# sile/libflate

Measured on AMD Instinct MI355X. Metric: gzip encode+decode throughput on 256 MiB synthetic text per GPU (uncompressed bytes through the round trip), higher is better.
Workload: dtype u8; 1 GPU; cfg2: gzip::Encoder (DefaultLz77Encoder, default options, mtime=0) + gzip::Decoder on TEXT(268435456 B) per GPU, write schedule S8K (8192-byte writes); bytes_per_gpu=268435456, schedule=S8K, compressed_bytes=129579521, parallelism=1 rank

## Files before the change

include/lfx_testhooks.h:

```cpp
#ifndef LFX_TESTHOOKS_H
#define LFX_TESTHOOKS_H

#include "lfx.h"

#ifdef __cplusplus
extern "C" {
#endif

int lfx_debug_huff_block(const uint32_t *hist320, uint32_t type, uint32_t *lit288, uint32_t *dist32, uint32_t *hdr160,
                         uint32_t *hdr_bits, uint64_t *body_bits);

int lfx_debug_plan(int format, const lfx_encode_opts *o, const lfx_schedule *s, uint64_t n, uint64_t *chunk_out,
                   size_t max_chunks, size_t *n_chunks, uint64_t *block_out, size_t max_blocks, size_t *n_blocks);

int lfx_debug_plan_incremental(int format, const lfx_encode_opts *o, const lfx_schedule *s, uint64_t n,
                               uint32_t take_every, uint64_t *chunk_out, size_t max_chunks, size_t *n_chunks,
                               uint64_t *block_out, size_t max_blocks, size_t *n_blocks);

void lfx_debug_symbols(uint32_t length, uint32_t distance, uint32_t *out6);

#ifdef __cplusplus
}
#endif
#endif
```

libflate_amd/_ffi.py:

```python
import ctypes as C
import os

_HERE = os.path.dirname(os.path.abspath(__file__))
SO_PATH = os.environ.get("LFX_SO") or os.path.join(_HERE, "liblfx.so")

DEFLATE, ZLIB, GZIP = 0, 1, 2
OK, E_INVALID_DATA, E_UNEXPECTED_EOF, E_IO, E_OOM, E_DEVICE, E_ARG, E_NOSPACE, E_UNSUPPORTED, E_WOULD_BLOCK = range(10)
LZ77_DEFAULT, LZ77_NOCOMPRESSION = 0, 1
FLUSH_NONE, FLUSH_SYNC = 0, 2
SCHED_SINGLE, SCHED_FIXED, SCHED_LIST = 0, 1, 2
SCHED_FLUSH = (1 << 64) - 1
DEC_MULTI = 1
DEC_NONBLOCKING = 2
MEMBERS_BGZF = 1
BGZF_MEMBER_SIZE = 65280

EXPORTS = [
    "lfx_encode_opts_default", "lfx_ctx_new", "lfx_ctx_free", "lfx_ctx_last_error", "lfx_ctx_set_stream",
    "lfx_device_count", "lfx_encode_bound", "lfx_encode_device", "lfx_encode_batch_device", "lfx_encode_host", "lfx_decode_device",
    "lfx_decode_host", "lfx_decode_batch_device", "lfx_encode_shard_prepare", "lfx_encode_shard_emit", "lfx_encode_shard_prezero", "lfx_decode_shard_device", "lfx_shard_place_device", "lfx_decode_range_scan", "lfx_decode_chain", "lfx_decode_range_emit", "lfx_decode_range_map", "lfx_decode_range_finish",
    "lfx_crc32_combine", "lfx_adler32_combine", "lfx_container_header_len", "lfx_encoder_new",
    "lfx_encoder_write", "lfx_encoder_write_codes", "lfx_encoder_flush", "lfx_encoder_finish", "lfx_encoder_last_error",
    "lfx_encoder_free", "lfx_decoder_new", "lfx_decoder_read", "lfx_decoder_unread",
    "lfx_decoder_consumed", "lfx_decoder_buffered", "lfx_decoder_surplus", "lfx_decoder_header", "lfx_decoder_last_error", "lfx_decoder_free", "lfx_lz77_new",
# ... 93 lines not shown
class LfxError(Exception):
    def __init__(self, status, message=""):
        super().__init__("lfx status %d: %s" % (status, message))
        self.status = status
        self.message = message


class DeviceError(LfxError):
    pass


_lib = None


def lib():
    global _lib
    if _lib is not None:
        return _lib
    if not os.path.exists(SO_PATH):
        raise ImportError(
            "libflate_amd: native library %s is missing — run `python -c 'import __graft_entry__ as g; "
            "g.build()'` (hipcc, gfx950). There is no CPU fallback." % SO_PATH)
    try:
        import torch
    except ImportError:
        pass
    L = C.CDLL(SO_PATH)
    u64, u32, vp, i32 = C.c_uint64, C.c_uint32, C.c_void_p, C.c_int
    L.lfx_encode_opts_default.argtypes = [C.POINTER(EncodeOpts)]
    L.lfx_ctx_new.restype = vp
    L.lfx_ctx_new.argtypes = [i32, C.POINTER(i32)]
    L.lfx_ctx_free.argtypes = [vp]
    L.lfx_ctx_last_error.restype = C.c_char_p
    L.lfx_ctx_last_error.argtypes = [vp]
    L.lfx_ctx_set_stream.argtypes = [vp, vp]
    L.lfx_encode_bound.restype = u64
    L.lfx_encode_bound.argtypes = [u64, C.POINTER(EncodeOpts), C.POINTER(Schedule)]
    L.lfx_encode_device.argtypes = [vp, i32, C.POINTER(EncodeOpts), C.POINTER(Schedule), vp, u64, vp, u64,
                                    C.POINTER(u64)]
    L.lfx_encode_host.argtypes = [vp, i32, C.POINTER(EncodeOpts), C.POINTER(Schedule), vp, u64, vp,
                                  u64, C.POINTER(u64)]
    L.lfx_host_alloc.restype = vp
    L.lfx_host_alloc.argtypes = [C.c_size_t]
    L.lfx_host_free.argtypes = [vp]
    L.lfx_ctx_match_fallbacks.restype = u64
    L.lfx_ctx_match_fallbacks.argtypes = [vp]
    L.lfx_decode_device.argtypes = [vp, i32, u32, vp, u64, vp, u64, C.POINTER(u64), C.POINTER(u64)]
    L.lfx_decode_host.argtypes = [vp, i32, u32, vp, u64, vp, u64, C.POINTER(u64), C.POINTER(u64)]
    L.lfx_decode_batch_device.argtypes = [vp, i32, u32, vp, vp, vp, vp, vp, vp, vp, vp]
    L.lfx_decode_members_device.argtypes = [vp, vp, u64, vp, u64, C.POINTER(u64), C.POINTER(u64), C.POINTER(Member), u32,
                                            C.POINTER(u32)]
    L.lfx_decode_members_host.argtypes = [vp, vp, u64, vp, u64, C.POINTER(u64), C.POINTER(u64), C.POINTER(Member), u32,
                                          C.POINTER(u32)]
    for f in (L.lfx_decode_size_device, L.lfx_decode_size_host):
        f.argtypes = [vp, i32, u32, vp, u64, C.POINTER(u64), C.POINTER(u64)]
    L.lfx_decode_batch_size_device.argtypes = [vp, i32, u32, vp, vp, vp, vp, vp, vp]
    for f in (L.lfx_decode_members_size_device, L.lfx_decode_members_size_host):
        f.argtypes = [vp, vp, u64, C.POINTER(u64), C.POINTER(u64), C.POINTER(Member), u32, C.POINTER(u32)]
    L.lfx_encode_members_bound.restype = u64
    L.lfx_encode_members_bound.argtypes = [u64, u64, u32, C.POINTER(EncodeOpts), C.POINTER(Schedule)]
    for f in (L.lfx_encode_members_device, L.lfx_encode_members_host):
        f.argtypes = [vp, C.POINTER(EncodeOpts), C.POINTER(Schedule), u64, u32, vp, u64, vp, u64, C.POINTER(u64),
                      C.POINTER(Member), u32, C.POINTER(u32)]
    L.lfx_members_gzi.argtypes = [C.POINTER(Member), u32, vp, u64, C.POINTER(u64)]
    L.lfx_decode_index_device.argtypes = [vp, i32, u32, vp, u64, vp, u64, C.POINTER(u64), C.POINTER(u64), u64, C.POINTER(vp)]
    L.lfx_encode_index_device.argtypes = [vp, i32, C.POINTER(EncodeOpts), C.POINTER(Schedule), vp, u64, vp, u64, C.POINTER(u64), u64,
                                          C.POINTER(vp)]
    L.lfx_index_read_device.argtypes = [vp, vp, vp, u64, u64, u32, vp, vp, vp, vp, vp, vp]
    L.lfx_index_span.argtypes = [vp, u64, u64, C.POINTER(u64), C.POINTER(u64)]
    L.lfx_index_get_info.argtypes = [vp, C.POINTER(IndexInfo)]
    L.lfx_index_get_point.argtypes = [vp, u32, C.POINTER(IndexPoint)]
    L.lfx_index_export.argtypes = [vp, vp, vp, u64, C.POINTER(u64)]
    L.lfx_index_import.argtypes = [vp, vp, u64, C.POINTER(i32)]
    L.lfx_index_import.restype = vp
    L.lfx_index_check.argtypes = [vp, u64, C.POINTER(IndexInfo)]
    L.lfx_index_free.argtypes = [vp]
    L.lfx_index_free.restype = None
    L.lfx_encode_batch_device.argtypes = [vp, i32, C.POINTER(EncodeOpts), C.POINTER(Schedule), u32, vp, vp, vp, vp, vp, vp, vp, vp]
    L.lfx_encode_shard_prepare.argtypes = [vp, i32, C.POINTER(EncodeOpts), C.POINTER(Schedule), vp, u64, i32,
                                           i32, C.POINTER(ShardInfo)]
    L.lfx_encode_shard_emit.argtypes = [vp, u64, u32, u64, vp, u64, C.POINTER(u64)]
    L.lfx_encode_shard_prezero.argtypes = [vp, vp, u64]
    L.lfx_decode_shard_device.argtypes = [vp, vp, u64, u64, u64, i32, vp, u64, C.POINTER(u64)]
    L.lfx_shard_place_device.argtypes = [vp, vp, u64, vp, u64, u64, i32]
    L.lfx_decode_range_scan.argtypes = [vp, vp, u64, u64, u64, u64, u64, u32, C.POINTER(BlkTuple), u32, C.POINTER(u32)]
    L.lfx_decode_chain.argtypes = [C.POINTER(BlkTuple), u32, u64, C.POINTER(u32), u32, C.POINTER(u32), C.POINTER(u64)]
    L.lfx_decode_range_emit.argtypes = [vp, vp, u64, u64, C.POINTER(BlkTuple), C.POINTER(u32), u32, u32, vp, u64,
                                        C.POINTER(u64), C.POINTER(u64), C.POINTER(u32)]
    L.lfx_decode_range_map.argtypes = [vp, vp]
    L.lfx_decode_range_finish.argtypes = [vp, vp, u32, C.POINTER(u32), C.POINTER(u32)]
    L.lfx_crc32_combine.restype = u32
    L.lfx_crc32_combine.argtypes = [u32, u32, u64]
    L.lfx_adler32_combine.restype = u32
    L.lfx_adler32_combine.argtypes = [u32, u32, u64]
    L.lfx_container_header_len.restype = u64
    L.lfx_container_header_len.argtypes = [i32, C.POINTER(EncodeOpts)]
    L.lfx_encoder_new.restype = vp
    L.lfx_encoder_new.argtypes = [vp, i32, C.POINTER(EncodeOpts), WRITE_CB, FLUSH_CB, vp, C.POINTER(i32)]
    L.lfx_encoder_write.restype = C.c_int64
    L.lfx_encoder_write.argtypes = [vp, C.c_char_p, C.c_size_t]
    L.lfx_encoder_write_codes.argtypes = [vp, C.POINTER(u32), C.c_size_t, C.c_char_p, C.c_size_t, i32]
    L.lfx_encoder_flush.argtypes = [vp]
    L.lfx_encoder_finish.argtypes = [vp]
    L.lfx_encoder_last_error.restype = C.c_char_p
    L.lfx_encoder_last_error.argtypes = [vp]
    L.lfx_encoder_free.argtypes = [vp]
    L.lfx_decoder_new.restype = vp
    L.lfx_decoder_new.argtypes = [vp, i32, u32, READ_CB, vp, C.POINTER(i32)]
    L.lfx_decoder_read.restype = C.c_int64
    L.lfx_decoder_read.argtypes = [vp, vp, C.c_size_t]
    L.lfx_decoder_unread.argtypes = [vp, C.POINTER(C.POINTER(C.c_uint8)), C.POINTER(C.c_size_t)]
    L.lfx_decoder_consumed.restype = u64
    L.lfx_decoder_consumed.argtypes = [vp]
    L.lfx_decoder_buffered.restype = u64
    L.lfx_decoder_buffered.argtypes = [vp]
    L.lfx_decoder_surplus.argtypes = [vp, C.POINTER(C.POINTER(C.c_uint8)), C.POINTER(C.c_size_t)]
    L.lfx_decoder_header.argtypes = [vp, C.POINTER(Header)]
    L.lfx_decoder_last_error.restype = C.c_char_p
    L.lfx_decoder_last_error.argtypes = [vp]
    L.lfx_decoder_free.argtypes = [vp]
    L.lfx_lz77_new.restype = vp
    L.lfx_lz77_new.argtypes = [vp, u32, u32, C.POINTER(i32)]
    L.lfx_lz77_encode.argtypes = [vp, C.c_char_p, C.c_size_t, SINK_CB, vp]
    L.lfx_lz77_flush.argtypes = [vp, SINK_CB, vp]
    L.lfx_lz77_window_size.restype = u32
    L.lfx_lz77_window_size.argtypes = [vp]
    L.lfx_lz77_compression_level.argtypes = [vp]
    L.lfx_lz77_free.argtypes = [vp]
    L.lfx_ctx_last_timing.argtypes = [vp, C.POINTER(Timing)]
    L.lfx_ctx_enable_timing.argtypes = [vp, i32]
    L.lfx_version.restype = u32
    L.lfx_comm_rccl.argtypes = [vp, vp, u32, u32, C.POINTER(Comm)]
    L.lfx_comm_rccl_free.argtypes = [C.POINTER(Comm)]
    L.lfx_comm_rccl_free.restype = None
    L.lfx_sharded_encode_begin.argtypes = [vp, C.POINTER(Comm), i32, C.POINTER(EncodeOpts), C.POINTER(Schedule), vp, u64, vp, u64,
                                           vp, u64, vp, u64, C.POINTER(vp), C.POINTER(ShardedPart)]
    L.lfx_sharded_encode_finish.argtypes = [vp, C.POINTER(Comm), vp, C.POINTER(u64)]
    L.lfx_sharded_byte_range.argtypes = [u64, u64, u32, u32, C.POINTER(u64), C.POINTER(u64), C.POINTER(u64)]
    L.lfx_sharded_byte_range.restype = None
    L.lfx_sharded_decode.argtypes = [vp, C.POINTER(Comm), vp, u64, u64, u64, u64, u64, vp, u64, C.POINTER(ShardedSlice)]
    L.lfx_sharded_layout.argtypes = [C.POINTER(Comm), C.POINTER(ShardInfo), u64, i32, C.POINTER(u64), C.POINTER(u32), C.POINTER(u64)]
    L.lfx_sharded_gather_tuples.argtypes = [C.POINTER(Comm), C.POINTER(BlkTuple), u32, i32, C.POINTER(C.POINTER(BlkTuple)),
                                            C.POINTER(u32), C.POINTER(u32)]
    L.lfx_sharded_fold.argtypes = [C.POINTER(Comm), i32, u32, u64, u32, u32, C.POINTER(u32), C.POINTER(u32), C.POINTER(u32),
                                   C.POINTER(u64), C.POINTER(u32)]
    L.lfx_sharded_free.argtypes = [vp]
    L.lfx_sharded_free.restype = None
    L.lfx_debug_huff_block.argtypes = [vp, u32, vp, vp, vp, C.POINTER(u32), C.POINTER(u64)]
    L.lfx_debug_plan.argtypes = [i32, C.POINTER(EncodeOpts), C.POINTER(Schedule), u64, vp, C.c_size_t,
                                 C.POINTER(C.c_size_t), vp, C.c_size_t, C.POINTER(C.c_size_t)]
    L.lfx_debug_plan_incremental.argtypes = [i32, C.POINTER(EncodeOpts), C.POINTER(Schedule), u64, u32, vp, C.c_size_t,
                                             C.POINTER(C.c_size_t), vp, C.c_size_t, C.POINTER(C.c_size_t)]
    L.lfx_debug_symbols.argtypes = [u32, u32, vp]
    _lib = L
    return L


def make_opts(**kw):
    o = EncodeOpts()
    lib().lfx_encode_opts_default(C.byref(o))
    keep = []
    for k, v in kw.items():
        if k == "extra":
            v = bytes(v)
            keep.append(v)
            o.extra, o.extra_len = v, len(v)
        elif k in ("filename", "comment"):
            v = bytes(v)
            keep.append(v)
            setattr(o, k, v)
        else:
            setattr(o, k, v)
    o._keep = keep
    return o


def members_to_gzi(members):
    members = list(members)
    table = (Member * max(len(members), 1))()
    for i, m in enumerate(members):
        table[i].in_off, table[i].in_len, table[i].out_off, table[i].out_len = m
    need = C.c_uint64(0)
    lib().lfx_members_gzi(table, len(members), None, 0, C.byref(need))
    buf = C.create_string_buffer(need.value)
    rc = lib().lfx_members_gzi(table, len(members), buf, need.value, C.byref(need))
    if rc:
        raise LfxError(rc, "lfx_members_gzi")
    return buf.raw[:need.value]


def make_schedule(write_size=0, writes=None):
    s = Schedule()
    if writes is not None:
        arr = (C.c_uint64 * len(writes))(*[SCHED_FLUSH if w is None else int(w) for w in writes])
        s.kind, s.writes, s.n_writes = SCHED_LIST, arr, len(writes)
        s._keep = arr
    elif write_size:
        s.kind, s.fixed_write = SCHED_FIXED, write_size
    else:
        s.kind = SCHED_SINGLE
    return s
```

libflate_amd/context.py:

```python
import ctypes as C

from . import _ffi


class Context:
    def __init__(self, device=0):
        st = C.c_int(0)
        self._h = _ffi.lib().lfx_ctx_new(device, C.byref(st))
        if not self._h:
            raise _ffi.DeviceError(st.value, "no usable MI355X device %d (there is no CPU fallback)" % device)
        self.device = device
        self._users = 0
        self._closing = False

    def _retain(self):
        self._users += 1

    def _release(self):
        self._users -= 1
        if self._users <= 0 and self._closing:
            self._free_now()

    def _free_now(self):
        if self._h:
            _ffi.lib().lfx_ctx_free(self._h)
            self._h = None

    def close(self):
        self._closing = True
        if self._users <= 0:
            self._free_now()

    def __del__(self):
        try:
            self.close()
        except Exception:
            pass

    @property
    def handle(self):
        return self._h

    def last_error(self):
        return (_ffi.lib().lfx_ctx_last_error(self._h) or b"").decode("utf-8", "replace")

    def set_stream(self, hip_stream_ptr):
        _ffi.lib().lfx_ctx_set_stream(self._h, hip_stream_ptr)

    def enable_timing(self, on=True):
        _ffi.lib().lfx_ctx_enable_timing(self._h, int(on) if on is not True and on is not False and 2 <= int(on) <= 6 else (1 if on else 0))

    def last_timing(self):
        t = _ffi.Timing()
        if _ffi.lib().lfx_ctx_last_timing(self._h, C.byref(t)) != 0:
            return None
        return {"total_ms": t.total_ms,
                "phases": [(bytes(t.phase_name[i]).split(b"\0")[0].decode(), t.phase_ms[i])
                           for i in range(t.n_phases)]}

    def match_fallbacks(self):
        return int(_ffi.lib().lfx_ctx_match_fallbacks(self._h))

    def encode_host_ptr(self, fmt, in_ptr, n, out_ptr, cap, opts=None, schedule=None):
        out_len = C.c_uint64(0)
        rc = _ffi.lib().lfx_encode_host(self._h, fmt, C.byref(opts) if opts is not None else None,
                                        C.byref(schedule) if schedule is not None else None, in_ptr, n, out_ptr, cap, C.byref(out_len))
        if rc:
            raise (_ffi.DeviceError if rc == _ffi.E_DEVICE else _ffi.LfxError)(rc, self.last_error())
        return out_len.value

    def decode_host_ptr(self, fmt, in_ptr, n, out_ptr, cap, flags=0):
        out_len, consumed = C.c_uint64(0), C.c_uint64(0)
        rc = _ffi.lib().lfx_decode_host(self._h, fmt, flags, in_ptr, n, out_ptr, cap, C.byref(out_len), C.byref(consumed))
        if rc in (_ffi.E_DEVICE, _ffi.E_OOM, _ffi.E_ARG):
            raise (_ffi.DeviceError if rc == _ffi.E_DEVICE else _ffi.LfxError)(rc, self.last_error())
        return rc, out_len.value, consumed.value, self.last_error() if rc else ""

    def encode_device(self, fmt, d_in, n, d_out, cap, opts=None, schedule=None):
        out_len = C.c_uint64(0)
        rc = _ffi.lib().lfx_encode_device(self._h, fmt, C.byref(opts) if opts is not None else None,
                                          C.byref(schedule) if schedule is not None else None,
                                          d_in, n, d_out, cap, C.byref(out_len))
        if rc:
            raise (_ffi.DeviceError if rc == _ffi.E_DEVICE else _ffi.LfxError)(rc, self.last_error())
        return out_len.value

    def encode_index_device(self, fmt, d_in, n, d_out, cap, opts=None, schedule=None, spacing=1 << 20):
        out_len, h = C.c_uint64(0), C.c_void_p(None)
        rc = _ffi.lib().lfx_encode_index_device(self._h, fmt, C.byref(opts) if opts is not None else None,
                                                C.byref(schedule) if schedule is not None else None,
                                                d_in, n, d_out, cap, C.byref(out_len), spacing, C.byref(h))
        if rc:
            raise (_ffi.DeviceError if rc == _ffi.E_DEVICE else _ffi.LfxError)(rc, self.last_error())
        return out_len.value, h.value

    def decode_device(self, fmt, d_in, n, d_out, cap, flags=0):
        out_len, consumed = C.c_uint64(0), C.c_uint64(0)
        rc = _ffi.lib().lfx_decode_device(self._h, fmt, flags, d_in, n, d_out, cap, C.byref(out_len),
                                          C.byref(consumed))
        if rc in (_ffi.E_DEVICE, _ffi.E_OOM, _ffi.E_ARG):
            raise (_ffi.DeviceError if rc == _ffi.E_DEVICE else _ffi.LfxError)(rc, self.last_error())
        return rc, out_len.value, consumed.value, self.last_error() if rc else ""

    def decode_members_device(self, d_in, n, d_out, cap, max_members=None):
        return self._members(_ffi.lib().lfx_decode_members_device, d_in, n, d_out, cap, max_members)

    def decode_index_device(self, fmt, d_in, n, d_out, cap, spacing=1 << 20, flags=0):
        out_len, consumed, h = C.c_uint64(0), C.c_uint64(0), C.c_void_p(None)
        rc = _ffi.lib().lfx_decode_index_device(self._h, fmt, flags, d_in, n, d_out, cap, C.byref(out_len), C.byref(consumed),
                                                spacing, C.byref(h))
        if rc in (_ffi.E_DEVICE, _ffi.E_OOM, _ffi.E_ARG):
            raise (_ffi.DeviceError if rc == _ffi.E_DEVICE else _ffi.LfxError)(rc, self.last_error())
        return rc, out_len.value, consumed.value, h.value, self.last_error() if rc else ""

    def index_read_device(self, index_handle, d_in, in_base, n, offs, lens, d_out, out_offs):
        k = len(offs)
        a = lambda v: (C.c_uint64 * max(k, 1))(*v)
        o, ln, oo = a(offs), a(lens), a(out_offs)
        out_len, st = (C.c_uint64 * max(k, 1))(), (C.c_int32 * max(k, 1))()
        rc = _ffi.lib().lfx_index_read_device(self._h, index_handle, d_in, in_base, n, k, o, ln, d_out, oo, out_len, st)
        if rc in (_ffi.E_DEVICE, _ffi.E_OOM) or (rc == _ffi.E_ARG and not any(st[i] == _ffi.E_ARG for i in range(k))):
            raise (_ffi.DeviceError if rc == _ffi.E_DEVICE else _ffi.LfxError)(rc, self.last_error())
        return rc, list(out_len[:k]), list(st[:k]), self.last_error() if rc else ""

    def _members(self, fn, src, n, dst, cap, max_members):
        if max_members is None:
            max_members = n // 20 + 1
        table = (_ffi.Member * max(int(max_members), 1))()
        out_len, consumed, count = C.c_uint64(0), C.c_uint64(0), C.c_uint32(0)
        rc = fn(self._h, src, n, dst, cap, C.byref(out_len), C.byref(consumed), table, int(max_members), C.byref(count))
        if rc in (_ffi.E_DEVICE, _ffi.E_OOM, _ffi.E_ARG):
            raise (_ffi.DeviceError if rc == _ffi.E_DEVICE else _ffi.LfxError)(rc, self.last_error())
        members = [(m.in_off, m.in_len, m.out_off, m.out_len) for m in table[:min(count.value, int(max_members))]]
        return rc, out_len.value, consumed.value, members, self.last_error() if rc else ""

    def decode_members_host(self, data, cap=None, max_members=None):
        data = bytes(data)
        grow = cap is None
        cap = cap if cap is not None else max(1 << 16, len(data) * 16)
        while True:
            out = C.create_string_buffer(cap)
            rc, ol, used, members, msg = self._members(_ffi.lib().lfx_decode_members_host, data, len(data), out, cap, max_members)
            if grow and rc == _ffi.E_NOSPACE and cap < len(data) * 1040 + (1 << 20):
                cap *= 8
                continue
            return rc, out.raw[:ol], used, members, msg

    def _raise_fatal(self, rc):
        if rc in (_ffi.E_DEVICE, _ffi.E_OOM, _ffi.E_ARG):
            raise (_ffi.DeviceError if rc == _ffi.E_DEVICE else _ffi.LfxError)(rc, self.last_error())

    def decode_size_device(self, fmt, d_in, n, flags=0):
        out_len, consumed = C.c_uint64(0), C.c_uint64(0)
        rc = _ffi.lib().lfx_decode_size_device(self._h, fmt, flags, d_in, n, C.byref(out_len), C.byref(consumed))
        self._raise_fatal(rc)
        return rc, out_len.value, consumed.value, self.last_error() if rc else ""

    def decode_size_host(self, fmt, data, flags=0):
        data = bytes(data)
        out_len, consumed = C.c_uint64(0), C.c_uint64(0)
        rc = _ffi.lib().lfx_decode_size_host(self._h, fmt, flags, data, len(data), C.byref(out_len), C.byref(consumed))
        self._raise_fatal(rc)
        return rc, out_len.value, consumed.value, self.last_error() if rc else ""

    def decode_batch_size_device(self, fmt, d_in, in_offs, in_lens):
        k = len(in_offs)
        a = lambda v: (C.c_uint64 * max(k, 1))(*v)
        io, il = a(in_offs), a(in_lens)
        ol, used, st = (C.c_uint64 * max(k, 1))(), (C.c_uint64 * max(k, 1))(), (C.c_int32 * max(k, 1))()
        rc = _ffi.lib().lfx_decode_batch_size_device(self._h, fmt, k, d_in, io, il, ol, used, st)
        if rc:
            raise (_ffi.DeviceError if rc == _ffi.E_DEVICE else _ffi.LfxError)(rc, self.last_error())
        return list(ol[:k]), list(used[:k]), list(st[:k])

    def _members_size(self, fn, src, n, max_members):
        if max_members is None:
            max_members = n // 20 + 1
        table = (_ffi.Member * max(int(max_members), 1))()
        out_len, consumed, count = C.c_uint64(0), C.c_uint64(0), C.c_uint32(0)
        rc = fn(self._h, src, n, C.byref(out_len), C.byref(consumed), table, int(max_members), C.byref(count))
        self._raise_fatal(rc)
        members = [(m.in_off, m.in_len, m.out_off, m.out_len) for m in table[:min(count.value, int(max_members))]]
        return rc, out_len.value, consumed.value, members, self.last_error() if rc else ""

    def decode_members_size_device(self, d_in, n, max_members=None):
        return self._members_size(_ffi.lib().lfx_decode_members_size_device, d_in, n, max_members)

    def decode_members_size_host(self, data, max_members=None):
        data = bytes(data)
        return self._members_size(_ffi.lib().lfx_decode_members_size_host, data, len(data), max_members)

    def _encode_members(self, fn, src, n, dst, cap, member_size, flags, opts, schedule, max_members):
        count = 0 if (flags & _ffi.MEMBERS_BGZF and n == 0) else max(1, -(-n // member_size)) if member_size else 0
        if max_members is None:
            max_members = count
        table = (_ffi.Member * max(int(max_members), 1))()
        out_len, got = C.c_uint64(0), C.c_uint32(0)
        rc = fn(self._h, C.byref(opts) if opts is not None else None, C.byref(schedule) if schedule is not None else None,
                member_size, flags, src, n, dst, cap, C.byref(out_len), table, int(max_members), C.byref(got))
        if rc in (_ffi.E_DEVICE, _ffi.E_OOM, _ffi.E_ARG, _ffi.E_UNSUPPORTED):
            raise (_ffi.DeviceError if rc == _ffi.E_DEVICE else _ffi.LfxError)(rc, self.last_error())
        members = [(m.in_off, m.in_len, m.out_off, m.out_len) for m in table[:min(got.value, int(max_members))]]
        return rc, out_len.value, got.value, members, self.last_error() if rc else ""

    def encode_members_device(self, d_in, n, d_out, cap, member_size=1 << 20, flags=0, opts=None, schedule=None, max_members=None):
        return self._encode_members(_ffi.lib().lfx_encode_members_device, d_in, n, d_out, cap, member_size, flags, opts, schedule,
                                    max_members)

    def encode_members_host(self, data, member_size=1 << 20, flags=0, opts=None, schedule=None, cap=None, max_members=None):
        data = bytes(data)
        if cap is None:
# ... 46 lines not shown
```

libflate_amd/csrc/lfx_api.cpp:

```cpp
#include "../../include/lfx.h"
#include "../../include/lfx_testhooks.h"

#include <hip/hip_runtime.h>

#include <algorithm>
#include <cstddef>
#include <cstdio>
#include <cstdlib>
#include <cstring>
#include <mutex>
#include <string>
#include <vector>

#include "lfx_ctx.h"
#include "lfx_device.h"
#include "lfx_huff.h"
#include "lfx_index.h"
#include "lfx_plan.h"
#include "lfx_abi_guard.h"

using namespace lfx;

static uint32_t host_crc32(const uint8_t *p, size_t n) {
    static uint32_t tab[256];
// ... 54 lines not shown
    lfx_encode_opts d;
    if (o) d = *o; else lfx_encode_opts_default(&d);
    if (d.window_size > MAX_WINDOW) d.window_size = MAX_WINDOW;
    if (d.max_length > MAX_LENGTH) d.max_length = MAX_LENGTH;
    return d;
}
static int check_opts(const lfx_encode_opts &o) {
    if (o.block_size == 0) return LFX_E_ARG;
    if (o.max_length < 3) return LFX_E_ARG;
    return LFX_OK;
}
static PlanOpts plan_opts(int format, const lfx_encode_opts &o) {
    PlanOpts p;
    p.block_size = o.block_size;
    p.dynamic_huffman = o.dynamic_huffman != 0;
    p.no_compression = o.no_compression != 0;
    p.lz77_kind = o.lz77_kind;
    p.window_size = o.window_size;
    p.max_length = o.max_length;
    p.zlib_sync = format == LFX_ZLIB && o.zlib_flush_mode == LFX_FLUSH_SYNC;
    return p;
}

static void gzip_header(const lfx_encode_opts &o, bool with_hcrc, std::vector<uint8_t> &b) {
    uint8_t flg = (uint8_t)((o.is_text ? 1 : 0) | (with_hcrc ? 2 : 0) | (o.extra ? 4 : 0) |
                            (o.filename ? 8 : 0) | (o.comment ? 16 : 0));
    const uint8_t xfl = o.lz77_level == 1 + LFX_LEVEL_FAST ? 4 : o.lz77_level == 1 + LFX_LEVEL_BEST ? 2 : 0;
    const uint8_t h[10] = {31, 139, 8, flg, (uint8_t)o.mtime, (uint8_t)(o.mtime >> 8),
                           (uint8_t)(o.mtime >> 16), (uint8_t)(o.mtime >> 24), xfl, o.os};
    b.insert(b.end(), h, h + 10);
    if (o.extra) {
        b.push_back((uint8_t)o.extra_len);
        b.push_back((uint8_t)(o.extra_len >> 8));
        b.insert(b.end(), o.extra, o.extra + o.extra_len);
    }
    if (o.filename) b.insert(b.end(), o.filename, o.filename + strlen(o.filename) + 1);
    if (o.comment) b.insert(b.end(), o.comment, o.comment + strlen(o.comment) + 1);
    if (with_hcrc) {
        std::vector<uint8_t> t;
        gzip_header(o, false, t);
        uint32_t c = host_crc32(t.data(), t.size());
        b.push_back((uint8_t)c);
        b.push_back((uint8_t)(c >> 8));
    }
}
static int container_header(int format, const lfx_encode_opts &o, std::vector<uint8_t> &b) {
    if (format == LFX_GZIP) {
        if (o.extra && o.extra_len > 0xFFFF) return LFX_E_INVALID_DATA;
        gzip_header(o, o.hcrc != 0, b);
    } else if (format == LFX_ZLIB) {
        uint32_t ws = o.window_size;
        uint8_t cinfo = ws > 16384 ? 7 : ws > 8192 ? 6 : ws > 4096 ? 5 : ws > 2048 ? 4 : ws > 1024 ? 3
                        : ws > 512 ? 2 : ws > 256 ? 1 : 0;
        uint8_t level = (o.no_compression || o.lz77_kind == LFX_LZ77_NOCOMPRESSION) ? 0 : 2;
        if (o.lz77_level && !o.no_compression) level = (uint8_t)((o.lz77_level - 1) & 3);
        uint8_t cmf = (uint8_t)((cinfo << 4) | 8), flg = (uint8_t)(level << 6);
        uint32_t check = ((uint32_t)cmf << 8) + flg;
        if (check % 31 != 0) flg = (uint8_t)(flg + (31 - check % 31));
        b.push_back(cmf);
        b.push_back(flg);
    } else if (format != LFX_DEFLATE) {
        return LFX_E_ARG;
    }
    return LFX_OK;
}
extern "C" uint64_t lfx_container_header_len(int format, const lfx_encode_opts *o) {
    std::vector<uint8_t> b;
    lfx_encode_opts d = norm_opts(o);
    container_header(format, d, b);
    return b.size();
}

static void apply_schedule(Planner &pl, const lfx_schedule *s, uint64_t n) {
    if (!s || s->kind == LFX_SCHED_SINGLE) {
        pl.write(n);
    } else if (s->kind == LFX_SCHED_FIXED) {
        uint64_t w = s->fixed_write ? s->fixed_write : n;
        if (w) {
            pl.write_repeat(w, n / w);
            if (n % w) pl.write(n % w);
        }
    } else {
        uint64_t used = 0;
        for (size_t i = 0; i < s->n_writes; i++) {
            if (s->writes[i] == LFX_SCHED_FLUSH) { pl.flush(); continue; }
            uint64_t w = std::min(s->writes[i], n - used);
            pl.write(w);
            used += w;
        }
        if (used < n) pl.write(n - used);
    }
}

extern "C" uint64_t lfx_encode_bound(uint64_t n, const lfx_encode_opts *o, const lfx_schedule *s) {
    lfx_encode_opts d = norm_opts(o);
    if (check_opts(d)) return 0;
    Planner pl(plan_opts(LFX_ZLIB, d));
    apply_schedule(pl, s, n);
    Plan &p = pl.finish();
    uint64_t hdr = 64 + (d.extra ? d.extra_len + 2 : 0) + (d.filename ? strlen(d.filename) + 1 : 0) +
                   (d.comment ? strlen(d.comment) + 1 : 0);
    return n + n / 4 + 1024 * (uint64_t)p.blocks.size() + hdr + 64;
}

namespace lfx {

#define HIP_TRY(expr)                                                                 \
    do {                                                                              \
        hipError_t e_ = (expr);                                                       \
        if (e_ != hipSuccess) {                                                       \
            c->set_error(std::string(#expr) + ": " + hipGetErrorString(e_));          \
            return LFX_E_DEVICE;                                                      \
        }                                                                             \
    } while (0)

int DevBuf::reserve(size_t bytes) {
    if (bytes <= cap) return 0;
    if (p) (void)hipFree(p);
    p = nullptr;
    cap = 0;
    gen++;
    size_t want = bytes + bytes / 8 + 4096;
    if (hipMalloc(&p, want) != hipSuccess) {
        if (hipMalloc(&p, bytes) != hipSuccess) { p = nullptr; return LFX_E_OOM; }
        want = bytes;
    }
    cap = want;
    return 0;
}
void DevBuf::release() {
    if (p) (void)hipFree(p);
    p = nullptr;
    cap = 0;
}

void Diag::read() {
    auto on = [](const char *k) { return getenv(k) != nullptr; };
    debug = on("LFX_DEBUG");
    match_v1 = on("LFX_MATCH_V1");
    match_v5 = on("LFX_MATCH_V5");
    if (const char *mp = getenv("LFX_MATCH_PARTS")) match_parts = atoi(mp);
    if (const char *rc7 = getenv("LFX_R7_CAP")) r7_cap = atoi(rc7);
    no_serial = on("LFX_NO_SERIAL");
    batch_serial = on("LFX_BATCH_SERIAL");
    no_pieces = on("LFX_NO_PIECES");
    no_final_cand = on("LFX_NO_FINAL_CAND");
    if (const char *eb = getenv("LFX_ENC_BATCH_MB")) enc_batch_mb = atoi(eb);
    two_pass = on("LFX_TWO_PASS");
    hist_separate = on("LFX_HIST_SEPARATE");
    find2_exp = getenv("LFX_FIND2_EXP") ? atoi(getenv("LFX_FIND2_EXP")) : 0;
    no_pin_slots = on("LFX_NO_PIN_SLOTS");
    no_small_scan = on("LFX_NO_SMALL_SCAN");
    store_tight = on("LFX_STORE_TIGHT");
}

void Ctx::phase(const char *name) {
    if (!timing_on) return;
    if (timing_on >= 2 && timing_on <= 5) {
        static const char *const pair[4][2] = {{"lz77_resolve", "lz77_walk"}, {"find2", "blk_scan"}, {"upload", "lz77_cand"}, {"blk_emit", "lz77_copy"}};
        const char *const *pr = pair[timing_on - 2];
        if (strcmp(name, pr[0]) != 0 && strcmp(name, pr[1]) != 0) return;
    }
    if (n_ev >= 17) return;
    if (!ev[n_ev]) (void)hipEventCreate(&ev[n_ev]);
    (void)hipEventRecord(ev[n_ev], stream);
    snprintf(ev_name[n_ev], sizeof ev_name[n_ev], "%s", name);
    n_ev++;
}

}

extern "C" int lfx_device_count(void) {
    int n = 0;
    if (hipGetDeviceCount(&n) != hipSuccess) return 0;
    return n;
}

extern "C" lfx_ctx *lfx_ctx_new(int device, int *status) try {
    int st = LFX_OK;
    int n = 0;
    if (hipGetDeviceCount(&n) != hipSuccess || n <= 0 || device < 0 || device >= n) {
        if (status) *status = LFX_E_DEVICE;
        return nullptr;
    }
    Ctx *c = new Ctx();
    c->device = device;
    if (hipSetDevice(device) != hipSuccess || hipStreamCreate(&c->own_stream) != hipSuccess) {
        delete c;
        if (status) *status = LFX_E_DEVICE;
        return nullptr;
    }
    c->stream = c->own_stream;
    c->diag.read();
    (void)hipDeviceGetAttribute(&c->n_cu, hipDeviceAttributeMultiprocessorCount, device);
    if (hipStreamCreateWithFlags(&c->side_stream, hipStreamNonBlocking) != hipSuccess ||
        hipEventCreateWithFlags(&c->ev_fork, hipEventDisableTiming) != hipSuccess ||
        hipEventCreateWithFlags(&c->ev_join, hipEventDisableTiming) != hipSuccess ||
        hipEventCreateWithFlags(&c->ev_zero, hipEventDisableTiming) != hipSuccess ||
        hipEventCreateWithFlags(&c->ev_res, hipEventDisableTiming) != hipSuccess ||
        hipEventCreateWithFlags(&c->ev_part[0], hipEventDisableTiming) != hipSuccess ||
        hipEventCreateWithFlags(&c->ev_part[1], hipEventDisableTiming) != hipSuccess ||
        hipEventCreateWithFlags(&c->ev_part[2], hipEventDisableTiming) != hipSuccess ||
        hipEventCreateWithFlags(&c->ev_part[3], hipEventDisableTiming) != hipSuccess) {
        (void)hipStreamDestroy(c->own_stream);
        delete c;
        if (status) *status = LFX_E_DEVICE;
        return nullptr;
    }
    if (hipHostMalloc((void **)&c->h_res, 4096 + Ctx::PIN_ARENA, hipHostMallocDefault) != hipSuccess) {
        (void)hipStreamDestroy(c->own_stream);
        delete c;
        if (status) *status = LFX_E_OOM;
        return nullptr;
    }
    if (status) *status = st;
    return reinterpret_cast<lfx_ctx *>(c);
} LFX_ABI_CATCH_NEW
extern "C" void lfx_ctx_free(lfx_ctx *cc) {
    if (!cc) return;
    Ctx *c = reinterpret_cast<Ctx *>(cc);
    (void)hipSetDevice(c->device);
    (void)hipStreamSynchronize(c->stream);
    for (DevBuf *b : c->all_bufs()) b->release();
    for (DevBuf &b : c->dev_pool) b.release();
    c->dev_pool.clear();
    c->pin_pool.clear();
    for (auto &e : c->ev) if (e) (void)hipEventDestroy(e);
    if (c->h_res) (void)hipHostFree(c->h_res);
    c->hostio.release();
    if (c->ev_fork) (void)hipEventDestroy(c->ev_fork);
    if (c->ev_join) (void)hipEventDestroy(c->ev_join);
    if (c->ev_zero) (void)hipEventDestroy(c->ev_zero);
    if (c->ev_res) (void)hipEventDestroy(c->ev_res);
    for (hipEvent_t e : c->ev_part) if (e) (void)hipEventDestroy(e);
    if (c->side_stream) (void)hipStreamDestroy(c->side_stream);
    if (c->own_stream) (void)hipStreamDestroy(c->own_stream);
    delete c;
}
extern "C" const char *lfx_ctx_last_error(const lfx_ctx *cc) {
    return cc ? reinterpret_cast<const Ctx *>(cc)->err.c_str() : "no context";
}
extern "C" void lfx_ctx_set_stream(lfx_ctx *cc, void *s) {
    Ctx *c = reinterpret_cast<Ctx *>(cc);
    c->stream = s ? (hipStream_t)s : c->own_stream;
}
extern "C" uint64_t lfx_ctx_match_fallbacks(const lfx_ctx *cc) {
    return cc ? reinterpret_cast<const Ctx *>(cc)->match_fallbacks : 0;
}
extern "C" void lfx_ctx_enable_timing(lfx_ctx *cc, int on) { reinterpret_cast<Ctx *>(cc)->timing_on = on >= 2 && on <= 6 ? on : on != 0; }
extern "C" int lfx_ctx_last_timing(lfx_ctx *cc, lfx_timing *t) try {
    Ctx *c = reinterpret_cast<Ctx *>(cc);
    std::lock_guard<std::recursive_mutex> lock(c->mu);
    memset(t, 0, sizeof *t);
    if (c->n_ev < 2) return LFX_E_ARG;
    (void)hipEventSynchronize(c->ev[c->n_ev - 1]);
    (void)hipEventElapsedTime(&t->total_ms, c->ev[0], c->ev[c->n_ev - 1]);
    t->n_phases = c->n_ev - 1;
    for (int i = 0; i + 1 < c->n_ev && i < 16; i++) {
        (void)hipEventElapsedTime(&t->phase_ms[i], c->ev[i], c->ev[i + 1]);
        snprintf(t->phase_name[i], sizeof t->phase_name[i], "%s", c->ev_name[i + 1]);
    }
    return LFX_OK;
} LFX_ABI_CATCH

namespace lfx {

int encode_prepare(Ctx *c, const Plan &plan, const PlanOpts &po, const uint8_t *d_in, uint64_t n,
                   int ck_mode, const HostCodes *hc) {
    const bool want_checksum = ck_mode != 0;
    (void)hipSetDevice(c->device);
    hipStream_t st = c->stream;
    c->n_ev = 0;
    c->phase("start");
    for (const ChunkDesc &ch : plan.chunks)
        if (ch.len >= (1ull << 32) - 4) {
            c->set_error("an LZ77 chunk of 4 GiB or more is outside the reference's domain (u32 positions, default.rs:78)");
            return LFX_E_ARG;
        }
    const uint32_t nchunks = (uint32_t)plan.chunks.size(), nblocks = (uint32_t)plan.blocks.size();
    const bool match_v1 = c->force_match_v1 || c->diag.match_v1;
    if (c->force_match_v1 && !hc) c->match_fallbacks++;
    std::vector<SegDesc> segs;
    if (!hc) {
        uint64_t seg_len = SEG_POSITIONS;
        for (;;) {
            uint64_t cnt = 0;
            for (const ChunkDesc &ch : plan.chunks)
                if (!(ch.flags & CH_LITERALS) && ch.len > 3) cnt += div_up(ch.len - 3, seg_len);
            if (cnt >= 512 || seg_len <= 32768) break;
            seg_len /= 2;
        }
        for (uint32_t ci = 0; ci < nchunks; ci++) {
            const ChunkDesc &ch = plan.chunks[ci];
            if (ch.flags & CH_LITERALS) continue;
            for (uint64_t s = 0; s + 3 < ch.len; s += seg_len)
                segs.push_back(SegDesc{ci, (uint32_t)s, (uint32_t)std::min<uint64_t>(seg_len, ch.len - s), 0});
        }
    }
    uint64_t lnk_units = 0;
    for (SegDesc &sg : segs) {
        if (lnk_units > 0xFFFFFFFFull) { c->set_error("input too large for the link scratch"); return LFX_E_ARG; }
        sg.lnk_base = (uint32_t)lnk_units;
        lnk_units += div_up((uint64_t)sg.len + std::min<uint64_t>(sg.start, MAX_WINDOW) + 4, 64);
        lnk_units = (lnk_units + 1) & ~1ull;
    }
    std::vector<ParseWg> pwgs;
    for (uint32_t ci = 0; ci < nchunks && !hc; ci++) {
        const ChunkDesc &ch = plan.chunks[ci];
        if (ch.flags & CH_LITERALS) continue;
        for (uint32_t s = 0; s < ch.n_seg; s += PARSE_WG_SEGS) pwgs.push_back(ParseWg{ci, s});
    }
    if (pwgs.size() > 8) {
        const size_t nl = pwgs.size(), per = (nl + 7) / 8;
        std::vector<ParseWg> phys(per * 8);
        for (size_t i = 0; i < phys.size(); i++) {
            const size_t l = (i % 8) * per + i / 8;
            phys[i] = (i / 8 < per && l < nl && l / per == i % 8) ? pwgs[l] : ParseWg{0xFFFFFFFFu, 0u};
        }
        pwgs.swap(phys);
    }
    c->cur_nchunks = nchunks;
    c->cur_nblocks = nblocks;
    c->cur_ntiles = plan.n_tiles;
    c->cur_n = n;
    c->cur_in = d_in;
    int rc;
    if ((rc = c->d_chunks.reserve(sizeof(ChunkDesc) * std::max<size_t>(nchunks, 1)))) return rc;
    if ((rc = c->d_blocks.reserve(sizeof(BlockDesc) * std::max<size_t>(nblocks, 1)))) return rc;
    if ((rc = c->d_segs.reserve(sizeof(SegDesc) * std::max<size_t>(segs.size(), 1)))) return rc;
    if ((rc = c->d_pwgs.reserve(sizeof(ParseWg) * std::max<size_t>(pwgs.size(), 1)))) return rc;
    if (!hc && (rc = c->d_cd.reserve(2 * n + 64))) return rc;
    if (!hc && !match_v1 && (rc = c->d_glnk.reserve(264 * std::max<uint64_t>(lnk_units, 1)))) return rc;
    if (!hc && !match_v1 && (rc = c->d_ucount.reserve(4 * std::max<size_t>(segs.size(), 1)))) return rc;
    if (!hc && match_v1 && (rc = c->d_md.reserve(4 * std::max<uint64_t>(n, 1)))) return rc;
    if ((rc = c->d_codes.reserve(4 * std::max<uint64_t>(plan.n_codes_cap, 1)))) return rc;
    if ((rc = c->d_ncodes.reserve(4 * std::max<size_t>(nchunks, 1)))) return rc;
    if ((rc = c->d_vis.reserve(8 * std::max<uint64_t>(plan.n_vis, 1)))) return rc;
    if ((rc = c->d_segtmp.reserve(24ull * std::max<uint32_t>(plan.n_segs, 1)))) return rc;
    if (!hc && (rc = c->d_stage.reserve(4ull * (n + 64)))) return rc;
    if ((rc = c->d_chunkmap.reserve(4ull * (plan.n_tiles + plan.n_segs + 2)))) return rc;
    if ((rc = c->d_hist.reserve(4ull * 320 * std::max<size_t>(nblocks, 1)))) return rc;
    if ((rc = c->d_bc.reserve(sizeof(BlockCodes) * std::max<size_t>(nblocks, 1)))) return rc;
    if ((rc = c->d_block_start.reserve(8 * std::max<size_t>(nblocks, 1)))) return rc;
    if ((rc = c->d_tile_bits.reserve(4 * std::max<uint64_t>(plan.n_tiles, 1)))) return rc;
    if ((rc = c->d_tile_start.reserve(8 * std::max<uint64_t>(plan.n_tiles, 1)))) return rc;
    const uint64_t nspans = ck_nspans(n);
    if ((rc = c->d_ck.reserve(12 * nspans))) return rc;
    if ((rc = c->d_res.reserve(256))) return rc;
    if ((rc = c->d_small.reserve(70000))) return rc;

    auto upload = [&](int slot, DevBuf &b, const void *src, size_t bytes) -> hipError_t {
        std::vector<uint8_t> &sh = c->up_shadow[slot];
        const uint64_t tag = (uint64_t)(uintptr_t)b.p ^ ((uint64_t)b.gen << 48) ^ (1ull << 63);
        if (c->up_dev[slot] == tag && sh.size() == bytes && (bytes == 0 || memcmp(sh.data(), src, bytes) == 0)) return hipSuccess;
        sh.assign((const uint8_t *)src, (const uint8_t *)src + bytes);
        c->up_dev[slot] = tag;
        return bytes ? hipMemcpyAsync(b.p, sh.data(), bytes, hipMemcpyHostToDevice, st) : hipSuccess;
    };
    HIP_TRY(upload(0, c->d_chunks, plan.chunks.data(), sizeof(ChunkDesc) * nchunks));
    HIP_TRY(upload(1, c->d_blocks, plan.blocks.data(), sizeof(BlockDesc) * nblocks));
    HIP_TRY(upload(2, c->d_segs, segs.data(), sizeof(SegDesc) * segs.size()));
    HIP_TRY(upload(3, c->d_pwgs, pwgs.data(), sizeof(ParseWg) * pwgs.size()));
    const bool ucount_here = !hc && !match_v1 && !c->diag.match_v5;
    const ZeroSpan z_hist{(uint32_t *)c->d_hist.p, (uint32_t)(320 * std::max<size_t>(nblocks, 1))}, z_res{(uint32_t *)c->d_res.p, 64u},
        z_ucount{ucount_here ? (uint32_t *)c->d_ucount.p : nullptr, ucount_here ? (uint32_t)std::max<size_t>(segs.size(), 1) : 0u};
    c->phase("upload");
    uint32_t *tile_map = (uint32_t *)c->d_chunkmap.p, *seg_map = tile_map + plan.n_tiles;
    c->cur_tile_map = tile_map;
    if (int e_ = launch_chunk_maps(st, (const ChunkDesc *)c->d_chunks.p, nchunks, plan.n_tiles, plan.n_segs, tile_map, seg_map, z_hist,
                                   z_res, z_ucount)) {
        c->set_error(hipGetErrorString((hipError_t)e_));
        return LFX_E_DEVICE;
    }

#define LAUNCH_TRY(call)                                                              \
    do {                                                                              \
        int e_ = (call);                                                              \
        if (e_) {                                                                     \
            c->set_error(std::string(#call) + ": " + hipGetErrorString((hipError_t)e_)); \
            return LFX_E_DEVICE;                                                      \
        }                                                                             \
    } while (0)

    uint64_t *mdbg = nullptr;
    if (c->diag.debug) mdbg = (uint64_t *)((uint8_t *)c->d_small.p + 32768);
    bool fused_hist = false;
    bool forked = false;
    uint32_t emit_per = 0, emit_parts = 0;
    if (hc) {
        if (hc->n_codes) HIP_TRY(hipMemcpyAsync(c->d_codes.p, hc->codes, 4ull * hc->n_codes, hipMemcpyHostToDevice, st));
        if (nchunks) HIP_TRY(hipMemcpyAsync(c->d_ncodes.p, hc->chunk_codes, 4ull * nchunks, hipMemcpyHostToDevice, st));
        c->phase("codes_upload");
    } else {
    uint32_t *d_match_flags = (uint32_t *)((uint8_t *)c->d_res.p + offsetof(EncodeResult, match_flags));
    uint16_t *d_cd = (uint16_t *)c->d_cd.p;
    if (match_v1) {
        LAUNCH_TRY(launch_match(st, d_in, n, (const ChunkDesc *)c->d_chunks.p, (const SegDesc *)c->d_segs.p,
                                (uint32_t)segs.size(), po.window_size, po.max_length, (uint32_t *)c->d_md.p, mdbg));
        LAUNCH_TRY(launch_md_to_cd(st, (const uint32_t *)c->d_md.p, n, d_cd));
    } else {
// ... 1164 lines not shown
```

libflate_amd/csrc/lfx_blk.h:

```cpp
#pragma once
#include <stdint.h>

namespace lfx {

enum : uint32_t { BLK_OK = 0, BLK_BAD = 1, BLK_NO_EOB = 2 };
constexpr uint32_t BLK_PIECE_KNOWN = 2;
struct BlkJob {
    uint64_t start_bit;
    uint64_t end_bit;
    uint64_t lo_bit, warm_bit;
    uint32_t piece, _pad;
    uint64_t temp_off;
    uint32_t cap, _pad2;
};
struct BlkInfo {
    uint64_t end_bit;
    uint64_t n_out;
    uint64_t data_bit;
    uint32_t n_codes;
    uint32_t status, btype, bfinal, nlanes, rounds;
    uint32_t _pad;
    uint32_t cyc_hdr, cyc_total;
};
struct BlkLanes {
    uint64_t start[1024];
    uint64_t out_off[1024];
    uint32_t code_off[1024];
};
struct BlkLanesX {
    uint32_t n_head[1024];
    uint32_t n_rest[1024];
    uint32_t rest_at[1024];
    int32_t reach[1024];
    uint32_t cut_code[1024];
    uint32_t cut_out[1024];
};
struct BlkEmit {
    uint64_t start_bit, data_bit;
    uint64_t code_off;
    uint64_t out_off;
    uint64_t n_out;
    uint32_t n_codes, nlanes, btype, cand;
    uint64_t hist;
    uint64_t end_limit;
    uint32_t preload;
    uint32_t placed;
    uint64_t temp_off;
    uint32_t cap, _pad;
};
constexpr uint32_t MAX_FREE_UNITS = 64;
struct BlkUnits {
    uint32_t n;
    uint32_t code0[9];
    uint64_t out0[9];
    uint32_t cyc[4];
    uint32_t fn;
    uint32_t fcode0[MAX_FREE_UNITS + 1];
    uint64_t fout0[MAX_FREE_UNITS + 1];
};
struct SymUnit {
    uint64_t start;
    uint64_t len;
};
}
```

libflate_amd/csrc/lfx_ctx.h:

```cpp
#pragma once
#include <hip/hip_runtime.h>

#include <mutex>
#include <string>
#include <vector>

#include "lfx_common.h"
#include "lfx_device.h"
#include <string.h>

#include "lfx_hostio.h"

namespace lfx {

struct DevBuf {
    void *p = nullptr;
    size_t cap = 0;
    uint32_t gen = 0;
    int reserve(size_t bytes);
    void release();
};

struct Diag {
    bool debug = false;
    bool match_v1 = false;
    bool match_v5 = false;
    int r7_cap = 0;
    int match_parts = 1;
    bool no_serial = false;
    bool batch_serial = false;
    bool no_pieces = false;
    bool no_final_cand = false;
    bool no_small_scan = false;
    bool two_pass = false;
    bool no_pin_slots = false;
    int find2_exp = 0;
    bool hist_separate = false;
    bool store_tight = false;
    int enc_batch_mb = 0;
    void read();
};

struct RangeState {
    int state = -1;
    uint64_t total = 0, before = 0, max_len = 0;
    uint8_t *d_out = nullptr;
    uint32_t nsu = 0;
};

struct Ctx {
    int device = 0;
    RangeState range;
    std::vector<uint8_t> range_stored;
    std::vector<uint64_t> range_temp_off;
    std::vector<uint32_t> range_cap;
    Diag diag;
    int n_cu = 0;
    hipStream_t own_stream = nullptr, stream = nullptr;
    hipStream_t side_stream = nullptr;
    hipEvent_t ev_fork = nullptr, ev_join = nullptr, ev_zero = nullptr;
    hipEvent_t ev_part[4] = {}, ev_res = nullptr;
    const void *prezero_ptr = nullptr;
    uint64_t prezero_bytes = 0;
    std::recursive_mutex mu;
    std::string err;
    void set_error(const std::string &e) { err = e; }

    DevBuf d_chunks, d_blocks, d_segs, d_pwgs, d_cd, d_md, d_codes, d_ncodes, d_hist, d_bc, d_block_start, d_tile_bits,
        d_tile_start, d_ck, d_res, d_small, d_hdr, d_io_in, d_io_out, d_vis, d_segtmp, d_stage, d_chunkmap, d_glnk, d_ucount;
    std::vector<uint8_t> up_shadow[4];
    uint64_t up_dev[4] = {0, 0, 0, 0};
    DevBuf d_dec_streams, d_dec_state, d_dec_tmp, d_dec_cand, d_dec_blocks, d_dec_tabs, d_dec_sym, d_dec_win, d_dec_maps,
        d_dec_temp, d_dec_lanesx;
    DevBuf d_idx_tasks, d_idx_probe, d_idx_stage;
    DevBuf d_idx_enc;
    struct IdxCollect *idx = nullptr;
    struct IdxCollect *idx_enc = nullptr;
    std::vector<DevBuf *> all_bufs() {
        return {&d_chunks, &d_blocks, &d_segs, &d_pwgs, &d_cd, &d_md, &d_codes, &d_ncodes, &d_hist, &d_bc, &d_block_start,
                &d_tile_bits, &d_tile_start, &d_ck, &d_res, &d_small, &d_hdr, &d_io_in, &d_io_out, &d_vis, &d_segtmp, &d_stage, &d_chunkmap, &d_glnk, &d_ucount,
                &d_dec_streams, &d_dec_state, &d_dec_tmp, &d_dec_cand, &d_dec_blocks, &d_dec_tabs, &d_dec_sym, &d_dec_win, &d_dec_maps,
                &d_dec_temp, &d_dec_lanesx, &d_idx_tasks, &d_idx_probe, &d_idx_stage, &d_idx_enc};
    }
    void *h_res = nullptr;
    static constexpr size_t PIN_ARENA = 1u << 20;
    size_t pin_used = 0;
    struct PinDown { void *slot, *dst; size_t n; };
    std::vector<PinDown> pin_pending;
    void pin_reset() { pin_used = 0; pin_pending.clear(); }
    void *pin_take(size_t n) {
        const size_t at = (pin_used + 63) & ~(size_t)63;
        if (!h_res || diag.no_pin_slots || at + n > PIN_ARENA) return nullptr;
        pin_used = at + n;
        return (uint8_t *)h_res + 4096 + at;
    }
    hipError_t small_up(void *dev, const void *host, size_t n, hipStream_t st) {
        if (!n) return hipSuccess;
        void *slot = pin_take(n);
        if (!slot) return hipMemcpyAsync(dev, host, n, hipMemcpyHostToDevice, st);
        memcpy(slot, host, n);
        return hipMemcpyAsync(dev, slot, n, hipMemcpyHostToDevice, st);
    }
    hipError_t small_down(void *host, const void *dev, size_t n, hipStream_t st) {
        if (!n) return hipSuccess;
        void *slot = pin_take(n);
        if (!slot) return hipMemcpyAsync(host, dev, n, hipMemcpyDeviceToHost, st);
        pin_pending.push_back({slot, host, n});
        return hipMemcpyAsync(slot, dev, n, hipMemcpyDeviceToHost, st);
    }
    hipError_t small_sync(hipStream_t st) {
        const hipError_t e = hipStreamSynchronize(st);
        for (const PinDown &d : pin_pending) memcpy(d.dst, d.slot, d.n);
        pin_pending.clear();
        return e;
    }

    uint32_t cur_nchunks = 0, cur_nblocks = 0;
    uint64_t cur_ntiles = 0, cur_n = 0;
    const uint32_t *cur_tile_map = nullptr;
    const uint8_t *cur_in = nullptr;
    bool force_match_v1 = false;
    uint64_t match_fallbacks = 0;
    HostIo hostio;
    static constexpr size_t POOL_MAX = 8;
    std::vector<PinVec> pin_pool;
    std::vector<DevBuf> dev_pool;
    PinVec take_pin() {
        std::lock_guard<std::recursive_mutex> lock(mu);
        if (pin_pool.empty()) return PinVec();
        size_t best = 0;
        for (size_t i = 1; i < pin_pool.size(); i++)
            if (pin_pool[i].capacity() > pin_pool[best].capacity()) best = i;
        PinVec v = std::move(pin_pool[best]);
        pin_pool.erase(pin_pool.begin() + (std::ptrdiff_t)best);
        v.clear();
        return v;
    }
    void give_pin(PinVec &&v) {
        std::lock_guard<std::recursive_mutex> lock(mu);
        if (v.capacity() && pin_pool.size() < POOL_MAX) { v.clear(); pin_pool.push_back(std::move(v)); }
    }
    DevBuf take_dev() {
        std::lock_guard<std::recursive_mutex> lock(mu);
        if (dev_pool.empty()) return DevBuf();
        DevBuf b = dev_pool.back();
        dev_pool.pop_back();
        return b;
    }
    void give_dev(DevBuf &b) {
        std::lock_guard<std::recursive_mutex> lock(mu);
        if (b.p && dev_pool.size() < POOL_MAX) dev_pool.push_back(b);
        else b.release();
        b = DevBuf();
    }
    std::vector<uint8_t> shard_hdr;
    int shard_format = 0;
    bool shard_last = false;

    int timing_on = 0;
    bool timing_fine() const { return timing_on >= 2; }
    hipEvent_t ev[17] = {};
    char ev_name[17][24] = {};
    int n_ev = 0;
    void phase(const char *name);
};

struct HostCodes {
    const uint32_t *codes;
    uint64_t n_codes;
    const uint32_t *chunk_codes;
};
int encode_prepare(Ctx *c, const struct Plan &plan, const struct PlanOpts &po, const uint8_t *d_in,
                   uint64_t n, int ck_mode, const HostCodes *hc = nullptr);

}
```

libflate_amd/csrc/lfx_decode.h:

```cpp
#pragma once
#include <hip/hip_runtime.h>
#include <stdint.h>

#include "lfx_common.h"
#include "lfx_blk.h"

namespace lfx {

enum : uint32_t {
    ERR_NONE = 0,
    ERR_EOF,
    ERR_HUFF,
    ERR_CONFLICT,
    ERR_HDIST,
    ERR_NO_PREV,
    ERR_DIST_LIST,
    ERR_286,
    ERR_BACKREF,
    ERR_BTYPE3,
    ERR_LEN_NLEN,
    ERR_STORED_SHORT,
    ERR_NOSPACE,
    ERR_ZLIB_CHECK, ERR_METHOD, ERR_CINFO, ERR_FDICT,
    ERR_GZIP_ID, ERR_HCRC,
    ERR_CRC32, ERR_ADLER32,
};

struct DecStream {
    uint64_t in_off, in_len;
    uint64_t out_off, out_cap;
};
struct DecHeader {
    uint64_t deflate_off;
    uint32_t status;
    uint32_t err, a0, a1;
    uint32_t flags;
    uint32_t _pad;
};

enum : uint32_t { JOB_SINGLE_BLOCK = 1, JOB_COUNT_ONLY = 2 };
struct InflateJob {
    uint64_t in_off;
    uint64_t in_len;
    uint64_t start_bit;
    uint64_t out_off, out_cap;
    uint64_t hist_avail;
    uint64_t stop_bit;
    uint32_t flags;
    uint32_t _pad;
};
struct InflateResult {
    uint64_t end_bit;
    uint64_t out_len;
    uint32_t status;
    uint32_t final_seen;
    uint32_t err, a0, a1;
    uint32_t needs_hist;
    uint32_t nblocks;
    uint32_t _pad;
    uint64_t blk_out_start;
    uint64_t blk_start_bit;
};

enum : uint32_t { WALK_FINAL = 0,
                  WALK_STOP = 1,
                  WALK_STUCK = 2 };
struct WalkJob {
    uint64_t start_bit;
    uint64_t end_bit;
    uint64_t stop_bit;
};
struct WalkResult {
    uint64_t end_bit;
    uint64_t n_out;
    uint64_t stuck_bit, stuck_out;
    int64_t reach;
    uint32_t status, nblocks;
};
int launch_blk_walk_size(hipStream_t st, const uint8_t *in, uint64_t nbytes, const WalkJob *jobs, uint32_t njobs,
                         WalkResult *results, bool small_blocks);
size_t blk_tabs_bytes();
int launch_blk_scan(hipStream_t st, const uint8_t *in, uint64_t nbytes, const BlkJob *jobs, uint32_t njobs,
                    BlkInfo *infos, BlkLanes *lanes, void *tabs = nullptr,
                    bool small_blocks = false);
int launch_blk_scan_store(hipStream_t st, const uint8_t *in, uint64_t nbytes, const BlkJob *jobs, uint32_t njobs,
                          BlkInfo *infos, BlkLanes *lanes, void *tabs, uint32_t *temp, BlkLanesX *lanesx);
int launch_blk_place(hipStream_t st, const BlkEmit *jobs, uint32_t njobs, const BlkLanes *lanes, const BlkLanesX *lanesx,
                     const uint32_t *temp, uint32_t *codes, uint32_t *flags, BlkUnits *units, uint32_t unit_target,
                     uint32_t *job_flags, uint32_t free_shift);
int launch_blk_emit(hipStream_t st, const uint8_t *in, uint64_t nbytes, const BlkEmit *jobs, uint32_t njobs,
                    const BlkLanes *lanes, uint32_t *codes, uint32_t *flags, BlkUnits *units, uint32_t unit_target,
                    uint32_t *job_flags = nullptr,
                    const void *tabs = nullptr,
                    uint32_t free_shift = 17,
                    bool large_blocks = false,
                    bool small_blocks = false);
int launch_blk_materialize(hipStream_t st, const uint8_t *in, const BlkEmit *jobs, uint32_t njobs,
                           const BlkLanes *lanes, const BlkUnits *units, const uint32_t *codes, uint8_t *out,
                           uint64_t *dbg);

int launch_blk_materialize_sym(hipStream_t st, const uint8_t *in, const BlkEmit *jobs, uint32_t njobs,
                               const BlkUnits *units, const uint32_t *codes, uint16_t *sym,
                               bool few_units = false );
int launch_window_chain(hipStream_t st, const uint16_t *sym, const SymUnit *units, uint32_t nunits, uint8_t *windows,
                        const uint8_t *init_win = nullptr);
size_t window_prefix_scratch_bytes(uint32_t nunits);
int launch_window_prefix(hipStream_t st, const uint16_t *sym, const SymUnit *units, uint32_t nunits, void *scratch,
                         uint8_t *windows, const uint8_t *init_win = nullptr);
int launch_window_rank_map(hipStream_t st, const uint16_t *sym, const SymUnit *units, uint32_t nunits, void *scratch, uint16_t *out_map);
int launch_bytes_to_map(hipStream_t st, const uint8_t *out, uint64_t len, uint16_t *map);
int launch_window_ranks(hipStream_t st, const uint16_t *maps, uint32_t nranks, uint8_t *win);
int launch_sym_substitute(hipStream_t st, const uint16_t *sym, const SymUnit *units, uint32_t nunits,
                          const uint8_t *windows, uint8_t *out, uint64_t max_len, const uint8_t *init_win = nullptr);

int launch_container(hipStream_t st, int format, uint32_t count, const uint8_t *in,
                     const DecStream *streams, DecHeader *hdrs);
int launch_inflate(hipStream_t st, const uint8_t *in, uint8_t *out, const InflateJob *jobs,
                   InflateResult *results, uint32_t njobs);
constexpr uint32_t FIND_SHARDS = 256;
constexpr uint32_t FIND_HDR_WORDS = 1024, FIND_HDR_FINAL = 320, FIND_HDR_DBG = 360, FIND_HDR_READ = 512 ;
constexpr uint32_t FIND2_GROUPS = 16, FIND_HDR_WORK = 512, FIND_HDR_WORK_STRIDE = 32;
inline uint32_t find_shard_cap(uint64_t comp_bytes) {
    const uint64_t want = comp_bytes / 4000;
    return (uint32_t)(want < 4096 ? 4096 : want > (1u << 23) ? (1u << 23) : want);
}
int launch_find_stage1(hipStream_t st, const uint8_t *in, uint64_t nbytes, uint64_t first_byte,
                       uint32_t *count, uint64_t *cand, uint32_t shard_cap, uint64_t final_from_bit, uint32_t n_cu);
int launch_find_stage2(hipStream_t st, const uint8_t *in, uint64_t nbytes, const uint64_t *cand,
                       uint32_t shard_cap, const uint32_t *count ,
                       uint32_t *work ,
                       uint32_t *final_count, uint64_t *final_list, uint32_t final_cap, uint32_t n_cu,
                       uint64_t *dbg = nullptr ,
                       int exp = 0 );
constexpr uint64_t MEMBER_TILE = 16384;
constexpr uint64_t MEMBER_SKIP = ~0ull;
inline uint64_t member_tiles(uint64_t n) { return (n + MEMBER_TILE - 1) / MEMBER_TILE; }
int launch_member_count(hipStream_t st, const uint8_t *in, uint64_t n, uint32_t *tile_count );
int launch_member_emit(hipStream_t st, const uint8_t *in, uint64_t n, const uint64_t *tile_pos ,
                       uint64_t *out, uint64_t cap);
int launch_verify_trailers(hipStream_t st, int format, uint32_t count, const uint8_t *in,
                           const DecStream *streams, const DecHeader *hdrs, InflateResult *results,
                           const uint32_t *crc, const uint32_t *adler, uint64_t *consumed);
}
```

libflate_amd/csrc/lfx_device.h:

```cpp
#pragma once
#include <hip/hip_runtime.h>
#include <stdint.h>

#include "../../include/lfx.h"
#include "lfx_common.h"

namespace lfx {

struct SegDesc {
    uint32_t chunk;
    uint32_t start;
    uint32_t len;
    uint32_t lnk_base;
};
constexpr uint32_t SEG_POSITIONS = 256 * 1024;

struct EncodeResult {
    uint64_t end_bit;
    uint64_t out_bytes;
    uint32_t status;
    uint32_t crc32;
    uint32_t adler32;
    uint32_t match_flags;
};

struct BatchStream {
    uint64_t in_off, in_len;
    uint64_t out_off, out_cap;
    uint32_t first_block, n_blocks;
};

struct ParseWg {
    uint32_t chunk;
    uint32_t seg0;
};

int launch_match(hipStream_t st, const uint8_t *in, uint64_t in_bytes, const ChunkDesc *chunks,
                 const SegDesc *segs, uint32_t nsegs, uint32_t window, uint32_t max_len, uint32_t *md,
                 uint64_t *dbg = nullptr);
int launch_match7(hipStream_t st, const uint8_t *in, uint64_t in_bytes, const ChunkDesc *chunks, const SegDesc *segs,
                  uint32_t nsegs, uint32_t window, uint16_t *cd, uint32_t *glnk ,
                  uint64_t *umask , uint32_t *flags, uint64_t *dbg = nullptr);
int launch_resolve7(hipStream_t st, const ChunkDesc *chunks, const SegDesc *segs, uint32_t nsegs, uint32_t window, uint16_t *cd,
                    const uint32_t *glnk, const uint64_t *umask, uint32_t *ulist ,
                    uint32_t *ucount ,
                    uint32_t hop_cap = 0 );
int launch_match5(hipStream_t st, const uint8_t *in, uint64_t in_bytes, const ChunkDesc *chunks, const SegDesc *segs,
                  uint32_t nsegs, uint32_t window, uint16_t *cd, uint16_t *glnk, uint32_t *flags, uint64_t *dbg = nullptr);
int launch_md_to_cd(hipStream_t st, const uint32_t *md, uint64_t n, uint16_t *cd);
int launch_parse(hipStream_t st, const uint8_t *in, uint64_t in_bytes, const ChunkDesc *chunks, uint32_t nchunks,
                 uint32_t nsegs, const ParseWg *wgs, uint32_t nwgs, const uint16_t *cd, uint32_t max_len, uint64_t *vis,
                 uint32_t *seg_tmp, uint32_t *codes, uint32_t *ncodes, uint32_t *stage ,
                 const uint32_t *seg_map, int stop_after = 0 ,
                 uint64_t *dbg = nullptr ,
                 uint32_t *hist = nullptr ,
                 uint32_t emit_per = 0 ,
                 uint32_t emit_parts = 0 ,
                 hipEvent_t ev_walked = nullptr ,
                 const uint32_t *mflags = nullptr ,
                 int start_at = 0 );
struct ZeroSpan { uint32_t *p; uint32_t n; };
int launch_chunk_maps(hipStream_t st, const ChunkDesc *chunks, uint32_t nchunks, uint64_t ntiles, uint32_t nsegs,
                      uint32_t *tile_map, uint32_t *seg_map, ZeroSpan z0 = ZeroSpan{nullptr, 0}, ZeroSpan z1 = ZeroSpan{nullptr, 0},
                      ZeroSpan z2 = ZeroSpan{nullptr, 0});
int launch_histogram(hipStream_t st, const ChunkDesc *chunks, uint32_t nchunks, uint32_t split,
                     const uint32_t *codes, const uint32_t *ncodes, uint32_t *hist);
int launch_huffman(hipStream_t st, const BlockDesc *blocks, uint32_t nblocks, const uint32_t *hist,
                   BlockCodes *bc, uint64_t *dbg = nullptr);
int launch_offsets(hipStream_t st, const BlockDesc *blocks, uint32_t nblocks, const BlockCodes *bc,
                   uint64_t start_bit, uint64_t cap_bits, uint64_t *block_start, EncodeResult *res);
int launch_offsets_batch(hipStream_t st, const BatchStream *streams, uint32_t count, const BlockDesc *blocks, const BlockCodes *bc,
                         uint32_t hdr_len, uint32_t trailer_len, uint64_t *block_start, uint64_t *stream_end, int32_t *status,
                         EncodeResult *res);
int launch_frame_batch(hipStream_t st, int format, const BatchStream *streams, uint32_t count, const uint8_t *hdr, uint32_t hdr_len,
                       const uint64_t *stream_end, const uint32_t *crc, const uint32_t *adler, const EncodeResult *res, uint32_t *out,
                       uint64_t *out_len);
struct MembersGeom {
    uint64_t n, member_size;
    uint32_t count;
    uint32_t bpm, bpm_last;
    uint32_t hdr_len;
    uint32_t bgzf;
};
int launch_members_layout(hipStream_t st, const MembersGeom &g, BlockDesc *blocks, const BlockCodes *bc, uint64_t *local_off,
                          uint64_t *mlen, uint64_t *wg_sum, uint64_t cap, uint64_t *block_start, lfx_member *members,
                          EncodeResult *res);
int launch_members_frame(hipStream_t st, const MembersGeom &g, const uint8_t *hdr, const lfx_member *members, const uint32_t *crc,
                         const EncodeResult *res, uint32_t *out);
int launch_pack(hipStream_t st, const uint8_t *in, uint64_t in_bytes, const ChunkDesc *chunks,
                uint32_t nchunks, const BlockDesc *blocks, uint32_t nblocks, uint64_t ntiles,
                const uint32_t *codes, const uint32_t *ncodes, const BlockCodes *bc,
                const uint64_t *block_start, uint32_t *tile_bits, uint64_t *tile_start,
                const EncodeResult *res, uint64_t out_base_bit, uint32_t *out, const uint32_t *tile_map);
inline uint32_t ck_span(uint64_t n) { return n <= (64ull << 20) ? 8192u : 65536u; }
inline uint64_t ck_nspans(uint64_t n) { return div_up(n ? n : 1, ck_span(n)); }
int launch_checksum(hipStream_t st, const uint8_t *in, uint64_t n, uint32_t *crc_part,
                    uint32_t *a_part, uint32_t *b_part, EncodeResult *res,
                    int mode = 3)   ;
int launch_checksum_part(hipStream_t st, const uint8_t *in, uint64_t n, uint32_t *crc_part, uint32_t *a_part, uint32_t *b_part,
                         EncodeResult *res, int mode, uint32_t part, uint32_t nparts);
int launch_checksum_ranges(hipStream_t st, const uint8_t *data, uint32_t count, const uint64_t *off,
                           uint32_t off_stride, const uint64_t *len, uint32_t len_stride, uint32_t *crc, uint32_t *adler);
int launch_or_byte(hipStream_t st, uint8_t *dst, const uint8_t *src);
int launch_put_bytes(hipStream_t st, const uint8_t *d_bytes, uint32_t n, uint64_t at_byte, uint32_t *out);
int launch_trailer(hipStream_t st, int format, uint32_t isize, uint64_t out_base_bit,
                   EncodeResult *res, uint32_t *out);

}
```

libflate_amd/csrc/lfx_encode_kernels.hip:

```cpp
#include <hip/hip_runtime.h>
#include <stdint.h>

#include "lfx_common.h"
#include "lfx_device.h"
#include "lfx_huff.h"

namespace lfx {

struct ByteSrc {
    gptr_u32 w;
    uint64_t shift;
    uint64_t nbytes;
    __device__ __forceinline__ uint32_t load4(uint64_t off) const {
        uint64_t a = off + shift;
        uint64_t idx = a >> 2;
        uint32_t sh = (uint32_t)a & 3;
        uint64_t last = (nbytes + shift + 3) >> 2;
        uint32_t w0 = idx < last ? w[idx] : 0;
        uint32_t w1 = (sh != 0 && idx + 1 < last) ? w[idx + 1] : 0;
        return __builtin_amdgcn_alignbyte(w1, w0, sh);
    }
    __device__ __forceinline__ uint32_t load1(uint64_t off) const {
        uint64_t a = off + shift;
        return (w[a >> 2] >> (((uint32_t)a & 3) * 8)) & 0xFF;
// ... 746 lines not shown
}
__constant__ Xp8Table XP8 = cx_xp8_table();

struct AdvTable { uint32_t t[4][256]; };
constexpr uint32_t cx_xpow8n(uint64_t n) {
    uint32_t r = 0x80000000u, sq = 0x00800000u;
    while (n) { if (n & 1) r = cx_mulmod(r, sq); sq = cx_mulmod(sq, sq); n >>= 1; }
    return r;
}
constexpr AdvTable cx_adv_table() {
    AdvTable a{};
    const uint32_t adv = cx_xpow8n(4096 - 64);
    for (int k = 0; k < 4; ++k)
        for (uint32_t b = 0; b < 256; ++b) a.t[k][b] = cx_mulmod(b << (8 * k), adv);
    return a;
}
__constant__ AdvTable ADV = cx_adv_table();

__device__ __forceinline__ uint32_t gf2_xpow8n(uint64_t nbytes) {
    uint32_t r = 0x80000000u;
    bool first = true;
    for (uint32_t k = 0; nbytes; ++k, nbytes >>= 1)
        if (nbytes & 1) {
            const uint32_t f = XP8.v[k < 47 ? k : 47];
            r = first ? f : gf2_mulmod(r, f);
            first = false;
        }
    return r;
}

__device__ __forceinline__ void ck_tables(uint32_t (*tab)[256], uint32_t (*advt)[256]) {
    {
        uint32_t c = threadIdx.x;
        for (int k = 0; k < 8; ++k) c = (c >> 1) ^ (CRC_POLY & (0u - (c & 1)));
        tab[0][threadIdx.x] = c;
    }
    for (int k = 0; k < 4; ++k) advt[k][threadIdx.x] = ADV.t[k][threadIdx.x];
    __syncthreads();
    for (int t = 1; t < 4; ++t) {
        const uint32_t pv = tab[t - 1][threadIdx.x];
        tab[t][threadIdx.x] = (pv >> 8) ^ tab[0][pv & 0xFF];
        __syncthreads();
    }
}

struct CkPartial { uint32_t crc, a, b; };
template <int MODE = 3>
__device__ __forceinline__ CkPartial ck_span_partial(const uint8_t *p, uint32_t rlen, uint32_t lane,
                                                     const uint32_t (*tab)[256], const uint32_t (*advt)[256]) {
    constexpr bool CRC = (MODE & 1) != 0, ADL = (MODE & 2) != 0;
    const ByteSrc src = make_src(p, rlen);
    uint32_t crc = 0, stand = 0;
    uint32_t s1 = 0, s1_before = 0;
    uint64_t s2 = 0;
    const uint32_t first = 64 * lane;
    const uint32_t shb = (uint32_t)src.shift;
    const bool wide = shb == 0 && ((uint64_t)src.w & 15) == 0;
    auto load_piece = [&](uint32_t (&w)[16], uint32_t o) {
        if (wide) {
            const uint32_t last16 = (rlen - 1) >> 4;
            const uint4 *w16 = (const uint4 *)src.w;
#pragma unroll
            for (uint32_t q = 0; q < 4; ++q) {
                const uint32_t i = min((o >> 4) + q, last16);
                const uint4 v = w16[i];
                w[4 * q] = v.x; w[4 * q + 1] = v.y; w[4 * q + 2] = v.z; w[4 * q + 3] = v.w;
            }
        } else {
            const uint32_t lastd = (rlen + shb - 1) >> 2;
            const uint32_t i0 = (o + shb) >> 2;
            uint32_t raw[17];
#pragma unroll
            for (uint32_t q = 0; q < 17; ++q) raw[q] = src.w[min(i0 + q, lastd)];
#pragma unroll
            for (uint32_t q = 0; q < 16; ++q) w[q] = __builtin_amdgcn_alignbyte(raw[q + 1], raw[q], shb);
        }
#pragma unroll
        for (uint32_t q = 0; q < 16; ++q) {
            const int rem = (int)rlen - (int)(o + 4 * q);
            w[q] = rem >= 4 ? w[q] : rem <= 0 ? 0u : w[q] & ((1u << (8 * rem)) - 1u);
        }
    };
    auto walk_piece = [&](const uint32_t (&w)[16], uint32_t o) {
        if (CRC && o != first)
            crc = advt[0][crc & 0xFF] ^ advt[1][(crc >> 8) & 0xFF] ^ advt[2][(crc >> 16) & 0xFF] ^ advt[3][crc >> 24];
        const uint32_t len = min(64u, rlen - o);
        uint32_t wsum = 0;
#pragma unroll
        for (uint32_t q = 0; q < 16; ++q) {
            const uint32_t m = len > 4 * q ? min(4u, len - 4 * q) : 0u;
            if (m == 4) {
                if (CRC) {
                    const uint32_t x = crc ^ w[q];
                    crc = tab[3][x & 0xFF] ^ tab[2][(x >> 8) & 0xFF] ^ tab[1][(x >> 16) & 0xFF] ^ tab[0][x >> 24];
                }
                if (ADL) {
                    const uint32_t b0 = w[q] & 0xFF, b1 = (w[q] >> 8) & 0xFF, b2 = (w[q] >> 16) & 0xFF, b3 = w[q] >> 24;
                    s1 += b0 + b1 + b2 + b3;
                    wsum += 4 * q * (b0 + b1 + b2 + b3) + b1 + 2 * b2 + 3 * b3;
                }
            } else {
                for (uint32_t k = 0; k < m; ++k) {
                    const uint32_t byte = (w[q] >> (8 * k)) & 0xFF;
                    if (CRC) crc = (crc >> 8) ^ tab[0][(crc ^ byte) & 0xFF];
                    if (ADL) { s1 += byte; wsum += (4 * q + k) * byte; }
                }
            }
        }
        s2 += (uint64_t)o * (s1 - s1_before) + wsum;
        s1_before = s1;
        stand = o + len;
    };
    uint32_t wa[16], wb[16];
    load_piece(wa, first);
    for (uint32_t o = first; o < rlen; o += 2 * 4096) {
        load_piece(wb, o + 4096);
        walk_piece(wa, o);
        load_piece(wa, o + 2 * 4096);
        if (o + 4096 < rlen) walk_piece(wb, o + 4096);
    }
    CkPartial r;
    r.crc = 0; r.a = 0; r.b = 0;
    if (CRC) {
        uint32_t reg = first < rlen ? gf2_mulmod(crc, gf2_xpow8n(rlen - stand)) : 0u;
        for (int o = 32; o > 0; o >>= 1) reg ^= __shfl_xor(reg, o);
        r.crc = reg;
    }
    if (ADL) {
        uint64_t t1 = s1, t2 = s2 % 65521u;
        for (int o = 32; o > 0; o >>= 1) { t1 += __shfl_xor(t1, o); t2 += __shfl_xor(t2, o); }
        r.a = (uint32_t)(t1 % 65521u);
        r.b = (uint32_t)(((uint64_t)(rlen % 65521u) * r.a + 65521ull * 65521ull - (t2 % 65521u)) % 65521u);
    }
    return r;
}

template <int MODE>
__global__ __launch_bounds__(256) void checksum_span_kernel(const uint8_t *__restrict__ in,
                                                            uint64_t n, uint32_t span, uint32_t *__restrict__ crc_part,
                                                            uint32_t *__restrict__ a_part,
                                                            uint32_t *__restrict__ b_part, uint64_t region0) {
    __shared__ uint32_t tab[4][256];
    __shared__ uint32_t advt[4][256];
    ck_tables(tab, advt);
    const uint32_t lane = threadIdx.x & 63;
    const uint64_t region = region0 + (uint64_t)blockIdx.x * 4 + (threadIdx.x >> 6);
    const uint64_t r0 = region * span;
    if (r0 >= n) return;
    const uint32_t rlen = (uint32_t)min((uint64_t)span, n - r0);
    const CkPartial r = ck_span_partial<MODE>(in + r0, rlen, lane, tab, advt);
    if (lane == 0) { crc_part[region] = r.crc; a_part[region] = r.a; b_part[region] = r.b; }
}

__global__ __launch_bounds__(256) void checksum_ranges_kernel(const uint8_t *__restrict__ data, uint32_t count,
                                                              const uint64_t *__restrict__ off, uint32_t off_stride,
                                                              const uint64_t *__restrict__ len, uint32_t len_stride,
                                                              uint32_t *__restrict__ crc_out,
                                                              uint32_t *__restrict__ adler_out) {
    __shared__ uint32_t tab[4][256];
    __shared__ uint32_t advt[4][256];
    ck_tables(tab, advt);
    const uint32_t lane = threadIdx.x & 63;
    const uint32_t i = blockIdx.x * 4 + (threadIdx.x >> 6);
    if (i >= count) return;
    const uint8_t *p = data + off[(uint64_t)i * off_stride];
    const uint64_t n = len[(uint64_t)i * len_stride];
    uint32_t crc = 0, a = 0, b = 0;
    const uint32_t xs = gf2_xpow8n(CK_SPAN);
    for (uint64_t o = 0; o < n; o += CK_SPAN) {
        const uint32_t sl = (uint32_t)min((uint64_t)CK_SPAN, n - o);
        const CkPartial r = ck_span_partial(p + o, sl, lane, tab, advt);
        crc = gf2_mulmod(crc, sl == CK_SPAN ? xs : gf2_xpow8n(sl)) ^ r.crc;
        b = (uint32_t)((b + r.b + (sl % 65521u) * (uint64_t)a) % 65521u);
        a = (a + r.a) % 65521u;
    }
    if (lane == 0) {
        crc_out[i] = crc ^ gf2_mulmod(0xFFFFFFFFu, gf2_xpow8n(n)) ^ 0xFFFFFFFFu;
        const uint32_t A = (1u + a) % 65521u;
        const uint32_t B = (uint32_t)((n % 65521u + b) % 65521u);
        adler_out[i] = (B << 16) | A;
    }
}

__global__ __launch_bounds__(1024) void checksum_combine_kernel(const uint32_t *__restrict__ crc_part,
                                                                const uint32_t *__restrict__ a_part,
                                                                const uint32_t *__restrict__ b_part,
                                                                uint64_t n, uint32_t span,
                                                                EncodeResult *__restrict__ res) {
    __shared__ uint32_t s_crc[16], s_a[16], s_b[16];
    const uint64_t nspans = div_up(n, span);
    const uint64_t per = div_up(nspans ? nspans : 1, 1023);
    const uint32_t t = threadIdx.x;
    uint32_t crc = 0, a = 0, b = 0;
    if (t < 1023) {
        const uint64_t lo = (uint64_t)t * per, hi = min(nspans, lo + per);
        if (lo < hi) {
            uint64_t len = 0;
            const uint32_t xs = gf2_xpow8n(span);
            for (uint64_t s = lo; s < hi; ++s) {
                const uint64_t sl = min((uint64_t)span, n - s * span);
                const uint32_t sh = sl == span ? xs : gf2_xpow8n(sl);
                crc = gf2_mulmod(crc, sh) ^ crc_part[s];
                b = (uint32_t)((b + b_part[s] + (sl % 65521u) * (uint64_t)a) % 65521u);
                a = (a + a_part[s]) % 65521u;
                len += sl;
            }
            const uint64_t after = n - (lo * span + len);
            if (after) crc = gf2_mulmod(crc, gf2_xpow8n(after));
            b = (uint32_t)((b + (after % 65521u) * (uint64_t)a) % 65521u);
        }
    } else {
        crc = gf2_mulmod(0xFFFFFFFFu, gf2_xpow8n(n));
    }
    for (int o = 32; o > 0; o >>= 1) {
        crc ^= __shfl_xor(crc, o);
        a += __shfl_xor(a, o);
        b += __shfl_xor(b, o);
    }
    if ((t & 63) == 0) { s_crc[t >> 6] = crc; s_a[t >> 6] = a; s_b[t >> 6] = b; }
    __syncthreads();
    if (t == 0) {
        uint32_t c = 0;
        uint64_t A = 0, B = 0;
        for (int w = 0; w < 16; ++w) { c ^= s_crc[w]; A += s_a[w]; B += s_b[w]; }
        res->crc32 = c ^ 0xFFFFFFFFu;
        const uint32_t Af = (uint32_t)((1u + A) % 65521u);
        const uint32_t Bv = (uint32_t)((n % 65521u + B) % 65521u);
        res->adler32 = (Bv << 16) | Af;
    }
}

__global__ void put_bytes_kernel(const uint8_t *__restrict__ bytes, uint32_t n, uint64_t at_byte,
                                 uint32_t *__restrict__ out) {
    for (uint32_t i = threadIdx.x; i < n; i += blockDim.x) {
        const uint64_t ob = at_byte + i;
        atomicOr(&out[ob >> 2], (uint32_t)bytes[i] << (8 * (ob & 3)));
    }
}
__global__ void or_byte_kernel(uint8_t *__restrict__ dst, const uint8_t *__restrict__ src) {
    if (threadIdx.x == 0 && blockIdx.x == 0) dst[0] = (uint8_t)(dst[0] | src[0]);
}
int launch_or_byte(hipStream_t st, uint8_t *dst, const uint8_t *src) {
    hipLaunchKernelGGL(or_byte_kernel, dim3(1), dim3(64), 0, st, dst, src);
    const hipError_t e_ = hipGetLastError();
    return e_ != hipSuccess ? (int)e_ : 0;
}
__global__ void trailer_kernel(int format, uint32_t isize, uint64_t out_base_bit,
                               EncodeResult *__restrict__ res, uint32_t *__restrict__ out) {
    if (threadIdx.x != 0 || res->status != 0) return;
    const uint64_t at = (res->end_bit - out_base_bit + 7) >> 3;
    uint8_t t[8];
    uint32_t nt = 0;
    if (format == 2) {
        const uint32_t c = res->crc32;
        t[0] = c; t[1] = c >> 8; t[2] = c >> 16; t[3] = c >> 24;
        t[4] = isize; t[5] = isize >> 8; t[6] = isize >> 16; t[7] = isize >> 24;
        nt = 8;
    } else if (format == 1) {
        const uint32_t a = res->adler32;
        t[0] = a >> 24; t[1] = a >> 16; t[2] = a >> 8; t[3] = a;
        nt = 4;
    }
    for (uint32_t i = 0; i < nt; ++i) {
        const uint64_t ob = at + i;
        atomicOr(&out[ob >> 2], (uint32_t)t[i] << (8 * (ob & 3)));
    }
    res->out_bytes = at + nt;
}

#define LFX_LAUNCH_CHECK()                          \
    do {                                            \
        hipError_t e_ = hipGetLastError();          \
        if (e_ != hipSuccess) return (int)e_;       \
    } while (0)

int launch_match(hipStream_t st, const uint8_t *in, uint64_t in_bytes, const ChunkDesc *chunks,
                 const SegDesc *segs, uint32_t nsegs, uint32_t window, uint32_t max_len, uint32_t *md, uint64_t *dbg) {
    if (nsegs == 0) return 0;
    const size_t lds = MATCH_LDS;
    static bool attr_set[64] = {};
    int dev_ = 0;
    (void)hipGetDevice(&dev_);
    if (!attr_set[dev_ & 63]) {
        (void)hipFuncSetAttribute((const void *)lz77_match_kernel, hipFuncAttributeMaxDynamicSharedMemorySize, (int)lds);
        attr_set[dev_ & 63] = true;
    }
    hipLaunchKernelGGL(lz77_match_kernel, dim3(nsegs), dim3(MATCH_THREADS), lds, st, in, in_bytes,
                       chunks, segs, window, max_len, md, dbg);
    LFX_LAUNCH_CHECK();
    return 0;
}
int launch_chunk_maps(hipStream_t st, const ChunkDesc *chunks, uint32_t nchunks, uint64_t ntiles, uint32_t nsegs,
                      uint32_t *tile_map, uint32_t *seg_map, ZeroSpan z0, ZeroSpan z1, ZeroSpan z2) {
    if (nchunks == 0) {
        for (const ZeroSpan &z : {z0, z1, z2})
            if (z.n && hipMemsetAsync(z.p, 0, 4ull * z.n, st) != hipSuccess) return (int)hipGetLastError();
        return 0;
    }
    uint32_t split = nchunks >= 256 ? 1 : 256 / nchunks + 1;
    if (split > 64) split = 64;
    hipLaunchKernelGGL(chunk_maps_kernel, dim3(nchunks, split), dim3(256), 0, st, chunks, nchunks, ntiles, nsegs, tile_map, seg_map, z0, z1, z2);
    LFX_LAUNCH_CHECK();
    return 0;
}
int launch_histogram(hipStream_t st, const ChunkDesc *chunks, uint32_t nchunks, uint32_t split,
                     const uint32_t *codes, const uint32_t *ncodes, uint32_t *hist) {
    if (nchunks == 0) return 0;
    hipLaunchKernelGGL(histogram_kernel, dim3(nchunks, split), dim3(256), 0, st, chunks, codes, ncodes, hist);
    LFX_LAUNCH_CHECK();
    return 0;
}
int launch_huffman(hipStream_t st, const BlockDesc *blocks, uint32_t nblocks, const uint32_t *hist,
                   BlockCodes *bc, uint64_t *dbg) {
    if (nblocks == 0) return 0;
    hipLaunchKernelGGL(huffman_kernel, dim3(nblocks), dim3(HUFF_THREADS), 0, st, blocks, hist, bc, dbg);
    LFX_LAUNCH_CHECK();
    return 0;
}
int launch_offsets(hipStream_t st, const BlockDesc *blocks, uint32_t nblocks, const BlockCodes *bc,
                   uint64_t start_bit, uint64_t cap_bits, uint64_t *block_start, EncodeResult *res) {
    hipLaunchKernelGGL(offsets_kernel, dim3(1), dim3(256), 0, st, blocks, nblocks, bc, start_bit,
                       cap_bits, block_start, res);
    LFX_LAUNCH_CHECK();
    return 0;
}
int launch_offsets_batch(hipStream_t st, const BatchStream *streams, uint32_t count, const BlockDesc *blocks, const BlockCodes *bc,
                         uint32_t hdr_len, uint32_t trailer_len, uint64_t *block_start, uint64_t *stream_end, int32_t *status,
                         EncodeResult *res) {
    if (!count) return 0;
    hipLaunchKernelGGL(offsets_batch_kernel, dim3((count + 255) / 256), dim3(256), 0, st, streams, count, blocks, bc, hdr_len,
                       trailer_len, block_start, stream_end, status, res);
    LFX_LAUNCH_CHECK();
    return 0;
}
int launch_frame_batch(hipStream_t st, int format, const BatchStream *streams, uint32_t count, const uint8_t *hdr, uint32_t hdr_len,
                       const uint64_t *stream_end, const uint32_t *crc, const uint32_t *adler, const EncodeResult *res, uint32_t *out,
                       uint64_t *out_len) {
    if (!count) return 0;
    hipLaunchKernelGGL(frame_batch_kernel, dim3((count + 255) / 256), dim3(256), 0, st, format, streams, count, hdr, hdr_len,
                       stream_end, crc, adler, res, out, out_len);
    LFX_LAUNCH_CHECK();
    return 0;
}
int launch_pack(hipStream_t st, const uint8_t *in, uint64_t in_bytes, const ChunkDesc *chunks,
                uint32_t nchunks, const BlockDesc *blocks, uint32_t nblocks, uint64_t ntiles,
                const uint32_t *codes, const uint32_t *ncodes, const BlockCodes *bc,
                const uint64_t *block_start, uint32_t *tile_bits, uint64_t *tile_start,
                const EncodeResult *res, uint64_t out_base_bit, uint32_t *out, const uint32_t *tile_map) {
    if (ntiles) {
        const uint32_t ngroups = (uint32_t)div_up(ntiles, PACK_TPW);
        hipLaunchKernelGGL(tile_bits_kernel, dim3(ngroups), dim3(PACK_THREADS), 0, st, chunks,
                           nchunks, blocks, codes, ncodes, bc, tile_bits, tile_map, ntiles);
        LFX_LAUNCH_CHECK();
        hipLaunchKernelGGL(tile_scan_kernel, dim3(nblocks), dim3(ntiles / (nblocks ? nblocks : 1) > 2048 ? 1024 : 256), 0, st, chunks, blocks, bc,
                           block_start, tile_bits, ntiles, nchunks, tile_start);
        LFX_LAUNCH_CHECK();
        hipLaunchKernelGGL(pack_kernel, dim3(ngroups), dim3(PACK_THREADS), 0, st, chunks,
                           nchunks, blocks, codes, ncodes, bc, tile_start, res, out_base_bit, out, tile_map, ntiles);
        LFX_LAUNCH_CHECK();
    }
    if (nblocks) {
        hipLaunchKernelGGL(block_header_kernel, dim3(nblocks), dim3(256), 0, st, in, in_bytes, blocks,
                           bc, block_start, res, out_base_bit, out);
        LFX_LAUNCH_CHECK();
    }
    return 0;
}
int launch_checksum_part(hipStream_t st, const uint8_t *in, uint64_t n, uint32_t *crc_part, uint32_t *a_part, uint32_t *b_part,
                         EncodeResult *res, int mode, uint32_t part, uint32_t nparts) {
    const uint32_t span = ck_span(n);
    const uint64_t nspans = div_up(n, span);
    const uint64_t ngroups = div_up(nspans, 4);
    const uint64_t g0 = ngroups * part / nparts, g1 = ngroups * (part + 1) / nparts;
    if (g1 > g0) {
        const dim3 grid((uint32_t)(g1 - g0));
        if (mode == 1) hipLaunchKernelGGL(checksum_span_kernel<1>, grid, dim3(256), 0, st, in, n, span, crc_part, a_part, b_part, 4 * g0);
        else if (mode == 2) hipLaunchKernelGGL(checksum_span_kernel<2>, grid, dim3(256), 0, st, in, n, span, crc_part, a_part, b_part, 4 * g0);
        else hipLaunchKernelGGL(checksum_span_kernel<3>, grid, dim3(256), 0, st, in, n, span, crc_part, a_part, b_part, 4 * g0);
        LFX_LAUNCH_CHECK();
    }
    if (part + 1 == nparts) {
        hipLaunchKernelGGL(checksum_combine_kernel, dim3(1), dim3(1024), 0, st, crc_part, a_part, b_part, n, span, res);
        LFX_LAUNCH_CHECK();
    }
    return 0;
}
int launch_checksum(hipStream_t st, const uint8_t *in, uint64_t n, uint32_t *crc_part,
                    uint32_t *a_part, uint32_t *b_part, EncodeResult *res, int mode) {
    return launch_checksum_part(st, in, n, crc_part, a_part, b_part, res, mode, 0, 1);
}
int launch_checksum_ranges(hipStream_t st, const uint8_t *data, uint32_t count, const uint64_t *off,
                           uint32_t off_stride, const uint64_t *len, uint32_t len_stride, uint32_t *crc, uint32_t *adler) {
    if (!count) return 0;
    hipLaunchKernelGGL(checksum_ranges_kernel, dim3((count + 3) / 4), dim3(256), 0, st, data, count, off, off_stride, len,
                       len_stride, crc, adler);
    LFX_LAUNCH_CHECK();
    return 0;
}
int launch_put_bytes(hipStream_t st, const uint8_t *d_bytes, uint32_t n, uint64_t at_byte, uint32_t *out) {
    if (n == 0) return 0;
    hipLaunchKernelGGL(put_bytes_kernel, dim3(1), dim3(256), 0, st, d_bytes, n, at_byte, out);
    LFX_LAUNCH_CHECK();
    return 0;
}
int launch_trailer(hipStream_t st, int format, uint32_t isize, uint64_t out_base_bit,
                   EncodeResult *res, uint32_t *out) {
    hipLaunchKernelGGL(trailer_kernel, dim3(1), dim3(64), 0, st, format, isize, out_base_bit, res, out);
    LFX_LAUNCH_CHECK();
    return 0;
}

}
```

libflate_amd/csrc/lfx_inflate_fast.hip:

```cpp
#include <hip/hip_runtime.h>
#include <stdint.h>
#include <stdlib.h>

#include <type_traits>

#include "lfx_common.h"
#include "lfx_decode.h"

namespace lfx {

__constant__ uint16_t f_len_base[29] = {3,  4,  5,  6,  7,  8,  9,  10, 11,  13,  15,  17,  19,  23, 27,
                                        31, 35, 43, 51, 59, 67, 83, 99, 115, 131, 163, 195, 227, 258};
__constant__ uint8_t f_len_extra[29] = {0, 0, 0, 0, 0, 0, 0, 0, 1, 1, 1, 1, 2, 2, 2,
                                        2, 3, 3, 3, 3, 4, 4, 4, 4, 5, 5, 5, 5, 0};
__constant__ uint16_t f_dist_base[30] = {1,    2,    3,    4,    5,    7,    9,    13,    17,    25,
                                         33,   49,   65,   97,   129,  193,  257,  385,   513,   769,
                                         1025, 1537, 2049, 3073, 4097, 6145, 8193, 12289, 16385, 24577};
__constant__ uint8_t f_dist_extra[30] = {0, 0, 0, 0, 1, 1, 2, 2,  3,  3,  4,  4,  5,  5,  6,
                                         6, 7, 7, 8, 8, 9, 9, 10, 10, 11, 11, 12, 12, 13, 13};
__constant__ uint8_t f_clen_order[19] = {16, 17, 18, 0, 8, 7, 9, 6, 10, 5, 11, 4, 12, 3, 13, 2, 14, 1, 15};
constexpr uint32_t f_clen_order_c(uint32_t k) {
    constexpr uint8_t o[19] = {16, 17, 18, 0, 8, 7, 9, 6, 10, 5, 11, 4, 12, 3, 13, 2, 14, 1, 15};
    return o[k];
}
__device__ __forceinline__ uint32_t clen_order(uint32_t k) {
    const uint64_t lo = 16ull | 17ull << 5 | 18ull << 10 | 0ull << 15 | 8ull << 20 | 7ull << 25 | 9ull << 30 | 6ull << 35 |
                        10ull << 40 | 5ull << 45 | 11ull << 50 | 4ull << 55;
    const uint64_t hi = 12ull | 3ull << 5 | 13ull << 10 | 2ull << 15 | 14ull << 20 | 1ull << 25 | 15ull << 30;
    return k < 12 ? (uint32_t)(lo >> (5 * k)) & 31 : (uint32_t)(hi >> (5 * (k - 12))) & 31;
}

constexpr uint32_t K_LIT = 0, K_LEN = 1, K_EOB = 2, K_LONG = 3;
constexpr uint32_t E_LONG = (K_LONG << 4);

struct LaneBits {
    gptr_u32 w;
    uint64_t wlast;
    uint64_t widx;
    uint64_t pos;
    uint64_t buf;
    uint32_t nb;
    uint32_t c0, c1, c2, c3, cn;
    uint32_t n0, n1, n2, n3;
    __device__ __forceinline__ uint32_t ld(uint64_t i) const { return w[i < wlast ? i : wlast]; }
    __device__ __forceinline__ void init(const uint8_t *base, uint64_t nbytes, uint64_t bitpos) {
        const uint64_t a = (uint64_t)base;
        w = (gptr_u32)(a & ~3ull);
        const uint64_t sh = (a & 3) * 8;
        wlast = ((a & 3) + nbytes + 3) / 4;
        wlast = wlast ? wlast - 1 : 0;
        const uint64_t abs = bitpos + sh;
        widx = abs >> 5;
        const uint32_t off = (uint32_t)abs & 31;
        c0 = ld(widx); c1 = ld(widx + 1); c2 = ld(widx + 2); c3 = ld(widx + 3);
        n0 = ld(widx + 4); n1 = ld(widx + 5); n2 = ld(widx + 6); n3 = ld(widx + 7);
        widx += 8;
        buf = (uint64_t)(c0 >> off);
        nb = 32 - off;
        c0 = c1; c1 = c2; c2 = c3; cn = 3;
        pos = bitpos;
    }
    __device__ __forceinline__ void refill() {
        if (nb <= 32) {
            buf |= (uint64_t)c0 << nb;
            nb += 32;
            c0 = c1; c1 = c2; c2 = c3;
            if (--cn == 0) {
                c0 = n0; c1 = n1; c2 = n2; c3 = n3; cn = 4;
                n0 = ld(widx); n1 = ld(widx + 1); n2 = ld(widx + 2); n3 = ld(widx + 3);
                widx += 4;
            }
        }
    }
    __device__ __forceinline__ void skip(uint32_t k) { buf >>= k; nb -= k; pos += k; }
};

constexpr uint32_t LIT_BITS = 12, DIST_BITS = 10;
struct FastTabs {
    uint32_t lit[1u << LIT_BITS];
    uint32_t dist[1u << DIST_BITS];
    uint32_t lit_info[288];
    uint32_t dist_info[32];
    uint16_t lit_sorted[288];
    uint16_t dist_sorted[32];
    uint16_t lit_count[16];
    uint16_t dist_count[16];
};

__device__ __forceinline__ uint32_t long_decode(const uint16_t *count, const uint16_t *sorted, uint64_t bits,
                                                uint32_t &width) {
    uint32_t code = 0, first = 0, index = 0;
    for (uint32_t w = 1; w <= 15; ++w) {
        code |= (uint32_t)(bits >> (w - 1)) & 1;
        const uint32_t cnt = count[w];
        if (code < first + cnt) { width = w; return sorted[index + (code - first)]; }
        index += cnt;
        first = (first + cnt) << 1;
        code <<= 1;
    }
    width = 0;
    return 0xFFFF;
}

__device__ __forceinline__ uint32_t lit_entry_of(uint32_t s, uint32_t w) {
    if (s < 256) return w | (K_LIT << 4) | (s << 16);
    if (s == 256) return w | (K_EOB << 4);
    if (s < 286) return w | (K_LEN << 4) | ((uint32_t)f_len_extra[s - 257] << 6) | ((uint32_t)f_len_base[s - 257] << 16);
    return 0;
}
__device__ __forceinline__ uint32_t dist_entry_of(uint32_t s, uint32_t w) {
    if (s >= 30) return 0;
    return w | ((uint32_t)f_dist_extra[s] << 6) | ((uint32_t)f_dist_base[s] << 16);
}

__device__ __forceinline__ uint32_t short_decode(const uint16_t *count, const uint16_t *sorted, uint32_t bits,
                                                 uint32_t maxw, uint32_t &width) {
    uint32_t code = 0, first = 0, index = 0;
    for (uint32_t w = 1; w <= maxw; ++w) {
        code |= (bits >> (w - 1)) & 1;
        const uint32_t cnt = count[w];
        if (code < first + cnt) { width = w; return sorted[index + (code - first)]; }
        index += cnt;
        first = (first + cnt) << 1;
        code <<= 1;
    }
    width = 0;
    return 0xFFFF;
}

__device__ bool build_fast(FastTabs &T, const uint8_t *lw, uint32_t nl, const uint8_t *dw, uint32_t nd,
                           uint32_t tid, uint32_t nthreads) {
    __shared__ uint32_t s_cnt[2][16], s_off[2][16], s_bad, s_long[2];
    if (tid < 32) s_cnt[tid >> 4][tid & 15] = 0;
    for (uint32_t i = tid; i < 288; i += nthreads) T.lit_info[i] = lit_entry_of(i, 0);
    for (uint32_t i = tid; i < 32; i += nthreads) T.dist_info[i] = dist_entry_of(i, 0);
    __syncthreads();
    for (uint32_t s = tid; s < nl + nd; s += nthreads) {
        const uint32_t t = s >= nl;
        const uint32_t w = t ? dw[s - nl] : lw[s];
        if (w) atomicAdd(&s_cnt[t][w], 1u);
    }
    __syncthreads();
    if (tid < 2) {
        const uint32_t t = tid;
        uint16_t *cnt = t ? T.dist_count : T.lit_count;
        const uint32_t pri = t ? DIST_BITS : LIT_BITS;
        uint32_t off = 0, nlong = 0;
        int left = 1;
        bool bad = false;
        cnt[0] = 0;
        for (uint32_t w = 1; w <= 15; ++w) {
            const uint32_t c = s_cnt[t][w];
            cnt[w] = (uint16_t)c;
            s_off[t][w] = off;
            left = (left << 1) - (int)c;
            if (left < 0) bad = true;
            off += c;
            if (w > pri) nlong += c;
        }
        s_long[t] = nlong;
// ... 1002 lines not shown
    if (lane == 0) s_wmin[wave] = sfx;
    __syncthreads();
    int64_t later = __shfl_down(sfx, 1);
    if (lane == 63) later = INT64_MAX;
    for (uint32_t w = wave + 1; w < NT / 64; ++w) { const int64_t y = s_wmin[w]; if (y < later) later = y; }
    if (cut_code != 0xFFFFFFFFu && later < (int64_t)cut_pos) cut_code = 0xFFFFFFFFu;
    __shared__ uint32_t s_cut_code[NT];
    __shared__ uint64_t s_cut_pos[NT];
    s_cut_code[tid] = cut_code;
    s_cut_pos[tid] = cut_pos;
    __shared__ uint64_t s_legal[NT / 64];
    const uint64_t legal = __ballot(cut_code != 0xFFFFFFFFu);
    if (lane == 0) s_legal[wave] = legal;
    __syncthreads();
    const uint64_t t_cut = clock64();
    if (tid == 0) {
        uint32_t nu = 0, last = 0;
        uint32_t want_units = (job.n_codes + unit_target / 2) / unit_target;
        if (want_units < 1) want_units = 1;
        if (want_units > MAX_UNITS) want_units = MAX_UNITS;
        const uint32_t tol = job.n_codes / (2 * want_units);
        U->code0[0] = 0; U->out0[0] = 0;
        for (uint32_t b = 1; b < want_units; ++b) {
            const uint32_t ideal = (uint32_t)((uint64_t)job.n_codes * b / want_units);
            uint32_t l0 = (uint32_t)((uint64_t)job.nlanes * b / want_units);
            if (l0 >= NT) l0 = NT - 1;
            int up = -1, dn = -1;
            for (uint32_t w = l0 >> 6; w < NT / 64 && up < 0; ++w) {
                uint64_t m = s_legal[w];
                if (w == (l0 >> 6)) m &= ~0ull << (l0 & 63);
                if (m) up = (int)(w * 64 + (uint32_t)__builtin_ctzll(m));
            }
            for (int w = (int)(l0 >> 6); w >= 0 && dn < 0; --w) {
                uint64_t m = s_legal[w];
                if (w == (int)(l0 >> 6)) m &= (l0 & 63) ? ~0ull >> (64 - (l0 & 63)) : 0ull;
                if (m) dn = w * 64 + 63 - __builtin_clzll(m);
            }
            int pick = -1;
            uint32_t best = 0xFFFFFFFFu;
            if (up >= 0) { const uint32_t cc = s_cut_code[up]; const uint32_t d = cc > ideal ? cc - ideal : ideal - cc; if (d < best) { best = d; pick = up; } }
            if (dn >= 0) { const uint32_t cc = s_cut_code[dn]; const uint32_t d = cc > ideal ? cc - ideal : ideal - cc; if (d < best) { best = d; pick = dn; } }
            if (pick < 0 || best > tol) continue;
            const uint32_t cc = s_cut_code[pick];
            if (cc == 0 || cc <= last || cc >= job.n_codes) continue;
            nu++;
            U->code0[nu] = cc; U->out0[nu] = s_cut_pos[pick];
            last = cc;
        }
        nu++;
        U->code0[nu] = job.n_codes; U->out0[nu] = job.n_out;
        U->n = nu;
        uint32_t fn = 0;
        uint32_t fwant = (uint32_t)(job.n_out >> free_shift);
        fwant = fwant < 1 ? 1 : fwant > MAX_FREE_UNITS ? MAX_FREE_UNITS : fwant;
        U->fcode0[0] = 0; U->fout0[0] = 0;
        for (uint32_t b = 1; b < fwant; ++b) {
            const uint32_t l = (uint32_t)((uint64_t)job.nlanes * b / fwant);
            if (l == 0 || l >= job.nlanes) continue;
            const uint32_t cc = L->code_off[l];
            if (cc <= U->fcode0[fn] || cc >= job.n_codes) continue;
            fn++;
            U->fcode0[fn] = cc; U->fout0[fn] = L->out_off[l];
        }
        fn++;
        U->fcode0[fn] = job.n_codes; U->fout0[fn] = job.n_out;
        U->fn = fn;
        U->cyc[0] = (uint32_t)(t_hdr - t_begin); U->cyc[1] = (uint32_t)(t_dec - t_hdr);
        U->cyc[2] = (uint32_t)(t_cut - t_dec); U->cyc[3] = (uint32_t)(clock64() - t_cut);
    }
}

__device__ __forceinline__ void blk_flag_reach(uint32_t tid, int64_t reach, uint64_t hist, uint32_t *__restrict__ flags,
                                               uint32_t *__restrict__ job_flags) {
    __shared__ uint32_t s_fl;
    if (tid == 0) s_fl = 0;
    __syncthreads();
    if (reach < -(int64_t)hist) atomicOr(&s_fl, 1u);
    else if (reach < 0) atomicOr(&s_fl, 2u);
    __syncthreads();
    if (tid == 0 && s_fl) {
        const uint32_t f = s_fl;
        if ((f & 1u) && job_flags) job_flags[blockIdx.x] = 1u;
        if ((__atomic_load_n(&flags[0], __ATOMIC_RELAXED) & f) != f) atomicOr(&flags[0], f);
    }
}

template <bool RING, int NT = SCAN_THREADS>
__global__ __launch_bounds__(NT, RING ? 4 : 8) void blk_emit_kernel(const uint8_t *__restrict__ in, uint64_t nbytes,
                                                                const BlkEmit *__restrict__ jobs,
                                                                const BlkLanes *__restrict__ lanes,
                                                                uint32_t *__restrict__ codes,
                                                                uint32_t *__restrict__ flags,
                                                                BlkUnits *__restrict__ units, uint32_t unit_target, uint32_t free_shift,
                                                                uint32_t *__restrict__ job_flags,
                                                                const FastTabs *__restrict__ tabs) {
    __shared__ FastTabs T;
    __shared__ __attribute__((aligned(4))) uint8_t lens[640];
    __shared__ uint32_t hdr[8];
    __shared__ uint64_t hdr64[2];
    extern __shared__ uint32_t emit_stage[];
    __shared__ uint32_t s_ring[RING ? NT * RING_STRIDE : 1];
    const uint32_t tid = threadIdx.x;
    const BlkEmit job = jobs[blockIdx.x];
    BlkUnits *U = &units[blockIdx.x];
    if (job.placed) return;
    if (job.btype == 0) {
        if (tid == 0) {
            U->n = 1; U->code0[0] = 0; U->code0[1] = 0; U->out0[0] = 0; U->out0[1] = job.n_out;
            U->fn = 1; U->fcode0[0] = 0; U->fcode0[1] = 0; U->fout0[0] = 0; U->fout0[1] = job.n_out;
        }
        return;
    }
    const uint64_t t_begin = clock64();
    if (tabs) {
        const uint32_t *srcw = (const uint32_t *)&tabs[job.cand];
        uint32_t *dst = (uint32_t *)&T;
        constexpr uint32_t TW = sizeof(FastTabs) / 4, TPER = (TW + NT - 1) / NT;
        uint32_t tv[TPER];
#pragma unroll
        for (uint32_t k = 0; k < TPER; ++k) tv[k] = srcw[min(tid + k * NT, TW - 1)];
#pragma unroll
        for (uint32_t k = 0; k < TPER; ++k) if (tid + k * NT < TW) dst[tid + k * NT] = tv[k];
        __syncthreads();
    } else parse_header<NT>(in, nbytes, job.start_bit, T, lens, hdr, hdr64, tid);
    const uint64_t t_hdr = clock64();
    const BlkLanes *L = &lanes[job.cand];
    int64_t reach = INT64_MAX;
    uint32_t cut_code = 0xFFFFFFFFu;
    uint64_t cut_pos = 0;
    if (tid < job.nlanes) {
        const uint64_t st = L->start[tid];
        const uint64_t lim = tid + 1 < job.nlanes ? L->start[tid + 1] : (job.end_limit ? job.end_limit : ~0ull >> 1);
        uint32_t nc = 0, cc = 0, co = 0;
        const uint64_t out0 = L->out_off[tid];
        uint64_t no = out0, endpos;
        if (RING)
            lane_decode<true>(T, in, nbytes, st, lim, nc, no, codes + job.code_off + L->code_off[tid], reach, endpos, cc, co,
                              s_ring + tid * RING_STRIDE, emit_stage + tid * EMIT_STRIDE);
        else
            lane_decode_fifo<true>(T, in, nbytes, st, lim, nc, no, codes + job.code_off + L->code_off[tid], reach, endpos, cc, co,
                                   emit_stage + tid * EMIT_STRIDE);
        if (cc < nc) { cut_code = L->code_off[tid] + cc; cut_pos = out0 + co; }
    }
    blk_flag_reach(tid, reach, job.hist, flags, job_flags);
    blk_units_tail<NT>(tid, job, L, reach, cut_code, cut_pos, U, unit_target, free_shift, t_begin, t_hdr);
}



__global__ __launch_bounds__(SCAN_THREADS) void blk_place_kernel(const BlkEmit *__restrict__ jobs, const BlkLanes *__restrict__ lanes,
                                                                  const BlkLanesX *__restrict__ lanesx, const uint32_t *__restrict__ temp,
                                                                  uint32_t *__restrict__ codes, uint32_t *__restrict__ flags,
                                                                  BlkUnits *__restrict__ units, uint32_t unit_target, uint32_t free_shift,
                                                                  uint32_t *__restrict__ job_flags) {
    const uint32_t tid = threadIdx.x, lane = tid & 63;
    const BlkEmit job = jobs[blockIdx.x];
    if (!job.placed) return;
    const uint64_t t_begin = clock64();
    BlkUnits *U = &units[blockIdx.x];
    const BlkLanes *L = &lanes[job.cand];
    const BlkLanesX *X = &lanesx[job.cand];
    const bool live = tid < job.nlanes;
    const uint32_t my_head = live ? X->n_head[tid] : 0u, my_rest = live ? X->n_rest[tid] : 0u, my_at = X->rest_at[tid];
    const uint32_t my_off = L->code_off[tid];
    const uint32_t *src0 = temp + job.temp_off + (uint64_t)(tid & ~63u) * job.cap;
    uint32_t *dst0 = codes + job.code_off;
    constexpr uint32_t DEEP = 8;
    const uint32_t j0 = blockIdx.y * 32u;
    for (uint32_t j = j0; j < j0 + 32u; j += 2) {
        uint32_t nh[2], n[2], at[2];
        const uint32_t *src[2];
        uint32_t *dst[2];
#pragma unroll
        for (uint32_t q = 0; q < 2; ++q) {
            nh[q] = (uint32_t)__shfl((int)my_head, (int)(j + q));
            n[q] = nh[q] + (uint32_t)__shfl((int)my_rest, (int)(j + q));
            at[q] = (uint32_t)__shfl((int)my_at, (int)(j + q));
            src[q] = src0 + (uint64_t)(j + q) * job.cap;
            dst[q] = dst0 + (uint32_t)__shfl((int)my_off, (int)(j + q));
        }
        const uint32_t nmax = n[0] > n[1] ? n[0] : n[1];
        for (uint32_t base = 0; base < nmax; base += 64 * DEEP) {
            uint32_t v[2][DEEP];
#pragma unroll
            for (uint32_t q = 0; q < 2; ++q)
#pragma unroll
                for (uint32_t k = 0; k < DEEP; ++k) {
                    const uint32_t i = base + k * 64 + lane;
                    const uint32_t si = i < nh[q] ? i : at[q] + (i - nh[q]);
                    v[q][k] = i < n[q] ? src[q][si] : 0u;
                }
#pragma unroll
            for (uint32_t q = 0; q < 2; ++q)
#pragma unroll
                for (uint32_t k = 0; k < DEEP; ++k) {
                    const uint32_t i = base + k * 64 + lane;
                    if (i < n[q]) dst[q][i] = v[q][k];
                }
        }
    }
    if (blockIdx.y != 0) return;
    const uint64_t t_hdr = clock64();
    int64_t reach = INT64_MAX;
    uint32_t cut_code = 0xFFFFFFFFu;
    uint64_t cut_pos = 0;
    if (live) {
        const uint64_t out0 = L->out_off[tid];
        const int32_t rr = X->reach[tid];
        if (rr != INT32_MAX) reach = (int64_t)out0 + (int64_t)rr;
        const uint32_t cc = X->cut_code[tid];
        if (cc != 0xFFFFFFFFu) { cut_code = my_off + cc; cut_pos = out0 + X->cut_out[tid]; }
    }
    blk_flag_reach(tid, reach, job.hist, flags, job_flags);
    blk_units_tail(tid, job, L, reach, cut_code, cut_pos, U, unit_target, free_shift, t_begin, t_hdr);
}

template <uint32_t THREADS>
struct M2 {
    static constexpr uint32_t WAVES = THREADS / 64;
    static constexpr uint32_t NC = 2 * THREADS;
    static constexpr uint32_t TILE = 4 * THREADS;
    static constexpr uint32_t RING = 32768 + TILE;
    static constexpr uint32_t PASSES = (TILE + 4 * THREADS - 1) / (4 * THREADS);
    static_assert(RING % 4 == 0 && TILE >= 258 && TILE < 0xFFFFu && RING + 64 < 65536, "tile");
};
constexpr uint32_t M2_THREADS = 256;
constexpr uint32_t M2_WIDE_THREADS = 1024;
constexpr uint32_t M2_FEW_JOBS = 4;
constexpr uint32_t M2_SYM_THREADS = 256;
constexpr uint32_t M2_DONE = 0xFFFFu;
#ifndef LFX_M2_PRIO_TILES
#define LFX_M2_PRIO_TILES 8
#endif
constexpr uint32_t M2_PRIO_TILES = LFX_M2_PRIO_TILES;

template <uint32_t RING> __device__ __forceinline__ uint32_t m2_wrap(uint32_t x) { return min(x, x - RING); }
template <uint32_t RING> __device__ __forceinline__ uint32_t m2_back(uint32_t idx, uint32_t d) {
    const uint32_t a = idx - d;
    return min(a, a + RING);
}

template <bool SYM, uint32_t THREADS>
struct M2Lds {
    using elem_t = typename std::conditional<SYM, uint16_t, uint8_t>::type;
    using G = M2<THREADS>;
    static constexpr uint32_t RING_BYTES = ((G::RING + 64) * (uint32_t)sizeof(elem_t) + 15u) & ~15u;
    static constexpr uint32_t P_BYTES = G::PASSES * 4 * THREADS * 2;
    static constexpr uint32_t XC_BYTES = (G::NC + 4) * 8;
    static constexpr uint32_t SW_BYTES = 2 * G::WAVES * 4;
    static constexpr uint32_t BYTES = RING_BYTES + P_BYTES + XC_BYTES + SW_BYTES;
};
template <bool SYM, uint32_t THREADS, bool DYN = false>
__device__ __forceinline__ void materialize2_body(const uint8_t *__restrict__ in, const BlkEmit *__restrict__ jobs,
                                                  const BlkUnits *__restrict__ units,
                                                  const uint32_t *__restrict__ codes,
                                                  typename std::conditional<SYM, uint16_t, uint8_t>::type *__restrict__ out,
                                                  uint32_t njobs, uint64_t *__restrict__ dbg) {
    using elem_t = typename std::conditional<SYM, uint16_t, uint8_t>::type;
    using G = M2<THREADS>;
    using LD = M2Lds<SYM, THREADS>;
    constexpr uint32_t WAVES = G::WAVES, TILE = G::TILE, RING = G::RING, PASSES = G::PASSES, NC = G::NC;
    constexpr uint32_t EPD = 4 / sizeof(elem_t);
    elem_t *ring;
    uint16_t *P;
    uint2 *XC;
    uint32_t *s_w;
    if constexpr (DYN) {
        extern __shared__ __attribute__((aligned(16))) uint8_t m2_dyn[];
        ring = (elem_t *)m2_dyn;
        P = (uint16_t *)(m2_dyn + LD::RING_BYTES);
        XC = (uint2 *)(m2_dyn + LD::RING_BYTES + LD::P_BYTES);
        s_w = (uint32_t *)(m2_dyn + LD::RING_BYTES + LD::P_BYTES + LD::XC_BYTES);
    } else {
        __shared__ __attribute__((aligned(16))) elem_t ring_s[RING + 64];
        __shared__ __attribute__((aligned(8))) uint16_t P_s[PASSES * 4 * THREADS];
        __shared__ __attribute__((aligned(16))) uint2 XC_s[G::NC + 4];
        __shared__ uint32_t s_w_s[2 * WAVES];
        ring = ring_s; P = P_s; XC = XC_s; s_w = s_w_s;
    }
    const uint32_t bidx = blockIdx.x % njobs, u = blockIdx.x / njobs;
    const BlkEmit job = jobs[bidx];
    const uint32_t tid = threadIdx.x, lane = tid & 63, wave = tid >> 6;
    if (job.btype == 0) {
        if (u != 0) return;
        elem_t *o = out + job.out_off;
        const uint8_t *src = in + (job.data_bit >> 3);
        for (uint64_t k = tid; k < job.n_out; k += THREADS) o[k] = src[k];
        return;
    }
    const BlkUnits *U = &units[bidx];
    if (u >= (SYM ? U->fn : U->n)) return;
    const uint32_t c0 = SYM ? U->fcode0[u] : U->code0[u], c1 = SYM ? U->fcode0[u + 1] : U->code0[u + 1];
    const uint64_t ob = SYM ? U->fout0[u] : U->out0[u];
    const uint64_t gbase = job.out_off + ob;
    elem_t *o = out + gbase;
    const uint32_t *cp = codes + job.code_off + c0;
    const uint32_t n = c1 - c0;
    const uint32_t hist = SYM ? 32768u : (u == 0 && job.preload) ? (uint32_t)(job.hist < 32768 ? job.hist : 32768) : 0;
    const uint32_t shift = (uint32_t)((gbase - hist) & (EPD - 1)) + hist;
    for (uint32_t k = tid; k < hist; k += THREADS)
        ring[shift - hist + k] = SYM ? (elem_t)(256 + k) : (elem_t)o[(int64_t)k - (int64_t)hist];
    if (tid < 4) XC[NC + tid] = make_uint2(0xFFFFFFFFu, 0u);
    uint64_t produced = 0, flushed = 0;
    uint32_t tr = shift;
    uint32_t fr = shift;
    uint32_t base = 0, ntiles = 0, nrounds = 0;
    uint32_t cw0 = 2 * tid < n ? cp[2 * tid] : 0u, cw1 = 2 * tid + 1 < n ? cp[2 * tid + 1] : 0u;
    const uint64_t t0 = dbg ? clock64() : 0;
    while (base < n) {
        if ((ntiles & (M2_PRIO_TILES - 1)) == 0) {
            switch (((ntiles / M2_PRIO_TILES) + u) & 3u) {
            case 0: __builtin_amdgcn_s_setprio(0); break;
            case 1: __builtin_amdgcn_s_setprio(1); break;
            case 2: __builtin_amdgcn_s_setprio(2); break;
            default: __builtin_amdgcn_s_setprio(3); break;
            }
        }
        ntiles++;
        const uint32_t i = base + 2 * tid;
        const uint32_t len0 = i < n ? ((cw0 & 0xFFFFu) ? cw0 >> 16 : 1u) : 0u;
        const uint32_t len1 = i + 1 < n ? ((cw1 & 0xFFFFu) ? cw1 >> 16 : 1u) : 0u;
        uint32_t x = wave_inclusive_sum(len0 + len1);
        if (lane == 63) s_w[wave] = x;
        __syncthreads();
        uint32_t tot = 0, cum[WAVES];
#pragma unroll
        for (uint32_t j = 0; j < WAVES; ++j) {
            const uint32_t wj = s_w[j];
            x += j < wave ? wj : 0u;
            tot += wj;
            cum[j] = tot;
        }
        *(uint4 *)&XC[2 * tid] = make_uint4(x - len1, cw0, x, cw1);
        if (tot > TILE) {
            const uint32_t cnt = (uint32_t)__popcll(__ballot(x - len1 <= TILE)) + (uint32_t)__popcll(__ballot(x <= TILE));
            if (lane == 0) s_w[WAVES + wave] = cnt;
        }
        __syncthreads();
        uint32_t take = NC, total = tot;
        if (tot > TILE) {
            take = 0;
#pragma unroll
            for (uint32_t j = 0; j < WAVES; ++j) take += s_w[WAVES + j];
            total = XC[take - 1].x;
        }
        const uint32_t j0 = 2 * tid + take, j1 = j0 + 1;
        const uint32_t rf0 = (j0 >= NC && base + j0 < n) ? cp[base + j0] : 0u;
        const uint32_t rf1 = (j1 >= NC && base + j1 < n) ? cp[base + j1] : 0u;
        uint32_t pp[PASSES][4];
        bool pend = false;
        auto round0 = [&](auto periodic_tag) {
        constexpr bool PERIODIC = decltype(periodic_tag)::value;
#pragma unroll
        for (uint32_t ps = 0; ps < PASSES; ++ps) {
            const uint32_t b = ps * 4 * THREADS + 4 * tid;
#pragma unroll
            for (uint32_t q = 0; q < 4; ++q) pp[ps][q] = M2_DONE;
            if (ps == 0 || __ballot(b < total)) {
                uint32_t k = 0;
#pragma unroll
                for (uint32_t j = 0; j + 1 < WAVES; ++j) k += cum[j] <= b ? 128u : 0u;
#pragma unroll
                for (uint32_t step = 64; step; step >>= 1) k += XC[k + step - 1].x <= b ? step : 0u;
                uint32_t src[4], dst[4], cwq[4];
                bool lit[4], fin[4];
#pragma unroll
                for (uint32_t q = 0; q < 4; ++q) {
                    const uint32_t bi = b + q;
                    if (q) k += bi >= cwq[q - 1] ? 1u : 0u;
                    const uint2 xc = XC[k];
                    const uint32_t d = xc.y & 0xFFFFu;
                    const uint32_t t = m2_wrap<RING>(tr + bi);
                    const bool in = bi < total;
                    lit[q] = d == 0;
                    uint32_t tgt = bi, tt = t;
                    if constexpr (PERIODIC) {
                        const uint32_t s0 = xc.x - (xc.y >> 16);
                        const uint32_t off = bi - s0;
                        if (d != 0 && off >= d) {
                            uint32_t r = off - d * (uint32_t)((float)off * __builtin_amdgcn_rcpf((float)d));
                            r = r >= d ? r - d : r;
// ... 558 lines not shown
        val = run ? val : 0u;
        adv = run ? adv : 0u;
        o += adv;
        const bool pass = o >= 32;
        cur = pass ? nxt : cur;
        nxt = pass ? ahead : nxt;
        di += pass ? 1u : 0u;
        o &= 31u;
        const uint32_t nlit_part = have < nl ? min(rep, nl - have) : 0u;
        const uint32_t ndist_part = rep - nlit_part;
        const uint32_t wgt = val ? 32768u >> val : 0u;
        kl += __umul24(nlit_part, wgt);
        kd += __umul24(ndist_part, wgt);
        nlit += val ? nlit_part : 0u;
        ndist += val ? ndist_part : 0u;
        eob_len = (val && have <= 256 && 256 < have + rep) ? val : eob_len;
        bad |= kl > 32768u || kd > 32768u;
        bad |= have + rep >= nl && have < nl && !(kl == 32768u || (nlit == 1 && kl == 16384u));
        have += rep;
        last = val;
        good = good && !bad;
        run = good && have < total;
    }
    if (good) {
        if (eob_len == 0) good = false;
        if (!(kl == 32768u || (nlit == 1 && kl == 16384u))) good = false;
        if (!(kd == 32768u || (ndist == 1 && kd == 16384u) || ndist == 0)) good = false;
        if (((gd + di - 2) << 5) + o > nbytes * 8 + (a & 3) * 8) good = false;
    }
    if (dbg && lane == 0) {
        const uint64_t t3 = clock64();
        atomicAdd((unsigned long long *)&dbg[0], (unsigned long long)(t1 - t0));
        atomicAdd((unsigned long long *)&dbg[1], (unsigned long long)(t2 - t1));
        atomicAdd((unsigned long long *)&dbg[2], (unsigned long long)(t3 - t2));
        atomicAdd((unsigned long long *)&dbg[3], (unsigned long long)steps);
        atomicAdd((unsigned long long *)&dbg[4], (unsigned long long)restaged);
        atomicAdd((unsigned long long *)&dbg[5], 1ull);
    }
    return good;
}

template <int EXP>
__global__ __launch_bounds__(64) void find_blocks_stage2(const uint8_t *__restrict__ in, uint64_t nbytes,
                                                         const uint64_t *__restrict__ cand, uint32_t shard_cap,
                                                         const uint32_t *__restrict__ count, uint32_t *__restrict__ work,
                                                         uint32_t *__restrict__ final_count,
                                                         uint64_t *__restrict__ final_list, uint32_t final_cap,
                                                         uint64_t *__restrict__ dbg) {
    __shared__ uint8_t cl_tab[128 * 64];
    __shared__ uint32_t hbuf[FIND2_HB * 64];
    const uint64_t tk0 = dbg ? clock64() : 0;
    __shared__ uint32_t s_pre[FIND_SHARDS + 1];
    {
        constexpr uint32_t PER = FIND_SHARDS / 64;
        static_assert(PER * 64 == FIND_SHARDS, "lists per lane");
        uint32_t cnt[PER], sum = 0;
#pragma unroll
        for (uint32_t q = 0; q < PER; ++q) { cnt[q] = min(count[threadIdx.x * PER + q], shard_cap); sum += cnt[q]; }
        const uint32_t incl = wave_inclusive_sum(sum);
        uint32_t at = incl - sum;
#pragma unroll
        for (uint32_t q = 0; q < PER; ++q) { s_pre[threadIdx.x * PER + q] = at; at += cnt[q]; }
        if (threadIdx.x == 63) s_pre[FIND_SHARDS] = incl;
    }
    __syncthreads();
    const uint32_t n1 = s_pre[FIND_SHARDS];
    const uint32_t grp = blockIdx.x % FIND2_GROUPS, members = (gridDim.x - grp + FIND2_GROUPS - 1) / FIND2_GROUPS;
    uint32_t *my_work = work + grp * FIND_HDR_WORK_STRIDE;
    uint32_t base = (grp + FIND2_GROUPS * (blockIdx.x / FIND2_GROUPS)) * 64u;
    while (base < n1) {
        uint32_t next_raw = 0;
        const uint32_t gi = base + threadIdx.x;
        const bool valid = gi < n1;
        uint32_t shard = 0;
#pragma unroll
        for (uint32_t step = FIND_SHARDS / 2; step; step >>= 1) shard += s_pre[shard + step] <= gi ? step : 0u;
        const uint64_t i = (uint64_t)shard * shard_cap + (gi - s_pre[shard]);
        const uint64_t cand_bit = valid ? cand[i] : 0;
        const bool good = stage2_check_staged<EXP>(in, nbytes, cand_bit, valid, cl_tab, hbuf, dbg, my_work, next_raw);
        if (good) {
            const uint32_t slot = atomicAdd(final_count, 1u);
            if (slot < final_cap) final_list[slot] = cand_bit;
        }
        __syncthreads();
        if (EXP == 4) base += gridDim.x * 64u;
        else base = (grp + FIND2_GROUPS * (members + (uint32_t)__builtin_amdgcn_readfirstlane((int)next_raw))) * 64u;
    }
    if (dbg && threadIdx.x == 0) atomicAdd((unsigned long long *)&dbg[6], (unsigned long long)(clock64() - tk0));
}

__global__ __launch_bounds__(M2_SYM_THREADS) void blk_materialize2_sym_kernel(const uint8_t *__restrict__ in,
                                                                          const BlkEmit *__restrict__ jobs,
                                                                          const BlkUnits *__restrict__ units,
                                                                          const uint32_t *__restrict__ codes,
                                                                          uint16_t *__restrict__ sym, uint32_t njobs) {
    materialize2_body<true, M2_SYM_THREADS>(in, jobs, units, codes, sym, njobs, nullptr);
}
__global__ __launch_bounds__(M2_WIDE_THREADS) void blk_materialize2_sym_wide_kernel(const uint8_t *__restrict__ in,
                                                                                const BlkEmit *__restrict__ jobs,
                                                                                const BlkUnits *__restrict__ units,
                                                                                const uint32_t *__restrict__ codes,
                                                                                uint16_t *__restrict__ sym, uint32_t njobs) {
    materialize2_body<true, M2_WIDE_THREADS, true>(in, jobs, units, codes, sym, njobs, nullptr);
}

#define LFX_LAUNCH_CHECK()                          \
    do {                                            \
        hipError_t e_ = hipGetLastError();          \
        if (e_ != hipSuccess) return (int)e_;       \
    } while (0)

size_t blk_tabs_bytes() { return sizeof(FastTabs); }
constexpr int SCAN_SMALL = 256;
int launch_blk_scan(hipStream_t st, const uint8_t *in, uint64_t nbytes, const BlkJob *jobs, uint32_t njobs,
                    BlkInfo *infos, BlkLanes *lanes, void *tabs, bool small_blocks) {
    if (!njobs) return 0;
    if (small_blocks)
        hipLaunchKernelGGL((blk_scan_kernel<false, SCAN_SMALL>), dim3(njobs), dim3(SCAN_SMALL), 0, st, in, nbytes, jobs, infos, lanes,
                           (FastTabs *)tabs, (uint32_t *)nullptr, (BlkLanesX *)nullptr);
    else
        hipLaunchKernelGGL((blk_scan_kernel<false, SCAN_THREADS>), dim3(njobs), dim3(SCAN_THREADS), 0, st, in, nbytes, jobs, infos, lanes,
                           (FastTabs *)tabs, (uint32_t *)nullptr, (BlkLanesX *)nullptr);
    LFX_LAUNCH_CHECK();
    return 0;
}
int launch_blk_walk_size(hipStream_t st, const uint8_t *in, uint64_t nbytes, const WalkJob *jobs, uint32_t njobs,
                         WalkResult *results, bool small_blocks) {
    if (!njobs) return 0;
    if (small_blocks)
        hipLaunchKernelGGL((blk_walk_size_kernel<SCAN_SMALL>), dim3(njobs), dim3(SCAN_SMALL), 0, st, in, nbytes, jobs, results);
    else
        hipLaunchKernelGGL((blk_walk_size_kernel<SCAN_THREADS>), dim3(njobs), dim3(SCAN_THREADS), 0, st, in, nbytes, jobs, results);
    LFX_LAUNCH_CHECK();
    return 0;
}
int launch_blk_scan_store(hipStream_t st, const uint8_t *in, uint64_t nbytes, const BlkJob *jobs, uint32_t njobs,
                          BlkInfo *infos, BlkLanes *lanes, void *tabs, uint32_t *temp, BlkLanesX *lanesx) {
    if (!njobs) return 0;
    constexpr size_t stage_bytes = (size_t)SCAN_THREADS * EMIT_STRIDE * 4;
    static bool attr_set[64] = {};
    int dev_ = 0;
    (void)hipGetDevice(&dev_);
    if (!attr_set[dev_ & 63]) {
        (void)hipFuncSetAttribute((const void *)blk_scan_kernel<true, SCAN_THREADS>, hipFuncAttributeMaxDynamicSharedMemorySize, (int)stage_bytes);
        attr_set[dev_ & 63] = true;
    }
    hipLaunchKernelGGL((blk_scan_kernel<true, SCAN_THREADS>), dim3(njobs), dim3(SCAN_THREADS), stage_bytes, st, in, nbytes, jobs, infos, lanes,
                       (FastTabs *)tabs, temp, lanesx);
    LFX_LAUNCH_CHECK();
    return 0;
}
int launch_blk_place(hipStream_t st, const BlkEmit *jobs, uint32_t njobs, const BlkLanes *lanes, const BlkLanesX *lanesx,
                     const uint32_t *temp, uint32_t *codes, uint32_t *flags, BlkUnits *units, uint32_t unit_target, uint32_t *job_flags,
                     uint32_t free_shift) {
    if (!njobs) return 0;
    hipLaunchKernelGGL(blk_place_kernel, dim3(njobs, 2), dim3(SCAN_THREADS), 0, st, jobs, lanes, lanesx, temp, codes, flags, units,
                       unit_target ? unit_target : 1u, free_shift < 15 ? 15u : free_shift, job_flags);
    LFX_LAUNCH_CHECK();
    return 0;
}
int launch_blk_emit(hipStream_t st, const uint8_t *in, uint64_t nbytes, const BlkEmit *jobs, uint32_t njobs,
                    const BlkLanes *lanes, uint32_t *codes, uint32_t *flags, BlkUnits *units, uint32_t unit_target,
                    uint32_t *job_flags, const void *tabs, uint32_t free_shift, bool large_blocks, bool small_blocks) {
    if (!njobs) return 0;
    constexpr size_t stage_bytes = (size_t)SCAN_THREADS * EMIT_STRIDE * 4, stage_small = (size_t)SCAN_SMALL * EMIT_STRIDE * 4;
    static bool attr_set[64] = {};
    int dev_ = 0;
    (void)hipGetDevice(&dev_);
    if (!attr_set[dev_ & 63]) {
        (void)hipFuncSetAttribute((const void *)blk_emit_kernel<false, SCAN_THREADS>, hipFuncAttributeMaxDynamicSharedMemorySize, (int)stage_bytes);
        (void)hipFuncSetAttribute((const void *)blk_emit_kernel<true, SCAN_THREADS>, hipFuncAttributeMaxDynamicSharedMemorySize, (int)stage_bytes);
        attr_set[dev_ & 63] = true;
    }
    const uint32_t ut = unit_target ? unit_target : 1u, fs = free_shift < 15 ? 15u : free_shift;
    if (small_blocks)
        hipLaunchKernelGGL((blk_emit_kernel<false, SCAN_SMALL>), dim3(njobs), dim3(SCAN_SMALL), stage_small, st, in, nbytes, jobs, lanes, codes,
                           flags, units, ut, fs, job_flags, (const FastTabs *)tabs);
    else if (large_blocks)
        hipLaunchKernelGGL((blk_emit_kernel<true, SCAN_THREADS>), dim3(njobs), dim3(SCAN_THREADS), stage_bytes, st, in, nbytes, jobs, lanes,
                           codes, flags, units, ut, fs, job_flags, (const FastTabs *)tabs);
    else
        hipLaunchKernelGGL((blk_emit_kernel<false, SCAN_THREADS>), dim3(njobs), dim3(SCAN_THREADS), stage_bytes, st, in, nbytes, jobs, lanes, codes,
                           flags, units, ut, fs, job_flags, (const FastTabs *)tabs);
    LFX_LAUNCH_CHECK();
    return 0;
}
int launch_blk_materialize(hipStream_t st, const uint8_t *in, const BlkEmit *jobs, uint32_t njobs,
                           const BlkLanes *lanes, const BlkUnits *units, const uint32_t *codes, uint8_t *out,
                           uint64_t *dbg) {
    if (!njobs) return 0;
    if (njobs <= M2_FEW_JOBS)
        hipLaunchKernelGGL(blk_materialize2_kernel<M2_WIDE_THREADS>, dim3(njobs * MAX_UNITS), dim3(M2_WIDE_THREADS), 0, st, in, jobs, units, codes, out, njobs, dbg);
    else
        hipLaunchKernelGGL(blk_materialize2_kernel<M2_THREADS>, dim3(njobs * MAX_UNITS), dim3(M2_THREADS), 0, st, in, jobs, units, codes, out, njobs, dbg);
    LFX_LAUNCH_CHECK();
    return 0;
}
int launch_blk_materialize_sym(hipStream_t st, const uint8_t *in, const BlkEmit *jobs, uint32_t njobs,
                               const BlkUnits *units, const uint32_t *codes, uint16_t *sym, bool few_units) {
    if (!njobs) return 0;
    if (few_units) {
        constexpr int lds = (int)M2Lds<true, M2_WIDE_THREADS>::BYTES;
        static bool attr_set[64] = {};
        int dev_ = 0;
        (void)hipGetDevice(&dev_);
        if (!attr_set[dev_ & 63]) {
            (void)hipFuncSetAttribute((const void *)blk_materialize2_sym_wide_kernel, hipFuncAttributeMaxDynamicSharedMemorySize, lds);
            attr_set[dev_ & 63] = true;
        }
        hipLaunchKernelGGL(blk_materialize2_sym_wide_kernel, dim3(njobs * MAX_FREE_UNITS), dim3(M2_WIDE_THREADS), lds, st, in, jobs, units, codes, sym, njobs);
    } else
        hipLaunchKernelGGL(blk_materialize2_sym_kernel, dim3(njobs * MAX_FREE_UNITS), dim3(M2_SYM_THREADS), 0, st, in, jobs, units, codes, sym, njobs);
    LFX_LAUNCH_CHECK();
    return 0;
}
int launch_window_chain(hipStream_t st, const uint16_t *sym, const SymUnit *units, uint32_t nunits, uint8_t *windows,
                        const uint8_t *init_win) {
    if (!nunits) return 0;
    static bool attr_set[64] = {};
    int dev_ = 0;
    (void)hipGetDevice(&dev_);
    if (!attr_set[dev_ & 63]) {
        (void)hipFuncSetAttribute((const void *)window_chain_kernel, hipFuncAttributeMaxDynamicSharedMemorySize, 65536);
        attr_set[dev_ & 63] = true;
    }
    hipLaunchKernelGGL(window_chain_kernel, dim3(1), dim3(1024), 65536, st, sym, units, nunits, windows, init_win);
    LFX_LAUNCH_CHECK();
    return 0;
}
size_t window_prefix_scratch_bytes(uint32_t nunits) {
    const uint32_t g = wc_group(nunits);
    return (size_t)nunits * 65536 + (size_t)((nunits + g - 1) / g) * 32768;
}
int launch_window_prefix(hipStream_t st, const uint16_t *sym, const SymUnit *units, uint32_t nunits, void *scratch,
                         uint8_t *windows, const uint8_t *init_win) {
    if (!nunits) return 0;
    static bool attr_set[64] = {};
    int dev_ = 0;
    (void)hipGetDevice(&dev_);
    if (!attr_set[dev_ & 63]) {
        (void)hipFuncSetAttribute((const void *)window_compose_kernel, hipFuncAttributeMaxDynamicSharedMemorySize, 131072);
        (void)hipFuncSetAttribute((const void *)window_groups_kernel, hipFuncAttributeMaxDynamicSharedMemorySize, 65536);
        attr_set[dev_ & 63] = true;
    }
    uint16_t *maps = (uint16_t *)scratch;
    uint8_t *gwin = (uint8_t *)scratch + (size_t)nunits * 65536;
    const uint32_t G = wc_group(nunits);
    const uint32_t ngroups = (nunits + G - 1) / G;
    hipLaunchKernelGGL(window_compose_kernel, dim3(ngroups), dim3(1024), 131072, st, sym, units, nunits, maps, G);
    LFX_LAUNCH_CHECK();
    hipLaunchKernelGGL(window_groups_kernel, dim3(1), dim3(1024), 65536, st, maps, nunits, gwin, init_win, G);
    LFX_LAUNCH_CHECK();
    hipLaunchKernelGGL(window_apply_kernel, dim3(nunits), dim3(1024), 0, st, maps, gwin, windows, init_win, G);
    LFX_LAUNCH_CHECK();
    return 0;
}
int launch_window_rank_map(hipStream_t st, const uint16_t *sym, const SymUnit *units, uint32_t nunits, void *scratch, uint16_t *out_map) {
    static bool attr_set[64] = {};
    int dev_ = 0;
    (void)hipGetDevice(&dev_);
    if (!attr_set[dev_ & 63]) {
        (void)hipFuncSetAttribute((const void *)window_compose_kernel, hipFuncAttributeMaxDynamicSharedMemorySize, 131072);
        (void)hipFuncSetAttribute((const void *)window_rank_map_kernel, hipFuncAttributeMaxDynamicSharedMemorySize, 131072);
        attr_set[dev_ & 63] = true;
    }
    uint16_t *maps = (uint16_t *)scratch;
    const uint32_t G = wc_group(nunits);
    const uint32_t ngroups = (nunits + G - 1) / G;
    if (nunits) {
        hipLaunchKernelGGL(window_compose_kernel, dim3(ngroups), dim3(1024), 131072, st, sym, units, nunits, maps, G);
        LFX_LAUNCH_CHECK();
    }
    hipLaunchKernelGGL(window_rank_map_kernel, dim3(1), dim3(1024), 131072, st, maps, nunits, out_map, G);
    LFX_LAUNCH_CHECK();
    return 0;
}
int launch_bytes_to_map(hipStream_t st, const uint8_t *out, uint64_t len, uint16_t *map) {
    hipLaunchKernelGGL(bytes_to_map_kernel, dim3(128), dim3(256), 0, st, out, len, map);
    LFX_LAUNCH_CHECK();
    return 0;
}
int launch_window_ranks(hipStream_t st, const uint16_t *maps, uint32_t nranks, uint8_t *win) {
    static bool attr_set[64] = {};
    int dev_ = 0;
    (void)hipGetDevice(&dev_);
    if (!attr_set[dev_ & 63]) {
        (void)hipFuncSetAttribute((const void *)window_ranks_kernel, hipFuncAttributeMaxDynamicSharedMemorySize, 65536);
        attr_set[dev_ & 63] = true;
    }
    hipLaunchKernelGGL(window_ranks_kernel, dim3(1), dim3(1024), 65536, st, maps, nranks, win);
    LFX_LAUNCH_CHECK();
    return 0;
}
int launch_sym_substitute(hipStream_t st, const uint16_t *sym, const SymUnit *units, uint32_t nunits,
                          const uint8_t *windows, uint8_t *out, uint64_t max_len, const uint8_t *init_win) {
    if (!nunits) return 0;
    const uint32_t gy = (uint32_t)((max_len + 16383) / 16384);
    hipLaunchKernelGGL(sym_substitute_kernel, dim3(nunits, gy ? gy : 1), dim3(256), 0, st, sym, units, windows, out, init_win);
    LFX_LAUNCH_CHECK();
    return 0;
}
int launch_find_stage2(hipStream_t st, const uint8_t *in, uint64_t nbytes, const uint64_t *cand,
                       uint32_t shard_cap, const uint32_t *count, uint32_t *work, uint32_t *final_count, uint64_t *final_list,
                       uint32_t final_cap, uint32_t n_cu, uint64_t *dbg, int exp) {
    static int per_cu_dev[64] = {};
    int dev_ = 0;
    (void)hipGetDevice(&dev_);
    int &per_cu = per_cu_dev[dev_ & 63];
    if (per_cu == 0) {
        int nb = 0;
// ... 18 lines not shown
```

libflate_amd/csrc/lfx_member.cpp:

```cpp
#include "lfx_decode_int.h"

#include <algorithm>
#include <cstdio>
#include <cstring>

#include "lfx_index.h"

namespace lfx {

std::string format_error(uint32_t err, uint32_t a0, uint32_t a1) {
    char m[200];
    switch (err) {
        case ERR_EOF: return "failed to fill whole buffer";
        case ERR_HUFF: return "Invalid huffman coded stream";
        case ERR_CONFLICT: snprintf(m, sizeof m, "Bit region conflict: symbol=%u", a0); return m;
        case ERR_HDIST: snprintf(m, sizeof m, "The value of HDIST is too big: max=30, actual=%u", a0); return m;
        case ERR_NO_PREV: return "No preceding value";
        case ERR_DIST_LIST:
            snprintf(m, sizeof m, "The length of `distance_code_bitwidthes` is too large: actual=%u, expected=%u", a0, a1);
            return m;
        case ERR_286: snprintf(m, sizeof m, "The value %u must not occur in compressed data", a0); return m;
        case ERR_BACKREF: snprintf(m, sizeof m, "Too long backword reference: buffer.len=%u, distance=%u", a0, a1); return m;
        case ERR_BTYPE3: return "btype 0x11 of DEFLATE is reserved(error) value";
        case ERR_LEN_NLEN: snprintf(m, sizeof m, "LEN=%u is not the one's complement of NLEN=%u", a0, a1); return m;
// ... 197 lines not shown
    Ctx *c = m.c;
    FindBufs fb;
    int rc;
    const uint64_t final_from = c->diag.no_final_cand ? ~0ull >> 1 : find_final_from(m.n, m.comp);
    if ((rc = find_launch(c, m.d_in, m.n, m.off0, final_from, fb))) return rc;
    c->phase("find1");
    if ((rc = find_collect(c, m.d_in, m.n, fb, fd))) return rc;
    starts.clear();
    starts.push_back(m.first_bit);
    if (fd.overflow) return LFX_OK;
    c->phase("find2");
    for (uint64_t b : fd.cand) if (b != m.first_bit) starts.push_back(b);
    std::sort(starts.begin(), starts.end());
    return LFX_OK;
}

int scan_pieces(const Member &m, const std::vector<BlkJob> &jobs, uint32_t slot0, std::vector<BlkInfo> &infos) {
    Ctx *c = m.c;
    hipStream_t st = c->stream;
    const uint32_t nj = (uint32_t)jobs.size();
    infos.resize(nj);
    HIP_TRY(hipMemcpyAsync((BlkJob *)c->d_dec_streams.p + slot0, jobs.data(), sizeof(BlkJob) * nj, hipMemcpyHostToDevice, st));
    LAUNCH_TRY(launch_blk_scan(st, m.d_in, m.n, (const BlkJob *)c->d_dec_streams.p + slot0, nj, (BlkInfo *)c->d_dec_state.p + slot0,
                               (BlkLanes *)c->d_dec_blocks.p + slot0, (uint8_t *)c->d_dec_tabs.p + blk_tabs_bytes() * slot0));
    HIP_TRY(hipMemcpyAsync(infos.data(), (BlkInfo *)c->d_dec_state.p + slot0, sizeof(BlkInfo) * nj, hipMemcpyDeviceToHost, st));
    HIP_TRY(hipStreamSynchronize(st));
    return LFX_OK;
}
int reserve_scan_slots(Ctx *c, size_t nslots) {
    int rc;
    if ((rc = c->d_dec_streams.reserve(sizeof(BlkJob) * nslots))) return rc;
    if ((rc = c->d_dec_state.reserve(sizeof(BlkInfo) * nslots))) return rc;
    if ((rc = c->d_dec_blocks.reserve(sizeof(BlkLanes) * nslots))) return rc;
    return c->d_dec_tabs.reserve(blk_tabs_bytes() * nslots);
}

int pieces_over_ranges(const Member &m, const std::vector<uint64_t> &starts, Chain &ch) {
    Ctx *c = m.c;
    const uint32_t nc = (uint32_t)starts.size();
    const uint64_t end_bits = m.end_bits();
    auto start_at = [&](uint32_t i) { return i < nc ? starts[i] : end_bits; };
    const uint64_t ptarget = (uint64_t)std::max<int64_t>(2ll * std::max(c->n_cu, 1) - (int64_t)nc, (int64_t)nc);
    const uint64_t PIECE_BITS = piece_bits(end_bits - m.first_bit, ptarget), OVERLAP = piece_overlap(PIECE_BITS);
    std::vector<BlkJob> pj;
    std::vector<uint32_t> first_piece(nc + 1, 0);
    for (uint32_t i = 0; i < nc; i++) {
        first_piece[i] = (uint32_t)pj.size();
        add_pieces(pj, starts[i], start_at(i + 1), PIECE_BITS, OVERLAP);
    }
    first_piece[nc] = (uint32_t)pj.size();
    const uint32_t npj = (uint32_t)pj.size();
    ch.units_per_piece = npj >= (uint32_t)std::max(c->n_cu, 1);
    constexpr uint32_t REPAIRS = 2;
    const uint32_t repair_slots = REPAIRS * (2 * (uint32_t)((end_bits - m.first_bit) / nc / PIECE_BITS + 2) + 4);
    const uint32_t nslots = npj + repair_slots;
    int rc;
    if ((rc = reserve_scan_slots(c, nslots))) return rc;
    std::vector<BlkInfo> pi;
    if ((rc = scan_pieces(m, pj, 0, pi))) return rc;
    bool fail = false;
    auto walk_range = [&](const BlkInfo *infos, uint32_t cnt, uint32_t slot0) -> int {
        uint64_t prev_end = 0;
        for (uint32_t q = 0; q < cnt; q++) {
            const BlkInfo &r = infos[q];
            if (r.status == BLK_BAD || r.btype == 0 || (q && r.data_bit != prev_end) || r.end_bit <= ch.pos || r.end_bit > end_bits) return 2;
            ch.push(r, slot0 + q, m.hist);
            prev_end = r.end_bit;
            if (r.status == BLK_OK) {
                ch.pieces_multi |= q > 0;
                ch.close_block(r);
                return 0;
            }
        }
        return 1;
    };
    uint32_t repairs = 0, rslot = npj;
    for (uint32_t i = 0; i < nc && !fail && !ch.ok; i++) {
        if (starts[i] != ch.pos) { fail = true; break; }
        const size_t emit_mark = ch.emit.size();
        const uint64_t total_mark = ch.total, codes_mark = ch.total_codes;
        int res = walk_range(&pi[first_piece[i]], first_piece[i + 1] - first_piece[i], first_piece[i]);
        if (res == 1 && i + 1 < nc && repairs < REPAIRS) {
            ch.emit.resize(emit_mark); ch.total = total_mark; ch.total_codes = codes_mark;
            std::vector<BlkJob> rj;
            add_pieces(rj, starts[i], start_at(i + 2), PIECE_BITS, OVERLAP);
            const uint32_t nr = (uint32_t)rj.size();
            if (rslot + nr > nslots) { fail = true; break; }
            std::vector<BlkInfo> ri;
            if ((rc = scan_pieces(m, rj, rslot, ri))) return rc;
            res = walk_range(ri.data(), nr, rslot);
            if (c->diag.debug) fprintf(stderr, "[lfx]  pieces: candidate %u (bit %llu) is a false one, its block scanned again in %u pieces: %d\n", i + 1,
                                       (unsigned long long)starts[i + 1], nr, res);
            rslot += nr;
            repairs++;
            i++;
        }
        if (res != 0) fail = true;
    }
    if (c->diag.debug) fprintf(stderr, "[lfx]  pieces over %u candidate ranges: ok=%d fail=%d pieces=%zu of %u total=%llu\n", nc, (int)ch.ok, (int)fail,
                               ch.emit.size(), npj, (unsigned long long)ch.total);
    if (fail || !ch.ok) ch = Chain(m.first_bit);
    else ch.pieces = true;
    c->phase("pieces");
    return LFX_OK;
}

int pieces_block_walk(const Member &m, bool small_first, std::vector<uint64_t> &starts, Found &fd, Chain &ch) {
    Ctx *c = m.c;
    const uint64_t end_bits = m.end_bits();
    const uint64_t PIECE_BITS = piece_bits(end_bits - m.first_bit, 2ull * (uint64_t)std::max(c->n_cu, 1)), OVERLAP = piece_overlap(PIECE_BITS);
    const uint32_t cap_slots = (uint32_t)std::min<uint64_t>((end_bits - m.first_bit) / PIECE_BITS * 2 + 64, 1u << 20);
    int rc;
    if ((rc = reserve_scan_slots(c, cap_slots))) return rc;
    uint32_t base = 0;
    bool fail = false;
    for (uint32_t iter = 0; iter < (small_first ? 4u : 64u) && !fail && !ch.ok; iter++) {
        std::vector<BlkJob> pj;
        add_fixed_pieces(pj, ch.pos, end_bits, PIECE_BITS, OVERLAP);
        const uint32_t np = (uint32_t)pj.size();
        if (np == 0 || base + np > cap_slots) { fail = true; break; }
        std::vector<BlkInfo> pi;
        if ((rc = scan_pieces(m, pj, base, pi))) return rc;
        uint32_t used = 0;
        bool closed = false;
        uint64_t prev_end = 0;
        for (uint32_t q = 0; q < np && !closed; q++) {
            const BlkInfo &r = pi[q];
            if (c->diag.debug && (q < 3 || r.status != BLK_NO_EOB))
                fprintf(stderr, "[lfx]   piece %u/%u: status=%u btype=%u data=%llu end=%llu prev_end=%llu lanes=%u codes=%u out=%llu rounds=%u cyc_hdr=%u cyc_total=%u\n", q, np,
                        r.status, r.btype, (unsigned long long)r.data_bit, (unsigned long long)r.end_bit,
                        (unsigned long long)prev_end, r.nlanes, r.n_codes, (unsigned long long)r.n_out, r.rounds, r.cyc_hdr, r.cyc_total);
            if (r.status == BLK_BAD || (q && r.data_bit != prev_end) || r.end_bit <= ch.pos || r.end_bit > end_bits) { fail = true; break; }
            if (q == 0 && r.btype == 0 && r.status != BLK_OK) { fail = true; break; }
            ch.push(r, base + q, m.hist);
            used = q + 1;
            prev_end = r.end_bit;
            if (r.status == BLK_OK) {
                closed = true;
                ch.pieces_multi |= q > 0;
                ch.close_block(r);
            }
        }
        if (!closed) fail = true;
        base += used;
    }
    if (c->diag.debug) fprintf(stderr, "[lfx]  pieces: ok=%d fail=%d pieces=%zu total=%llu\n", (int)ch.ok, (int)fail, ch.emit.size(), (unsigned long long)ch.total);
    if (fail || !ch.ok) ch = Chain(m.first_bit);
    else ch.pieces = true;
    c->phase("pieces");
    if (small_first && !ch.pieces) return find_starts(m, starts, fd);
    return LFX_OK;
}

int block_scan(const Member &m, const std::vector<uint64_t> &starts, uint32_t n1, Chain &ch, MemberResult &mr) {
    Ctx *c = m.c;
    hipStream_t st = c->stream;
    const uint8_t *d_in = m.d_in;
    const uint64_t n = m.n;
    const uint32_t nc = (uint32_t)starts.size();
    const size_t tab_bytes = blk_tabs_bytes();
    int rc;
    std::vector<BlkJob> bj(nc);
    for (uint32_t i = 0; i < nc; i++) bj[i] = BlkJob{starts[i], i + 1 < nc ? starts[i + 1] : n * 8};
    const std::vector<int32_t> alt = add_alt_jobs(bj, starts, n * 8, m.comp);
    const uint32_t nj = (uint32_t)bj.size();
    constexpr uint32_t EXTRA = 64, MAX_ON_DEMAND = 1u << 16;
    if ((rc = c->d_dec_streams.reserve(sizeof(BlkJob) * (nj + 1)))) return rc;
    if ((rc = c->d_dec_state.reserve(sizeof(BlkInfo) * (nj + EXTRA + 1)))) return rc;
    if ((rc = c->d_dec_blocks.reserve(sizeof(BlkLanes) * (size_t)(nj + EXTRA + 1)))) return rc;
    if ((rc = c->d_dec_tabs.reserve(tab_bytes * (nj + EXTRA + 1)))) return rc;
    std::vector<uint8_t> stored(nj + EXTRA + 1, 0);
    ch.scan_small = !c->diag.no_small_scan && nj && (n * 8) / nj < (512ull << 10);
    const bool store_mode = !c->diag.two_pass && nj && (n * 8) / nj >= (1ull << 20) && plan_store(c, bj.data(), nj);
    HIP_TRY(c->small_up(c->d_dec_streams.p, bj.data(), sizeof(BlkJob) * nj, st));
    if (store_mode)
        LAUNCH_TRY(launch_blk_scan_store(st, d_in, n, (const BlkJob *)c->d_dec_streams.p, nj, (BlkInfo *)c->d_dec_state.p,
                                         (BlkLanes *)c->d_dec_blocks.p, c->d_dec_tabs.p, (uint32_t *)c->d_dec_temp.p,
                                         (BlkLanesX *)c->d_dec_lanesx.p));
    else
        LAUNCH_TRY(launch_blk_scan(st, d_in, n, (const BlkJob *)c->d_dec_streams.p, nj, (BlkInfo *)c->d_dec_state.p,
                                   (BlkLanes *)c->d_dec_blocks.p, c->d_dec_tabs.p, ch.scan_small));
    std::vector<BlkInfo> bi(nj);
    HIP_TRY(c->small_down(bi.data(), c->d_dec_state.p, sizeof(BlkInfo) * nj, st));
    HIP_TRY(c->small_sync(st));
    for (BlkInfo &b : bi) if (b.status == BLK_OK && b.end_bit > n * 8) b.status = BLK_NO_EOB;
    if (store_mode) for (uint32_t j = 0; j < nj; j++) stored[j] = bi[j].status == BLK_OK && bi[j].btype != 0 && bi[j]._pad == 0;
    c->phase("blk_scan");
    std::vector<uint32_t> slot(nc);
    for (uint32_t i = 0; i < nc; i++)
        slot[i] = (bi[i].status == BLK_NO_EOB && alt[i] >= 0 && bi[alt[i]].status == BLK_OK) ? (uint32_t)alt[i] : i;
    if (c->diag.debug) {
        fprintf(stderr, "[lfx] finder: stage1=%u candidates=%u scan jobs=%u (alternatives: %u)\n", n1, nc, nj, nj - nc);
        for (uint32_t i = 0; i < nc && i < 12; i++)
            fprintf(stderr, "[lfx]  cand %u start=%llu status=%u btype=%u final=%u end=%llu n_out=%llu n_codes=%u lanes=%u rounds=%u cyc_hdr=%u cyc_total=%u\n",
                    i, (unsigned long long)starts[i], bi[i].status, bi[i].btype, bi[i].bfinal,
                    (unsigned long long)bi[i].end_bit, (unsigned long long)bi[i].n_out, bi[i].n_codes,
                    bi[i].nlanes, bi[i].rounds, bi[i].cyc_hdr, bi[i].cyc_total);
        uint32_t nbad = 0, maxr = 0;
        for (uint32_t i = 0; i < nc; i++) { nbad += bi[i].status != BLK_OK; maxr = std::max(maxr, bi[i].rounds); }
        fprintf(stderr, "[lfx]  not-ok=%u max_rounds=%u\n", nbad, maxr);
    }
    if ((rc = rescan_widen(c, d_in, n, starts, nc, bi, slot, stored, ch.scan_small))) return rc;
    c->phase("repair");
    uint32_t n_extra = 0;
    for (;;) {
        if (ch.pos == m.stop_bit && !ch.emit.empty()) { ch.ok = true; break; }
        auto it = std::lower_bound(starts.begin(), starts.end(), ch.pos);
        uint32_t k;
        BlkInfo r;
        if (it != starts.end() && *it == ch.pos) { k = slot[(uint32_t)(it - starts.begin())]; r = bi[k]; }
        else {
            if (ch.pos >= n * 8 || ch.n_on_demand++ >= MAX_ON_DEMAND || n_extra >= EXTRA) break;
            k = nj + n_extra;
            const BlkJob one{ch.pos, it != starts.end() ? *it : n * 8};
            BlkJob *d_one = (BlkJob *)c->d_dec_streams.p + nj;
            HIP_TRY(hipMemcpyAsync(d_one, &one, sizeof one, hipMemcpyHostToDevice, st));
            LAUNCH_TRY(launch_blk_scan(st, d_in, n, d_one, 1, (BlkInfo *)c->d_dec_state.p + k,
                                       (BlkLanes *)c->d_dec_blocks.p + k, (uint8_t *)c->d_dec_tabs.p + tab_bytes * k, ch.scan_small));
            HIP_TRY(hipMemcpyAsync(&r, (BlkInfo *)c->d_dec_state.p + k, sizeof r, hipMemcpyDeviceToHost, st));
            HIP_TRY(hipStreamSynchronize(st));
            if (r.status == BLK_OK && r.btype != 0) n_extra++;
        }
        if (r.status == BLK_OK && r.end_bit > n * 8) r.status = BLK_NO_EOB;
        if (r.status != BLK_OK || r.end_bit <= ch.pos) { ch.front_bad = ch.emit.empty() && r.status == BLK_BAD; break; }
        if (m.partial && ch.total + r.n_out > m.cap) { mr.need_cap = ch.emit.empty(); break; }
        BlkEmit &e = ch.push(r, k, m.hist);
        if (k < nj && stored[k]) { e.placed = 1; e.temp_off = bj[k].temp_off; e.cap = bj[k].cap; ch.n_placed++; }
        ch.close_block(r);
        if (ch.ok) break;
    }
    if (m.partial && !ch.ok && !ch.emit.empty()) ch.ok = true;
    return LFX_OK;
}

void debug_emit_stats(Ctx *c, uint32_t ne, uint32_t fl, const uint64_t *dbgbuf) {
    fprintf(stderr, "[lfx]  emit flags=%u\n", fl);
    std::vector<BlkUnits> uv(ne);
    (void)hipMemcpy(uv.data(), c->d_hist.p, sizeof(BlkUnits) * ne, hipMemcpyDeviceToHost);
    for (uint32_t u = 0; u < 3 && u < ne; u++)
        fprintf(stderr, "[lfx]  K2 block %u: units=%u hdr=%u decode=%u cut=%u select=%u\n", u, uv[u].n, uv[u].cyc[0],
                uv[u].cyc[1], uv[u].cyc[2], uv[u].cyc[3]);
    std::vector<uint64_t> dv(64ull * ne);
    (void)hipMemcpy(dv.data(), dbgbuf, 64ull * 8 * ne, hipMemcpyDeviceToHost);
    uint32_t nunits = 0;
    uint64_t maxcyc = 0, tmin = ~0ull, tmax = 0;
    for (uint32_t u = 0; u < 8 * ne; u++) {
        if (!dv[u * 8 + 1]) continue;
        nunits++;
        maxcyc = std::max(maxcyc, dv[u * 8]);
        tmin = std::min(tmin, dv[u * 8 + 6]); tmax = std::max(tmax, dv[u * 8 + 6]);
    }
    fprintf(stderr, "[lfx]  K3: units=%u max_cycles=%llu end-time spread=%.1f us (100 MHz clock)\n", nunits,
            (unsigned long long)maxcyc, (double)(tmax - tmin) / 100.0);
    for (uint32_t u = 0; u < 8 && u < 8 * ne; u++)
        fprintf(stderr, "[lfx]  K3 unit %u: cycles=%llu batches=%llu nseq=%llu seq_cycles=%llu codes=%llu bytes=%llu\n", u,
                (unsigned long long)dv[u * 8], (unsigned long long)dv[u * 8 + 1], (unsigned long long)dv[u * 8 + 2],
                (unsigned long long)dv[u * 8 + 3], (unsigned long long)dv[u * 8 + 4], (unsigned long long)dv[u * 8 + 5]);
}

int materialise_markers(const Member &m, const Chain &ch, const BlkEmit *d_emit) {
    Ctx *c = m.c;
    hipStream_t st = c->stream;
    const uint32_t ne = (uint32_t)ch.emit.size();
    int rc;
    const uint8_t *init_win = m.hist ? m.d_out - MAX_WINDOW : nullptr;
    std::vector<BlkUnits> uv(ne);
    HIP_TRY(hipMemcpyAsync(uv.data(), c->d_hist.p, sizeof(BlkUnits) * ne, hipMemcpyDeviceToHost, st));
    HIP_TRY(hipStreamSynchronize(st));
    std::vector<SymUnit> su;
    const uint64_t max_len = sym_units(ch.emit, uv, su);
    const uint32_t nsu = (uint32_t)su.size();
    if ((rc = c->d_dec_sym.reserve(2 * std::max<uint64_t>(ch.total, 1)))) return rc;
    if ((rc = c->d_dec_win.reserve(32768ull * std::max<uint32_t>(nsu, 1) + sizeof(SymUnit) * (size_t)nsu + 64))) return rc;
    uint8_t *d_win = (uint8_t *)c->d_dec_win.p;
    SymUnit *d_su = (SymUnit *)(d_win + 32768ull * std::max<uint32_t>(nsu, 1));
    HIP_TRY(hipMemcpyAsync(d_su, su.data(), sizeof(SymUnit) * nsu, hipMemcpyHostToDevice, st));
    LAUNCH_TRY(launch_blk_materialize_sym(st, m.d_in, d_emit, ne, (const BlkUnits *)c->d_hist.p,
                                          (const uint32_t *)c->d_codes.p, (uint16_t *)c->d_dec_sym.p,
                                          nsu <= (uint32_t)std::max(c->n_cu, 1)));
    c->phase("lz77_sym");
    if (nsu >= 16) {
        if ((rc = c->d_dec_maps.reserve(window_prefix_scratch_bytes(nsu)))) return rc;
        LAUNCH_TRY(launch_window_prefix(st, (const uint16_t *)c->d_dec_sym.p, d_su, nsu, c->d_dec_maps.p, d_win, init_win));
    } else LAUNCH_TRY(launch_window_chain(st, (const uint16_t *)c->d_dec_sym.p, d_su, nsu, d_win, init_win));
    c->phase("win_chain");
    LAUNCH_TRY(launch_sym_substitute(st, (const uint16_t *)c->d_dec_sym.p, d_su, nsu, d_win, m.d_out, max_len, init_win));
    HIP_TRY(hipStreamSynchronize(st));
    c->phase("substitute");
    if (c->diag.debug) fprintf(stderr, "[lfx]  cross-block references: %u blocks, %u units through markers\n", ne, nsu);
    return LFX_OK;
}

int emit_and_materialise(const Member &m, const Chain &ch, MemberResult &mr, bool &done) {
    Ctx *c = m.c;
    hipStream_t st = c->stream;
    const uint8_t *d_in = m.d_in;
    const uint32_t ne = (uint32_t)ch.emit.size();
    const uint64_t total = ch.total;
    int rc;
    uint64_t *dbgbuf = nullptr;
    if (c->diag.debug) {
        if ((rc = c->d_ck.reserve(64ull * 8 * ne + 64))) return rc;
        dbgbuf = (uint64_t *)c->d_ck.p;
        HIP_TRY(hipMemsetAsync(dbgbuf, 0, 64ull * 8 * ne, st));
    }
    EmitBufs eb;
    const uint32_t free_shift = ch.pieces && ch.units_per_piece ? 20 : marker_unit_shift(total, c->n_cu);
    if ((rc = emit_codes(c, d_in, m.n, ch.emit, ch.total_codes, ch.n_placed, free_shift, ch.scan_small && !ch.pieces, eb))) return rc;
    bool giant = ch.pieces_multi;
    for (const BlkEmit &e : ch.emit) giant |= e.n_out >= (8ull << 20);
    const bool probe = !giant && total / ne < (256u << 10);
    uint32_t fl = 0;
    if (probe) {
        HIP_TRY(c->small_down(&fl, eb.d_flags, 4, st));
        HIP_TRY(c->small_sync(st));
    }
    const uint64_t end_bit = ch.pos == m.stop_bit ? ch.pos : ch.last_end, end_byte = end_bit / 8 + ((end_bit & 7) ? 1 : 0);
    bool ck_spec = false;
    if (!giant && !(probe && fl == 2)) {
        LAUNCH_TRY(launch_blk_materialize(st, d_in, eb.d_emit, ne, (const BlkLanes *)c->d_dec_blocks.p,
                                          (const BlkUnits *)c->d_hist.p, (const uint32_t *)c->d_codes.p, m.d_out, dbgbuf));
        if (mr.ck_mode && total && !m.partial && !c->diag.debug && end_byte + mr.trailer_len <= m.n) {
            c->phase("lz77_copy");
            const uint64_t nspans = ck_nspans(total);
            if ((rc = c->d_ck.reserve(12 * nspans))) return rc;
            if ((rc = c->d_res.reserve(256))) return rc;
            uint32_t *ck = (uint32_t *)c->d_ck.p;
            LAUNCH_TRY(launch_checksum(st, m.d_out, total, ck, ck + nspans, ck + 2 * nspans, (EncodeResult *)c->d_res.p, mr.ck_mode));
            HIP_TRY(hipMemcpyAsync(c->h_res, c->d_res.p, sizeof(EncodeResult), hipMemcpyDeviceToHost, st));
            if (mr.trailer_len) HIP_TRY(hipMemcpyAsync((uint8_t *)c->h_res + 256, d_in + end_byte, mr.trailer_len, hipMemcpyDeviceToHost, st));
            ck_spec = true;
        }
    }
    HIP_TRY(c->small_down(&fl, eb.d_flags, 4, st));
    HIP_TRY(c->small_sync(st));
    if (ck_spec && fl == 0) {
        const EncodeResult er = *(EncodeResult *)c->h_res;
        mr.ck_done = true; mr.crc32 = er.crc32; mr.adler32 = er.adler32;
        memcpy(mr.trailer, (uint8_t *)c->h_res + 256, mr.trailer_len);
        c->phase("checksum");
    }
    if (giant && !(fl & 1)) fl = 2;
    else if (giant) {
        LAUNCH_TRY(launch_blk_materialize(st, d_in, eb.d_emit, ne, (const BlkLanes *)c->d_dec_blocks.p,
                                          (const BlkUnits *)c->d_hist.p, (const uint32_t *)c->d_codes.p, m.d_out, dbgbuf));
        HIP_TRY(hipStreamSynchronize(st));
    }
    if (!ck_spec) c->phase("lz77_copy");
    if (c->diag.debug) debug_emit_stats(c, ne, fl, dbgbuf);
    if (fl == 2) {
        if ((rc = materialise_markers(m, ch, eb.d_emit))) return rc;
        fl = 0;
    }
    if (fl != 0) return LFX_OK;
    if (c->idx && (rc = idx_record_chain(c, ch.emit.data(), ne, (const BlkLanes *)c->d_dec_blocks.p, c->idx->bit_base,
                                         c->idx->out_base, true)))
        return rc;
    mr.status = LFX_OK;
    mr.out_len = total;
    mr.blk_out_start = total;
    mr.end_byte = end_byte;
    mr.end_bit = end_bit;
    mr.final_seen = ch.final;
    done = true;
    return LFX_OK;
}

int serial_walk(const Member &m, MemberResult &mr) {
    Ctx *c = m.c;
    const uint64_t n = m.n;
    InflateJob j{};
    j.in_off = 0; j.in_len = n; j.start_bit = m.first_bit;
    j.out_off = 0; j.out_cap = m.cap; j.hist_avail = m.hist; j.flags = 0;
    j.stop_bit = m.stop_bit == ~0ull ? 0 : m.stop_bit;
    std::vector<InflateResult> res;
    int rc;
    if ((rc = run_jobs(c, m.d_in, m.d_out, {j}, res))) return rc;
    c->phase("serial");
    InflateResult &r = res[0];
    if (m.stop_bit != ~0ull && r.status == 0 && (r.final_seen || r.end_bit != m.stop_bit)) {
        r.status = 1; r.err = ERR_HUFF; r.a0 = r.a1 = 0;
    }
    mr.status = map_status(r.status);
    mr.out_len = r.out_len;
    mr.blk_out_start = r.status ? r.blk_out_start : r.out_len;
    mr.end_byte = std::min<uint64_t>((r.end_bit + 7) / 8, n);
    mr.end_bit = r.end_bit;
    mr.final_seen = r.status == 0 && r.final_seen;
    mr.msg = format_error(r.err, r.a0, r.a1);
    if (m.partial && r.status != 0 && (r.status == 2 || r.status == 3 || r.end_bit + 64 >= n * 8)) {
        mr.status = LFX_OK;
        mr.out_len = mr.blk_out_start = r.blk_out_start;
        mr.end_bit = r.blk_start_bit;
        mr.end_byte = r.blk_start_bit / 8;
        mr.final_seen = false;
        mr.need_cap = r.status == 3 && r.blk_out_start == 0;
        mr.msg.clear();
    }
    return LFX_OK;
}

}

int inflate_member(Ctx *c, const uint8_t *d_in, uint64_t n, uint64_t off0, uint8_t *d_out, uint64_t cap, MemberResult &mr,
                   uint64_t start_bit0, uint64_t stop_bit, bool partial, uint64_t hist) {
    const Member m{c, d_in, n, off0, d_out, cap, start_bit0 == ~0ull ? off0 * 8 : start_bit0, stop_bit, partial, hist, n > off0 ? n - off0 : 0};
    mr.end_bit = m.first_bit;
    c->pin_reset();
    bool done = false;
    if (m.comp >= (4u << 10)) {
        int rc;
        std::vector<uint64_t> starts;
        Found fd;
        const bool may_piece = stop_bit == ~0ull && !partial && !c->diag.no_pieces;
        const bool small_first = m.comp < (1536u << 10) && may_piece;
        if (small_first) starts.push_back(m.first_bit);
        else if ((rc = find_starts(m, starts, fd))) return rc;
        if (!fd.overflow) {
            Chain ch(m.first_bit);
            const uint32_t nc = (uint32_t)starts.size();
            const bool giant_blocks = nc <= 8 && m.comp / nc >= (2u << 20);
            if (may_piece && !small_first && !giant_blocks && nc >= 2 && nc <= PIECE_RANGES_MAX && m.comp / nc >= (128u << 10) &&
                (rc = pieces_over_ranges(m, starts, ch)))
                return rc;
            if (!ch.pieces && may_piece && (small_first || giant_blocks) && (rc = pieces_block_walk(m, small_first, starts, fd, ch))) return rc;
            if (!ch.pieces && !fd.overflow && (rc = block_scan(m, starts, fd.n1, ch, mr))) return rc;
            if (c->diag.debug) fprintf(stderr, "[lfx]  chain ok=%d blocks=%zu pos=%llu total=%llu on_demand=%u\n", (int)ch.ok, ch.emit.size(), (unsigned long long)ch.pos, (unsigned long long)ch.total, ch.n_on_demand);
            if (partial && ch.emit.empty() && !ch.front_bad) {
                mr.status = LFX_OK; mr.out_len = 0; mr.blk_out_start = 0; mr.final_seen = false;
                mr.end_bit = m.first_bit; mr.end_byte = m.first_bit / 8;
                return LFX_OK;
            }
            if (ch.ok && ch.total <= cap && (rc = emit_and_materialise(m, ch, mr, done))) return rc;
        }
    }
    if (done) return LFX_OK;
    if (c->diag.no_serial) { c->set_error("serial fallback disabled (LFX_NO_SERIAL)"); return LFX_E_UNSUPPORTED; }
    return serial_walk(m, mr);
}

}
```

libflate_amd/csrc/lfx_stages.h:

```cpp
#pragma once
#include <algorithm>
#include <cstdint>
#include <vector>

#include "lfx_blk.h"

namespace lfx {

constexpr uint32_t PIECE_RANGES_MAX = 100;

inline uint64_t piece_bits(uint64_t span_bits, uint64_t want) {
    return std::min<uint64_t>(4ull << 20, std::max<uint64_t>(256ull << 10, (span_bits / want + 63) & ~63ull));
}
inline uint64_t piece_overlap(uint64_t piece) { return piece <= (1ull << 20) ? 2048 : 8192; }

inline void add_pieces(std::vector<BlkJob> &jobs, uint64_t s0, uint64_t s1, uint64_t piece, uint64_t overlap) {
    const uint64_t len = s1 - s0;
    const uint64_t np0 = std::max<uint64_t>((len + piece - 1) / piece, 1);
    const uint64_t pb = std::max<uint64_t>(((len + np0 - 1) / np0 + 63) & ~63ull, 64);
    const uint32_t np = (uint32_t)std::max<uint64_t>((len + pb - 1) / pb, 1);
    for (uint32_t q = 0; q < np; q++) {
        const uint64_t lo = s0 + q * pb;
        jobs.push_back(BlkJob{s0, std::min(lo + pb, s1), q ? lo : 0, q ? lo - overlap : 0, 1u, 0u});
    }
}
inline void add_fixed_pieces(std::vector<BlkJob> &jobs, uint64_t pos, uint64_t end_bits, uint64_t piece, uint64_t overlap) {
    const uint32_t np = (uint32_t)((end_bits - pos + piece - 1) / piece);
    for (uint32_t q = 0; q < np; q++) {
        const uint64_t lo = pos + q * piece;
        jobs.push_back(BlkJob{pos, std::min(lo + piece, end_bits), q ? lo : 0, q ? lo - overlap : 0, 1u, 0u});
    }
}

inline std::vector<int32_t> add_alt_jobs(std::vector<BlkJob> &bj, const std::vector<uint64_t> &starts, uint64_t end_bits, uint64_t comp) {
    const uint32_t nc = (uint32_t)starts.size();
    auto start_at = [&](uint32_t i) { return i < nc ? starts[i] : end_bits; };
    std::vector<int32_t> alt(nc, -1);
    std::vector<uint64_t> len(nc);
    for (uint32_t i = 0; i < nc; i++) len[i] = bj[i].end_bit - bj[i].start_bit;
    std::vector<uint64_t> sorted = len;
    std::nth_element(sorted.begin(), sorted.begin() + nc / 2, sorted.end());
    const uint64_t median = sorted[nc / 2], thresh = median / 5 * 3;
    const uint32_t max_extra = nc / 4 + 4;
    for (uint32_t i = 0; i + 1 < nc && bj.size() - nc < max_extra; i++) {
        if (len[i] >= thresh && len[i + 1] >= thresh) continue;
        if (i + 2 == nc && len[i] >= thresh) continue;
        if (len[i] + len[i + 1] > median + median / 4) continue;
        alt[i] = (int32_t)bj.size();
        bj.push_back(BlkJob{starts[i], start_at(i + 2)});
    }
    if (nc > 1 && nc <= 8 && alt[0] < 0 && comp / nc >= (2u << 20)) {
        alt[0] = (int32_t)bj.size();
        bj.push_back(BlkJob{starts[0], end_bits});
    }
    return alt;
}

inline uint64_t plan_store_regions(BlkJob *bj, uint32_t nj, bool tight) {
    uint64_t off = 0;
    for (uint32_t j = 0; j < nj; j++) {
        const uint64_t bits = bj[j].end_bit > bj[j].start_bit ? bj[j].end_bit - bj[j].start_bit : 0;
        const uint64_t slice = std::max<uint64_t>((bits + 1023) / 1024, 128);
        const uint64_t cap = (slice / (tight ? 16 : 2) + 448 + 64 + 3) & ~3ull;
        bj[j].temp_off = off;
        bj[j].cap = (uint32_t)cap;
        off += 1024 * cap;
    }
    return off;
}
inline void clear_store_regions(BlkJob *bj, uint32_t nj) {
    for (uint32_t j = 0; j < nj; j++) { bj[j].temp_off = 0; bj[j].cap = 0; }
}

inline BlkEmit blk_emit_of(const BlkInfo &r, uint64_t start_bit, uint32_t slot, uint64_t out_off, uint64_t code_off, uint64_t hist) {
    BlkEmit e{};
    e.start_bit = start_bit; e.data_bit = r.data_bit; e.code_off = code_off; e.out_off = out_off;
    e.n_out = r.n_out; e.n_codes = r.n_codes; e.nlanes = r.nlanes; e.btype = r.btype; e.cand = slot;
    e.hist = hist;
    e.end_limit = r.status == BLK_NO_EOB ? r.end_bit : 0;
    return e;
}
inline uint32_t emit_unit_target(uint64_t total_codes, int n_cu) {
    const uint64_t slots = 4ull * (uint64_t)std::max(n_cu, 1);
    return (uint32_t)std::min<uint64_t>((total_codes + slots - 1) / slots + 1, 0x7FFFFFFFu);
}
inline uint32_t marker_unit_shift(uint64_t total, int n_cu) {
    uint32_t free_shift = 15;
    while (free_shift < 20 && (total >> (free_shift + 1)) >= 2ull * (uint64_t)std::max(n_cu, 1)) free_shift++;
    return free_shift;
}
inline uint64_t sym_units(const std::vector<BlkEmit> &emit, const std::vector<BlkUnits> &uv, std::vector<SymUnit> &su) {
    uint64_t max_len = 0;
    su.clear();
    for (size_t q = 0; q < emit.size(); q++)
        for (uint32_t b = 0; b < uv[q].fn && b < MAX_FREE_UNITS; b++) {
            const uint64_t len = uv[q].fout0[b + 1] - uv[q].fout0[b];
            if (!len) continue;
            su.push_back(SymUnit{emit[q].out_off + uv[q].fout0[b], len});
            max_len = std::max(max_len, len);
        }
    return max_len;
}

}
```

Before: 59.80 GB/s.

## Resolve decode block chain on device to avoid host round trip

Adds a single-workgroup kernel that links scanned block candidates into the chain from the first block to the final block, using pointer jumping and a prefix scan, then writes the emit records and totals on the GPU. Placement and checksum kernels read their sizes and parameters from device memory, so the host no longer has to copy block infos back, walk the chain, and upload emit jobs between scan and emit. This removes a synchronisation and host walk per member, at the cost of a serial-ish one-block kernel and checksum grids sized for the worst case. A host path is kept behind LFX_HOST_CHAIN, and a fallback is counted when the device chain is rejected.

```diff
diff --git a/include/lfx_testhooks.h b/include/lfx_testhooks.h
--- a/include/lfx_testhooks.h
+++ b/include/lfx_testhooks.h
@@ -19,6 +19,8 @@
 
 void lfx_debug_symbols(uint32_t length, uint32_t distance, uint32_t *out6);
 
+void lfx_debug_decode_device_chains(const lfx_ctx *ctx, uint64_t *taken, uint64_t *fell_back);
+
 #ifdef __cplusplus
 }
 #endif
diff --git a/libflate_amd/_ffi.py b/libflate_amd/_ffi.py
--- a/libflate_amd/_ffi.py
+++ b/libflate_amd/_ffi.py
@@ -269,6 +269,8 @@
     L.lfx_debug_plan_incremental.argtypes = [i32, C.POINTER(EncodeOpts), C.POINTER(Schedule), u64, u32, vp, C.c_size_t,
                                              C.POINTER(C.c_size_t), vp, C.c_size_t, C.POINTER(C.c_size_t)]
     L.lfx_debug_symbols.argtypes = [u32, u32, vp]
+    L.lfx_debug_decode_device_chains.restype = None
+    L.lfx_debug_decode_device_chains.argtypes = [vp, C.POINTER(u64), C.POINTER(u64)]
     _lib = L
     return L
 
diff --git a/libflate_amd/context.py b/libflate_amd/context.py
--- a/libflate_amd/context.py
+++ b/libflate_amd/context.py
@@ -57,6 +57,11 @@
         return {"total_ms": t.total_ms,
                 "phases": [(bytes(t.phase_name[i]).split(b"\0")[0].decode(), t.phase_ms[i])
                            for i in range(t.n_phases)]}
+
+    def decode_device_chains(self):
+        taken, fell = C.c_uint64(0), C.c_uint64(0)
+        _ffi.lib().lfx_debug_decode_device_chains(self._h, C.byref(taken), C.byref(fell))
+        return int(taken.value), int(fell.value)
 
     def match_fallbacks(self):
         return int(_ffi.lib().lfx_ctx_match_fallbacks(self._h))
diff --git a/libflate_amd/csrc/lfx_api.cpp b/libflate_amd/csrc/lfx_api.cpp
--- a/libflate_amd/csrc/lfx_api.cpp
+++ b/libflate_amd/csrc/lfx_api.cpp
@@ -230,6 +230,7 @@
     no_pin_slots = on("LFX_NO_PIN_SLOTS");
     no_small_scan = on("LFX_NO_SMALL_SCAN");
     store_tight = on("LFX_STORE_TIGHT");
+    host_chain = on("LFX_HOST_CHAIN");
 }
 
 void Ctx::phase(const char *name) {
@@ -324,6 +325,11 @@
 }
 extern "C" uint64_t lfx_ctx_match_fallbacks(const lfx_ctx *cc) {
     return cc ? reinterpret_cast<const Ctx *>(cc)->match_fallbacks : 0;
+}
+extern "C" void lfx_debug_decode_device_chains(const lfx_ctx *cc, uint64_t *taken, uint64_t *fell_back) {
+    const Ctx *c = reinterpret_cast<const Ctx *>(cc);
+    if (taken) *taken = c ? c->dev_chains_taken : 0;
+    if (fell_back) *fell_back = c ? c->dev_chains_fell_back : 0;
 }
 extern "C" void lfx_ctx_enable_timing(lfx_ctx *cc, int on) { reinterpret_cast<Ctx *>(cc)->timing_on = on >= 2 && on <= 6 ? on : on != 0; }
 extern "C" int lfx_ctx_last_timing(lfx_ctx *cc, lfx_timing *t) try {
diff --git a/libflate_amd/csrc/lfx_blk.h b/libflate_amd/csrc/lfx_blk.h
--- a/libflate_amd/csrc/lfx_blk.h
+++ b/libflate_amd/csrc/lfx_blk.h
@@ -48,6 +48,29 @@
     uint64_t temp_off;
     uint32_t cap, _pad;
 };
+enum : uint32_t { CHAIN_TAKEN = 0,
+                  CHAIN_NO_ROOT = 1,
+                  CHAIN_STATUS = 2,
+                  CHAIN_END_BIT = 3,
+                  CHAIN_UNSTORED = 4,
+                  CHAIN_UNKNOWN_NEXT = 5,
+                  CHAIN_CAP = 6,
+                  CHAIN_CODES = 7,
+                  CHAIN_TRAILER = 8,
+                  CHAIN_NO_FINAL = 9 };
+constexpr uint32_t CHAIN_MAX_CAND = 4096;
+constexpr uint32_t CHAIN_LANES = 256;
+struct ChainResult {
+    uint32_t ok, reason;
+    uint32_t ne;
+    uint32_t final;
+    uint32_t unit_target;
+    uint32_t free_shift;
+    uint64_t total, total_codes;
+    uint64_t last_end;
+    uint8_t trailer[8];
+};
+constexpr uint32_t M2_FEW_JOBS = 4;
 constexpr uint32_t MAX_FREE_UNITS = 64;
 struct BlkUnits {
     uint32_t n;
diff --git a/libflate_amd/csrc/lfx_ctx.h b/libflate_amd/csrc/lfx_ctx.h
--- a/libflate_amd/csrc/lfx_ctx.h
+++ b/libflate_amd/csrc/lfx_ctx.h
@@ -36,6 +36,7 @@
     bool no_pin_slots = false;
     int find2_exp = 0;
     bool hist_separate = false;
+    bool host_chain = false;
     bool store_tight = false;
     int enc_batch_mb = 0;
     void read();
@@ -121,6 +122,7 @@
     const uint8_t *cur_in = nullptr;
     bool force_match_v1 = false;
     uint64_t match_fallbacks = 0;
+    uint64_t dev_chains_taken = 0, dev_chains_fell_back = 0;
     HostIo hostio;
     static constexpr size_t POOL_MAX = 8;
     std::vector<PinVec> pin_pool;
diff --git a/libflate_amd/csrc/lfx_decode.h b/libflate_amd/csrc/lfx_decode.h
--- a/libflate_amd/csrc/lfx_decode.h
+++ b/libflate_amd/csrc/lfx_decode.h
@@ -87,7 +87,11 @@
                           BlkInfo *infos, BlkLanes *lanes, void *tabs, uint32_t *temp, BlkLanesX *lanesx);
 int launch_blk_place(hipStream_t st, const BlkEmit *jobs, uint32_t njobs, const BlkLanes *lanes, const BlkLanesX *lanesx,
                      const uint32_t *temp, uint32_t *codes, uint32_t *flags, BlkUnits *units, uint32_t unit_target,
-                     uint32_t *job_flags, uint32_t free_shift);
+                     uint32_t *job_flags, uint32_t free_shift,
+                     const ChainResult *chain = nullptr);
+struct ChainArgs;
+int launch_blk_chain(hipStream_t st, const uint8_t *in, uint64_t nbytes, const ChainArgs &args, uint32_t *flags, BlkEmit *emit,
+                     ChainResult *res);
 int launch_blk_emit(hipStream_t st, const uint8_t *in, uint64_t nbytes, const BlkEmit *jobs, uint32_t njobs,
                     const BlkLanes *lanes, uint32_t *codes, uint32_t *flags, BlkUnits *units, uint32_t unit_target,
                     uint32_t *job_flags = nullptr,
diff --git a/libflate_amd/csrc/lfx_device.h b/libflate_amd/csrc/lfx_device.h
--- a/libflate_amd/csrc/lfx_device.h
+++ b/libflate_amd/csrc/lfx_device.h
@@ -97,6 +97,13 @@
 int launch_checksum(hipStream_t st, const uint8_t *in, uint64_t n, uint32_t *crc_part,
                     uint32_t *a_part, uint32_t *b_part, EncodeResult *res,
                     int mode = 3)   ;
+inline uint64_t ck_nspans_max(uint64_t n_max) {
+    const uint64_t small = n_max < (64ull << 20) ? n_max : (64ull << 20);
+    const uint64_t a = div_up(small ? small : 1, 8192), b = div_up(n_max ? n_max : 1, 65536);
+    return a > b ? a : b;
+}
+int launch_checksum_dev(hipStream_t st, const uint8_t *in, uint64_t n_max, const uint64_t *n_dev, const uint32_t *ok_dev,
+                        uint32_t *crc_part, uint32_t *a_part, uint32_t *b_part, EncodeResult *res, int mode);
 int launch_checksum_part(hipStream_t st, const uint8_t *in, uint64_t n, uint32_t *crc_part, uint32_t *a_part, uint32_t *b_part,
                          EncodeResult *res, int mode, uint32_t part, uint32_t nparts);
 int launch_checksum_ranges(hipStream_t st, const uint8_t *data, uint32_t count, const uint64_t *off,
diff --git a/libflate_amd/csrc/lfx_encode_kernels.hip b/libflate_amd/csrc/lfx_encode_kernels.hip
--- a/libflate_amd/csrc/lfx_encode_kernels.hip
+++ b/libflate_amd/csrc/lfx_encode_kernels.hip
@@ -922,6 +922,26 @@
     if (lane == 0) { crc_part[region] = r.crc; a_part[region] = r.a; b_part[region] = r.b; }
 }
 
+template <int MODE>
+__global__ __launch_bounds__(256) void checksum_span_dev_kernel(const uint8_t *__restrict__ in, const uint64_t *__restrict__ n_dev,
+                                                                const uint32_t *__restrict__ ok_dev, uint32_t *__restrict__ crc_part,
+                                                                uint32_t *__restrict__ a_part, uint32_t *__restrict__ b_part) {
+    __shared__ uint32_t tab[4][256];
+    __shared__ uint32_t advt[4][256];
+    if (!*ok_dev) return;
+    const uint64_t n = *n_dev;
+    const uint32_t span = n <= (64ull << 20) ? 8192u : 65536u;
+    if ((uint64_t)blockIdx.x * 4 * span >= n) return;
+    ck_tables(tab, advt);
+    const uint32_t lane = threadIdx.x & 63;
+    const uint64_t region = (uint64_t)blockIdx.x * 4 + (threadIdx.x >> 6);
+    const uint64_t r0 = region * span;
+    if (r0 >= n) return;
+    const uint32_t rlen = (uint32_t)min((uint64_t)span, n - r0);
+    const CkPartial r = ck_span_partial<MODE>(in + r0, rlen, lane, tab, advt);
+    if (lane == 0) { crc_part[region] = r.crc; a_part[region] = r.a; b_part[region] = r.b; }
+}
+
 __global__ __launch_bounds__(256) void checksum_ranges_kernel(const uint8_t *__restrict__ data, uint32_t count,
                                                               const uint64_t *__restrict__ off, uint32_t off_stride,
                                                               const uint64_t *__restrict__ len, uint32_t len_stride,
@@ -952,11 +972,9 @@
     }
 }
 
-__global__ __launch_bounds__(1024) void checksum_combine_kernel(const uint32_t *__restrict__ crc_part,
-                                                                const uint32_t *__restrict__ a_part,
-                                                                const uint32_t *__restrict__ b_part,
-                                                                uint64_t n, uint32_t span,
-                                                                EncodeResult *__restrict__ res) {
+__device__ __forceinline__ void ck_combine_body(const uint32_t *__restrict__ crc_part, const uint32_t *__restrict__ a_part,
+                                                const uint32_t *__restrict__ b_part, uint64_t n, uint32_t span,
+                                                EncodeResult *__restrict__ res) {
     __shared__ uint32_t s_crc[16], s_a[16], s_b[16];
     const uint64_t nspans = div_up(n, span);
     const uint64_t per = div_up(nspans ? nspans : 1, 1023);
@@ -999,6 +1017,22 @@
         res->adler32 = (Bv << 16) | Af;
     }
 }
+__global__ __launch_bounds__(1024) void checksum_combine_kernel(const uint32_t *__restrict__ crc_part,
+                                                                const uint32_t *__restrict__ a_part,
+                                                                const uint32_t *__restrict__ b_part,
+                                                                uint64_t n, uint32_t span,
+                                                                EncodeResult *__restrict__ res) {
+    ck_combine_body(crc_part, a_part, b_part, n, span, res);
+}
+__global__ __launch_bounds__(1024) void checksum_combine_dev_kernel(const uint32_t *__restrict__ crc_part,
+                                                                    const uint32_t *__restrict__ a_part,
+                                                                    const uint32_t *__restrict__ b_part,
+                                                                    const uint64_t *__restrict__ n_dev, const uint32_t *__restrict__ ok_dev,
+                                                                    EncodeResult *__restrict__ res) {
+    if (!*ok_dev) return;
+    const uint64_t n = *n_dev;
+    ck_combine_body(crc_part, a_part, b_part, n, n <= (64ull << 20) ? 8192u : 65536u, res);
+}
 
 __global__ void put_bytes_kernel(const uint8_t *__restrict__ bytes, uint32_t n, uint64_t at_byte,
                                  uint32_t *__restrict__ out) {
@@ -1159,6 +1193,19 @@
                     uint32_t *a_part, uint32_t *b_part, EncodeResult *res, int mode) {
     return launch_checksum_part(st, in, n, crc_part, a_part, b_part, res, mode, 0, 1);
 }
+int launch_checksum_dev(hipStream_t st, const uint8_t *in, uint64_t n_max, const uint64_t *n_dev, const uint32_t *ok_dev,
+                        uint32_t *crc_part, uint32_t *a_part, uint32_t *b_part, EncodeResult *res, int mode) {
+    const uint64_t ngroups = div_up(ck_nspans_max(n_max), 4);
+    if (ngroups > 0x7FFFFFFFull) return (int)hipErrorInvalidValue;
+    const dim3 grid((uint32_t)ngroups);
+    if (mode == 1) hipLaunchKernelGGL(checksum_span_dev_kernel<1>, grid, dim3(256), 0, st, in, n_dev, ok_dev, crc_part, a_part, b_part);
+    else if (mode == 2) hipLaunchKernelGGL(checksum_span_dev_kernel<2>, grid, dim3(256), 0, st, in, n_dev, ok_dev, crc_part, a_part, b_part);
+    else hipLaunchKernelGGL(checksum_span_dev_kernel<3>, grid, dim3(256), 0, st, in, n_dev, ok_dev, crc_part, a_part, b_part);
+    LFX_LAUNCH_CHECK();
+    hipLaunchKernelGGL(checksum_combine_dev_kernel, dim3(1), dim3(1024), 0, st, crc_part, a_part, b_part, n_dev, ok_dev, res);
+    LFX_LAUNCH_CHECK();
+    return 0;
+}
 int launch_checksum_ranges(hipStream_t st, const uint8_t *data, uint32_t count, const uint64_t *off,
                            uint32_t off_stride, const uint64_t *len, uint32_t len_stride, uint32_t *crc, uint32_t *adler) {
     if (!count) return 0;
diff --git a/libflate_amd/csrc/lfx_inflate_fast.hip b/libflate_amd/csrc/lfx_inflate_fast.hip
--- a/libflate_amd/csrc/lfx_inflate_fast.hip
+++ b/libflate_amd/csrc/lfx_inflate_fast.hip
@@ -6,6 +6,7 @@
 
 #include "lfx_common.h"
 #include "lfx_decode.h"
+#include "lfx_stages.h"
 
 namespace lfx {
 
@@ -1314,10 +1315,12 @@
                                                                   const BlkLanesX *__restrict__ lanesx, const uint32_t *__restrict__ temp,
                                                                   uint32_t *__restrict__ codes, uint32_t *__restrict__ flags,
                                                                   BlkUnits *__restrict__ units, uint32_t unit_target, uint32_t free_shift,
-                                                                  uint32_t *__restrict__ job_flags) {
+                                                                  uint32_t *__restrict__ job_flags,
+                                                                  const ChainResult *__restrict__ chain) {
     const uint32_t tid = threadIdx.x, lane = tid & 63;
     const BlkEmit job = jobs[blockIdx.x];
     if (!job.placed) return;
+    if (chain) { unit_target = chain->unit_target; free_shift = chain->free_shift; }
     const uint64_t t_begin = clock64();
     BlkUnits *U = &units[blockIdx.x];
     const BlkLanes *L = &lanes[job.cand];
@@ -1377,6 +1380,24 @@
     blk_units_tail(tid, job, L, reach, cut_code, cut_pos, U, unit_target, free_shift, t_begin, t_hdr);
 }
 
+__global__ __launch_bounds__(CHAIN_LANES) void blk_chain_kernel(const uint8_t *__restrict__ in, uint64_t nbytes, ChainArgs args,
+                                                                 uint32_t *__restrict__ flags, BlkEmit *__restrict__ emit,
+                                                                 ChainResult *__restrict__ res) {
+    __shared__ ChainWork w;
+    const uint32_t tid = threadIdx.x;
+    if (tid < 16) flags[tid] = 0u;
+    const uint32_t steps = chain_steps(args.nc);
+    for (uint32_t s = 0; s < steps; ++s) {
+        chain_step(args, w, s, tid, emit, res);
+        __syncthreads();
+    }
+    if (tid != 0) return;
+    if (res->ok && args.want_trailer) {
+        const uint64_t end_byte = (res->last_end + 7) / 8;
+        for (uint32_t k = 0; k < args.trailer_len && end_byte + k < nbytes; ++k) res->trailer[k] = in[end_byte + k];
+    }
+}
+
 template <uint32_t THREADS>
 struct M2 {
     static constexpr uint32_t WAVES = THREADS / 64;
@@ -1388,7 +1409,6 @@
 };
 constexpr uint32_t M2_THREADS = 256;
 constexpr uint32_t M2_WIDE_THREADS = 1024;
-constexpr uint32_t M2_FEW_JOBS = 4;
 constexpr uint32_t M2_SYM_THREADS = 256;
 constexpr uint32_t M2_DONE = 0xFFFFu;
 #ifndef LFX_M2_PRIO_TILES
@@ -2253,10 +2273,17 @@
 }
 int launch_blk_place(hipStream_t st, const BlkEmit *jobs, uint32_t njobs, const BlkLanes *lanes, const BlkLanesX *lanesx,
                      const uint32_t *temp, uint32_t *codes, uint32_t *flags, BlkUnits *units, uint32_t unit_target, uint32_t *job_flags,
-                     uint32_t free_shift) {
+                     uint32_t free_shift, const ChainResult *chain) {
     if (!njobs) return 0;
     hipLaunchKernelGGL(blk_place_kernel, dim3(njobs, 2), dim3(SCAN_THREADS), 0, st, jobs, lanes, lanesx, temp, codes, flags, units,
-                       unit_target ? unit_target : 1u, free_shift < 15 ? 15u : free_shift, job_flags);
+                       unit_target ? unit_target : 1u, free_shift < 15 ? 15u : free_shift, job_flags, chain);
+    LFX_LAUNCH_CHECK();
+    return 0;
+}
+int launch_blk_chain(hipStream_t st, const uint8_t *in, uint64_t nbytes, const ChainArgs &args, uint32_t *flags, BlkEmit *emit,
+                     ChainResult *res) {
+    if (!args.nc || args.nc > CHAIN_MAX_CAND || args.trailer_len > 8) return (int)hipErrorInvalidValue;
+    hipLaunchKernelGGL(blk_chain_kernel, dim3(1), dim3(CHAIN_LANES), 0, st, in, nbytes, args, flags, emit, res);
     LFX_LAUNCH_CHECK();
     return 0;
 }
diff --git a/libflate_amd/csrc/lfx_member.cpp b/libflate_amd/csrc/lfx_member.cpp
--- a/libflate_amd/csrc/lfx_member.cpp
+++ b/libflate_amd/csrc/lfx_member.cpp
@@ -373,7 +373,65 @@
     return LFX_OK;
 }
 
-int block_scan(const Member &m, const std::vector<uint64_t> &starts, uint32_t n1, Chain &ch, MemberResult &mr) {
+int chain_on_device(const Member &m, uint32_t nc, MemberResult &mr, bool &done) {
+    Ctx *c = m.c;
+    hipStream_t st = c->stream;
+    const uint64_t codes_cap = std::max<uint64_t>(std::min<uint64_t>(m.cap, m.comp * 8 / 4), 1);
+    const bool want_ck = mr.ck_mode != 0;
+    int rc;
+    constexpr size_t AT_RES = 64, AT_CK = 128, AT_EMIT = 256;
+    static_assert(sizeof(ChainResult) <= AT_CK - AT_RES && sizeof(EncodeResult) <= AT_EMIT - AT_CK, "layout");
+    if ((rc = c->d_dec_tmp.reserve(AT_EMIT + sizeof(BlkEmit) * (size_t)nc))) return rc;
+    if ((rc = c->d_hist.reserve(sizeof(BlkUnits) * (size_t)nc + 64))) return rc;
+    if ((rc = c->d_codes.reserve(4 * codes_cap))) return rc;
+    const uint64_t nspans = ck_nspans_max(m.cap);
+    if (want_ck && (rc = c->d_ck.reserve(12 * nspans))) return rc;
+    uint8_t *base = (uint8_t *)c->d_dec_tmp.p;
+    uint32_t *d_flags = (uint32_t *)base;
+    ChainResult *d_cr = (ChainResult *)(base + AT_RES);
+    BlkEmit *d_emit = (BlkEmit *)(base + AT_EMIT);
+    const ChainArgs args{(const BlkJob *)c->d_dec_streams.p, (const BlkInfo *)c->d_dec_state.p, nc, c->n_cu, m.first_bit, m.end_bits(),
+                         m.cap, codes_cap, want_ck ? 1u : 0u, want_ck ? mr.trailer_len : 0u};
+    LAUNCH_TRY(launch_blk_chain(st, m.d_in, m.n, args, d_flags, d_emit, d_cr));
+    c->phase("blk_scan");
+    LAUNCH_TRY(launch_blk_place(st, d_emit, nc, (const BlkLanes *)c->d_dec_blocks.p, (const BlkLanesX *)c->d_dec_lanesx.p,
+                                (const uint32_t *)c->d_dec_temp.p, (uint32_t *)c->d_codes.p, d_flags, (BlkUnits *)c->d_hist.p, 0, nullptr, 0, d_cr));
+    c->phase("blk_emit");
+    LAUNCH_TRY(launch_blk_materialize(st, m.d_in, d_emit, nc, (const BlkLanes *)c->d_dec_blocks.p, (const BlkUnits *)c->d_hist.p,
+                                      (const uint32_t *)c->d_codes.p, m.d_out, nullptr));
+    c->phase("lz77_copy");
+    if (want_ck) {
+        uint32_t *ck = (uint32_t *)c->d_ck.p;
+        LAUNCH_TRY(launch_checksum_dev(st, m.d_out, m.cap, &d_cr->total, &d_cr->ok, ck, ck + nspans, ck + 2 * nspans,
+                                       (EncodeResult *)(base + AT_CK), mr.ck_mode));
+    }
+    uint8_t back[AT_EMIT];
+    HIP_TRY(c->small_down(back, base, AT_EMIT, st));
+    HIP_TRY(c->small_sync(st));
+    ChainResult cr;
+    EncodeResult er;
+    uint32_t fl;
+    memcpy(&fl, back, 4);
+    memcpy(&cr, back + AT_RES, sizeof cr);
+    memcpy(&er, back + AT_CK, sizeof er);
+    if (!cr.ok || fl != 0) return LFX_OK;
+    if (want_ck) {
+        mr.ck_done = true; mr.crc32 = er.crc32; mr.adler32 = er.adler32;
+        memcpy(mr.trailer, cr.trailer, mr.trailer_len);
+        c->phase("checksum");
+    }
+    const uint64_t end_bit = cr.last_end;
+    mr.status = LFX_OK;
+    mr.out_len = cr.total;
+    mr.blk_out_start = cr.total;
+    mr.end_byte = end_bit / 8 + ((end_bit & 7) ? 1 : 0);
+    mr.end_bit = end_bit;
+    mr.final_seen = cr.final != 0;
+    done = true;
+    return LFX_OK;
+}
+
+int block_scan(const Member &m, const std::vector<uint64_t> &starts, uint32_t n1, Chain &ch, MemberResult &mr, bool direct, bool &done) {
     Ctx *c = m.c;
     hipStream_t st = c->stream;
     const uint8_t *d_in = m.d_in;
@@ -401,12 +459,19 @@
     else
         LAUNCH_TRY(launch_blk_scan(st, d_in, n, (const BlkJob *)c->d_dec_streams.p, nj, (BlkInfo *)c->d_dec_state.p,
                                    (BlkLanes *)c->d_dec_blocks.p, c->d_dec_tabs.p, ch.scan_small));
+    const bool dev_chain = direct && store_mode && !c->diag.host_chain && !c->diag.debug && !c->idx && !m.partial && m.stop_bit == ~0ull &&
+                           m.hist == 0 && nc > M2_FEW_JOBS && nc <= CHAIN_MAX_CAND;
+    if (dev_chain) {
+        if ((rc = chain_on_device(m, nc, mr, done))) return rc;
+        if (done) { c->dev_chains_taken++; return LFX_OK; }
+        c->dev_chains_fell_back++;
+    }
     std::vector<BlkInfo> bi(nj);
     HIP_TRY(c->small_down(bi.data(), c->d_dec_state.p, sizeof(BlkInfo) * nj, st));
     HIP_TRY(c->small_sync(st));
     for (BlkInfo &b : bi) if (b.status == BLK_OK && b.end_bit > n * 8) b.status = BLK_NO_EOB;
     if (store_mode) for (uint32_t j = 0; j < nj; j++) stored[j] = bi[j].status == BLK_OK && bi[j].btype != 0 && bi[j]._pad == 0;
-    c->phase("blk_scan");
+    if (!dev_chain) c->phase("blk_scan");
     std::vector<uint32_t> slot(nc);
     for (uint32_t i = 0; i < nc; i++)
         slot[i] = (bi[i].status == BLK_NO_EOB && alt[i] >= 0 && bi[alt[i]].status == BLK_OK) ? (uint32_t)alt[i] : i;
@@ -641,11 +706,12 @@
             Chain ch(m.first_bit);
             const uint32_t nc = (uint32_t)starts.size();
             const bool giant_blocks = nc <= 8 && m.comp / nc >= (2u << 20);
-            if (may_piece && !small_first && !giant_blocks && nc >= 2 && nc <= PIECE_RANGES_MAX && m.comp / nc >= (128u << 10) &&
-                (rc = pieces_over_ranges(m, starts, ch)))
-                return rc;
-            if (!ch.pieces && may_piece && (small_first || giant_blocks) && (rc = pieces_block_walk(m, small_first, starts, fd, ch))) return rc;
-            if (!ch.pieces && !fd.overflow && (rc = block_scan(m, starts, fd.n1, ch, mr))) return rc;
+            const bool over_ranges = may_piece && !small_first && !giant_blocks && nc >= 2 && nc <= PIECE_RANGES_MAX && m.comp / nc >= (128u << 10);
+            const bool block_walk = may_piece && (small_first || giant_blocks);
+            if (over_ranges && (rc = pieces_over_ranges(m, starts, ch))) return rc;
+            if (!ch.pieces && block_walk && (rc = pieces_block_walk(m, small_first, starts, fd, ch))) return rc;
+            if (!ch.pieces && !fd.overflow && (rc = block_scan(m, starts, fd.n1, ch, mr, !over_ranges && !block_walk, done))) return rc;
+            if (done) return LFX_OK;
             if (c->diag.debug) fprintf(stderr, "[lfx]  chain ok=%d blocks=%zu pos=%llu total=%llu on_demand=%u\n", (int)ch.ok, ch.emit.size(), (unsigned long long)ch.pos, (unsigned long long)ch.total, ch.n_on_demand);
             if (partial && ch.emit.empty() && !ch.front_bad) {
                 mr.status = LFX_OK; mr.out_len = 0; mr.blk_out_start = 0; mr.final_seen = false;
diff --git a/libflate_amd/csrc/lfx_stages.h b/libflate_amd/csrc/lfx_stages.h
--- a/libflate_amd/csrc/lfx_stages.h
+++ b/libflate_amd/csrc/lfx_stages.h
@@ -4,6 +4,12 @@
 #include <vector>
 
 #include "lfx_blk.h"
+
+#if defined(__HIPCC__)
+#define LFX_HD __host__ __device__
+#else
+#define LFX_HD
+#endif
 
 namespace lfx {
 
@@ -72,7 +78,7 @@
     for (uint32_t j = 0; j < nj; j++) { bj[j].temp_off = 0; bj[j].cap = 0; }
 }
 
-inline BlkEmit blk_emit_of(const BlkInfo &r, uint64_t start_bit, uint32_t slot, uint64_t out_off, uint64_t code_off, uint64_t hist) {
+LFX_HD inline BlkEmit blk_emit_of(const BlkInfo &r, uint64_t start_bit, uint32_t slot, uint64_t out_off, uint64_t code_off, uint64_t hist) {
     BlkEmit e{};
     e.start_bit = start_bit; e.data_bit = r.data_bit; e.code_off = code_off; e.out_off = out_off;
     e.n_out = r.n_out; e.n_codes = r.n_codes; e.nlanes = r.nlanes; e.btype = r.btype; e.cand = slot;
@@ -80,13 +86,14 @@
     e.end_limit = r.status == BLK_NO_EOB ? r.end_bit : 0;
     return e;
 }
-inline uint32_t emit_unit_target(uint64_t total_codes, int n_cu) {
-    const uint64_t slots = 4ull * (uint64_t)std::max(n_cu, 1);
-    return (uint32_t)std::min<uint64_t>((total_codes + slots - 1) / slots + 1, 0x7FFFFFFFu);
-}
-inline uint32_t marker_unit_shift(uint64_t total, int n_cu) {
+LFX_HD inline uint32_t emit_unit_target(uint64_t total_codes, int n_cu) {
+    const uint64_t slots = 4ull * (uint64_t)(n_cu > 1 ? n_cu : 1);
+    const uint64_t t = (total_codes + slots - 1) / slots + 1;
+    return (uint32_t)(t < 0x7FFFFFFFu ? t : 0x7FFFFFFFu);
+}
+LFX_HD inline uint32_t marker_unit_shift(uint64_t total, int n_cu) {
     uint32_t free_shift = 15;
-    while (free_shift < 20 && (total >> (free_shift + 1)) >= 2ull * (uint64_t)std::max(n_cu, 1)) free_shift++;
+    while (free_shift < 20 && (total >> (free_shift + 1)) >= 2ull * (uint64_t)(n_cu > 1 ? n_cu : 1)) free_shift++;
     return free_shift;
 }
 inline uint64_t sym_units(const std::vector<BlkEmit> &emit, const std::vector<BlkUnits> &uv, std::vector<SymUnit> &su) {
@@ -102,4 +109,144 @@
     return max_len;
 }
 
-}
+struct ChainArgs {
+    const BlkJob *bj;
+    const BlkInfo *bi;
+    uint32_t nc;
+    int n_cu;
+    uint64_t first_bit;
+    uint64_t end_bits;
+    uint64_t cap, codes_cap;
+    uint32_t want_trailer;
+    uint32_t trailer_len;
+};
+constexpr uint32_t CHAIN_NONE = 0xFFFFu, CHAIN_END = 0xFFFEu;
+struct ChainWork {
+    uint16_t nxt[2][CHAIN_MAX_CAND];
+    uint8_t mark[CHAIN_MAX_CAND];
+    uint8_t why[CHAIN_MAX_CAND];
+    uint64_t s_out[2][CHAIN_LANES], s_codes[2][CHAIN_LANES];
+    uint32_t s_cnt[2][CHAIN_LANES];
+    uint32_t s_bad[2][CHAIN_LANES], s_fin[2][CHAIN_LANES];
+    uint32_t root;
+};
+LFX_HD inline uint32_t chain_find(const BlkJob *bj, uint32_t nc, uint64_t bit) {
+    uint32_t lo = 0, hi = nc;
+    while (lo < hi) {
+        const uint32_t mid = (lo + hi) / 2;
+        if (bj[mid].start_bit < bit) lo = mid + 1; else hi = mid;
+    }
+    return lo < nc && bj[lo].start_bit == bit ? lo : CHAIN_NONE;
+}
+LFX_HD inline uint32_t chain_block_reason(const BlkInfo &r, uint64_t pos, uint64_t end_bits) {
+    if (r.status != BLK_OK || r.end_bit > end_bits) return CHAIN_STATUS;
+    if (r.end_bit <= pos) return CHAIN_END_BIT;
+    if (r.btype == 0 || r._pad != 0) return CHAIN_UNSTORED;
+    return CHAIN_TAKEN;
+}
+LFX_HD inline BlkEmit chain_emit_of(const BlkInfo &r, const BlkJob &j, uint32_t i, uint64_t out_off, uint64_t code_off) {
+    BlkEmit e = blk_emit_of(r, j.start_bit, i, out_off, code_off, out_off);
+    e.placed = 1; e.temp_off = j.temp_off; e.cap = j.cap;
+    return e;
+}
+LFX_HD inline uint32_t chain_rounds(uint32_t nc) {
+    uint32_t r = 0;
+    while ((1u << r) < nc) r++;
+    return r;
+}
+constexpr uint32_t CHAIN_SCAN_ROUNDS = 8;
+static_assert((1u << CHAIN_SCAN_ROUNDS) == CHAIN_LANES, "lanes");
+LFX_HD inline uint32_t chain_steps(uint32_t nc) { return chain_rounds(nc) + CHAIN_SCAN_ROUNDS + 3; }
+LFX_HD inline uint32_t chain_verdict(const ChainArgs &a, const ChainWork &w) {
+    const uint32_t L = CHAIN_LANES - 1;
+    if (w.root == CHAIN_NONE) return CHAIN_NO_ROOT;
+    if (w.s_bad[0][L] != 0xFFFFFFFFu) return w.s_bad[0][L] & 15u;
+    if (!w.s_fin[0][L]) return CHAIN_NO_FINAL;
+    if (w.s_out[0][L] > a.cap) return CHAIN_CAP;
+    if (w.s_codes[0][L] > a.codes_cap) return CHAIN_CODES;
+    if (a.want_trailer) {
+        const uint64_t last_end = a.bi[w.s_fin[0][L] - 1].end_bit, end_byte = last_end / 8 + ((last_end & 7) ? 1 : 0);
+        if (w.s_out[0][L] == 0 || end_byte + a.trailer_len > a.end_bits / 8) return CHAIN_TRAILER;
+    }
+    return CHAIN_TAKEN;
+}
+LFX_HD inline void chain_step(const ChainArgs &a, ChainWork &w, uint32_t step, uint32_t lane, BlkEmit *emit, ChainResult *res) {
+    const uint32_t nc = a.nc, R = chain_rounds(nc);
+    const uint32_t per = (nc + CHAIN_LANES - 1) / CHAIN_LANES;
+    const uint32_t i0 = lane * per < nc ? lane * per : nc, i1 = i0 + per < nc ? i0 + per : nc;
+    if (step == 0) {
+        if (lane == 0) w.root = chain_find(a.bj, nc, a.first_bit);
+        for (uint32_t i = i0; i < i1; i++) {
+            const BlkInfo r = a.bi[i];
+            uint32_t why = chain_block_reason(r, a.bj[i].start_bit, a.end_bits), nx = CHAIN_NONE;
+            if (!why) {
+                if (r.bfinal) nx = CHAIN_END;
+                else {
+                    nx = chain_find(a.bj, nc, r.end_bit);
+                    if (nx == CHAIN_NONE) why = CHAIN_UNKNOWN_NEXT;
+                }
+            }
+            w.nxt[0][i] = (uint16_t)nx;
+            w.why[i] = (uint8_t)why;
+            w.mark[i] = a.bj[i].start_bit == a.first_bit && (i == 0 || a.bj[i - 1].start_bit != a.first_bit);
+        }
+    } else if (step <= R) {
+        const uint32_t src = (step - 1) & 1, dst = step & 1;
+        for (uint32_t i = i0; i < i1; i++) {
+            const uint32_t nx = w.nxt[src][i];
+            if (nx < nc) {
+                if (w.mark[i]) w.mark[nx] = 1;
+                w.nxt[dst][i] = w.nxt[src][nx];
+            } else w.nxt[dst][i] = (uint16_t)nx;
+        }
+    } else if (step == R + 1) {
+        uint64_t so = 0, sc = 0;
+        uint32_t cnt = 0, bad = 0xFFFFFFFFu, fin = 0;
+        for (uint32_t i = i0; i < i1; i++) {
+            if (!w.mark[i]) continue;
+            if (w.why[i]) { if (bad == 0xFFFFFFFFu) bad = i << 4 | w.why[i]; continue; }
+            const BlkInfo r = a.bi[i];
+            so += r.n_out; sc += r.n_codes; cnt++;
+            if (r.bfinal) fin = i + 1;
+        }
+        w.s_out[0][lane] = so; w.s_codes[0][lane] = sc; w.s_cnt[0][lane] = cnt; w.s_bad[0][lane] = bad; w.s_fin[0][lane] = fin;
+    } else if (step <= R + 1 + CHAIN_SCAN_ROUNDS) {
+        const uint32_t k = step - R - 2, src = k & 1, dst = (k + 1) & 1, d = 1u << k;
+        uint64_t so = w.s_out[src][lane], sc = w.s_codes[src][lane];
+        uint32_t cnt = w.s_cnt[src][lane], bad = w.s_bad[src][lane], fin = w.s_fin[src][lane];
+        if (lane >= d) {
+            so += w.s_out[src][lane - d]; sc += w.s_codes[src][lane - d]; cnt += w.s_cnt[src][lane - d];
+            const uint32_t b2 = w.s_bad[src][lane - d];
+            bad = b2 < bad ? b2 : bad;
+            const uint32_t f2 = w.s_fin[src][lane - d];
+            fin = f2 > fin ? f2 : fin;
+        }
+        w.s_out[dst][lane] = so; w.s_codes[dst][lane] = sc; w.s_cnt[dst][lane] = cnt; w.s_bad[dst][lane] = bad; w.s_fin[dst][lane] = fin;
+    } else {
+        static_assert(CHAIN_SCAN_ROUNDS % 2 == 0, "the sums end in buffer 0");
+        const uint32_t reason = chain_verdict(a, w);
+        uint64_t out_off = lane ? w.s_out[0][lane - 1] : 0, code_off = lane ? w.s_codes[0][lane - 1] : 0;
+        for (uint32_t i = i0; i < i1; i++) {
+            BlkEmit e{};
+            if (!reason && w.mark[i]) {
+                const BlkInfo r = a.bi[i];
+                e = chain_emit_of(r, a.bj[i], i, out_off, code_off);
+                out_off += r.n_out; code_off += r.n_codes;
+            }
+            emit[i] = e;
+        }
+        if (lane == 0) {
+            const uint32_t L = CHAIN_LANES - 1;
+            ChainResult cr{};
+            cr.ok = !reason; cr.reason = reason;
+            cr.ne = w.s_cnt[0][L]; cr.final = w.s_fin[0][L] != 0;
+            cr.total = w.s_out[0][L]; cr.total_codes = w.s_codes[0][L];
+            const uint32_t ut = emit_unit_target(cr.total_codes, a.n_cu), fs = marker_unit_shift(cr.total, a.n_cu);
+            cr.unit_target = ut ? ut : 1u; cr.free_shift = fs < 15 ? 15u : fs;
+            cr.last_end = w.s_fin[0][L] ? a.bi[w.s_fin[0][L] - 1].end_bit : 0;
+            *res = cr;
+        }
+    }
+}
+
+}
```

Result: no change. 59.92 GB/s, median of 2 (+0.2%).
